# yanyan-li/PlanarSLAM

Measured on AMD Instinct MI355X. Metric: RGB-D frames/sec (extract+match+pose-opt) @640x480; 1->8-GPU batch scaling, higher is better.
Workload: dtype u8/f64

## Files before the change

### include/planar_abi.h

```cpp
#ifndef PLANAR_ABI_H
#define PLANAR_ABI_H

#include <stdint.h>

#ifdef __cplusplus
extern "C" {
#endif

#define PLANAR_OK 0
#define PLANAR_EINVAL (-1)
#define PLANAR_ENOMEM (-2)
#define PLANAR_EDEVICE (-3)
#define PLANAR_ECAPACITY (-4)
#define PLANAR_ESTATE (-5)

typedef struct planar_ctx planar_ctx;

typedef struct planar_keypoint {
    float x, y;
    float size;
    float angle;
    float response;
    int32_t octave;
    int32_t class_id;
// ... 193 lines not shown
    float level_sigma2[PLANAR_MAX_LEVELS];
} planar_tri_camera;

typedef struct planar_tri_keyframes {
    int32_t count, stride;
    const int32_t* n;
    const planar_keypoint* keys_un;
    const float* u_right;
    const uint8_t* desc;
    const int32_t* node;
    const uint8_t* occupied;
    const float* Tcw;
    const planar_keypoint* keys;
    const float* depth;
    const float* cos_stereo;
    const float* Twc;
    const float* mb;
    const float* mbf;
} planar_tri_keyframes;

int planar_search_for_triangulation(planar_ctx* ctx, const planar_tri_camera* cam, const planar_tri_keyframes* kf1, const planar_tri_keyframes* kf2,
                                    int only_stereo, int check_orientation, int32_t* match12, int32_t* nmatches);
int planar_search_for_triangulation_dev(planar_ctx* ctx, const planar_tri_camera* cam, const planar_tri_keyframes* d_kf1,
                                        const planar_tri_keyframes* d_kf2, int only_stereo, int check_orientation, int32_t* d_match12,
                                        int32_t* d_nmatches);

int planar_create_new_map_points(planar_ctx* ctx, const planar_tri_camera* cam, const planar_tri_keyframes* cur, const planar_tri_keyframes* neigh,
                                 const int32_t* n_neigh, int max_neigh, int32_t* n_new, int32_t* new_neigh, int32_t* new_idx1, int32_t* new_idx2,
                                 float* new_x3d);
int planar_create_new_map_points_dev(planar_ctx* ctx, const planar_tri_camera* cam, const planar_tri_keyframes* d_cur,
                                     const planar_tri_keyframes* d_neigh, const int32_t* d_n_neigh, int max_neigh, int32_t* d_n_new,
                                     int32_t* d_new_neigh, int32_t* d_new_idx1, int32_t* d_new_idx2, float* d_new_x3d);

#define PLANAR_MAX_KEYFRAME_LINES 256

struct planar_keyline;
typedef struct planar_tri_line_keyframes {
    int32_t count, stride;
    const int32_t* n;
    const struct planar_keyline* keylines;
    const uint8_t* ldesc;
    const uint8_t* occupied;
    const float* depth_line;
    const double* lines3d;
    const float* Tcw;
    const float* Twc;
    const float* mb;
} planar_tri_line_keyframes;

int planar_lsd_search_for_triangulation(planar_ctx* ctx, const planar_tri_line_keyframes* kf1, const planar_tri_line_keyframes* kf2, int32_t* match12,
                                        int32_t* nmatches, double* nn_mad, double* nn12_mad);
int planar_lsd_search_for_triangulation_dev(planar_ctx* ctx, const planar_tri_line_keyframes* d_kf1, const planar_tri_line_keyframes* d_kf2,
                                            int32_t* d_match12, int32_t* d_nmatches, double* d_nn_mad, double* d_nn12_mad);
int planar_lsd_search_by_descriptor_kf(planar_ctx* ctx, const planar_tri_line_keyframes* kf1, const planar_tri_line_keyframes* kf2, int32_t* match12,
                                       int32_t* nmatches);
int planar_lsd_search_by_descriptor_kf_dev(planar_ctx* ctx, const planar_tri_line_keyframes* d_kf1, const planar_tri_line_keyframes* d_kf2,
                                           int32_t* d_match12, int32_t* d_nmatches);

int planar_create_new_map_lines(planar_ctx* ctx, const planar_tri_camera* cam, const planar_tri_line_keyframes* cur, const planar_tri_line_keyframes* neigh,
                                const int32_t* n_neigh, int max_neigh, int32_t* n_new, int32_t* new_neigh, int32_t* new_idx1, int32_t* new_idx2,
                                double* new_line);
int planar_create_new_map_lines_dev(planar_ctx* ctx, const planar_tri_camera* cam, const planar_tri_line_keyframes* d_cur,
                                    const planar_tri_line_keyframes* d_neigh, const int32_t* d_n_neigh, int max_neigh, int32_t* d_n_new,
                                    int32_t* d_new_neigh, int32_t* d_new_idx1, int32_t* d_new_idx2, double* d_new_line);

int planar_update_average_dir(planar_ctx* ctx, int G, const int32_t* n, int stride, const double* xw6, const uint8_t* valid, const float* ref_Tcw,
                              const int32_t* ref_octave, const int32_t* obs_off, const float* obs_ow, const float* scale_factors, int n_levels,
                              double* normal, float* min_dist, float* max_dist);
int planar_update_average_dir_dev(planar_ctx* ctx, int G, const int32_t* d_n, int stride, const double* d_xw6, const uint8_t* d_valid,
                                  const float* d_ref_Tcw, const int32_t* d_ref_octave, const int32_t* d_obs_off, const float* d_obs_ow,
                                  const float* scale_factors, int n_levels, double* d_normal, float* d_min_dist, float* d_max_dist);

int planar_is_in_frustum_points(planar_ctx* ctx, const planar_frame_view* frame, float log_scale_factor, int n_levels, const int32_t* n, int stride,
                                const uint8_t* valid, const float* xw, const float* normal, const float* min_dist, const float* max_dist,
                                float viewing_cos_limit, uint8_t* in_view, float* proj_x, float* proj_y, float* proj_xr, int32_t* level,
                                float* view_cos);
int planar_is_in_frustum_points_dev(planar_ctx* ctx, const planar_frame_view* d_frame, float log_scale_factor, int n_levels, const int32_t* d_n,
                                    int stride, const uint8_t* d_valid, const float* d_xw, const float* d_normal, const float* d_min_dist,
                                    const float* d_max_dist, float viewing_cos_limit, uint8_t* d_in_view, float* d_proj_x, float* d_proj_y,
                                    float* d_proj_xr, int32_t* d_level, float* d_view_cos);
int planar_is_in_frustum_lines(planar_ctx* ctx, const planar_frame_view* frame, float log_scale_factor, const int32_t* n, int stride,
                               const uint8_t* valid, const double* xw6, const double* normal, const float* min_dist, const float* max_dist,
                               float viewing_cos_limit, uint8_t* in_view, float* proj, int32_t* level, float* view_cos);
int planar_is_in_frustum_lines_dev(planar_ctx* ctx, const planar_frame_view* d_frame, float log_scale_factor, const int32_t* d_n, int stride,
                                   const uint8_t* d_valid, const double* d_xw6, const double* d_normal, const float* d_min_dist,
                                   const float* d_max_dist, float viewing_cos_limit, uint8_t* d_in_view, float* d_proj, int32_t* d_level,
                                   float* d_view_cos);

int planar_fuse_search(planar_ctx* ctx, const planar_frame_view* kf, const float* inv_level_sigma2, float log_scale_factor, int n_levels,
                       const int32_t* n, int stride, int points_shared, const uint8_t* usable, const float* xw, const float* normal,
                       const float* min_dist, const float* max_dist, const uint8_t* desc, float th, int32_t* fuse_idx, int32_t* fuse_dist,
                       int32_t* n_fused);
int planar_fuse_search_dev(planar_ctx* ctx, const planar_frame_view* d_kf, const float* inv_level_sigma2 , float log_scale_factor, int n_levels,
                           const int32_t* d_n, int stride, int points_shared, const uint8_t* d_usable, const float* d_xw, const float* d_normal,
                           const float* d_min_dist, const float* d_max_dist, const uint8_t* d_desc, float th, int32_t* d_fuse_idx,
                           int32_t* d_fuse_dist, int32_t* d_n_fused);

typedef struct planar_keyline {
    float angle;
    int32_t class_id, octave;
    float pt_x, pt_y, response, size;
    float start_x, start_y, end_x, end_y;
    float s_oct_x, s_oct_y, e_oct_x, e_oct_y;
    float line_length;
    int32_t num_pixels;
} planar_keyline;

int planar_lsd_search_by_projection(planar_ctx* ctx, int B, const int32_t* n_lines, int line_stride, const planar_keyline* keylines,
                                    const uint8_t* ldesc, const uint8_t* blocked, const int32_t* n_ml, int ml_stride,
                                    const uint8_t* ml_in_view, const float* ml_proj, const int32_t* ml_level, const float* ml_view_cos,
                                    const uint8_t* ml_desc, const uint8_t* ml_observed, const float* scale_factors, int n_levels, float th,
                                    float nn_ratio, int32_t* match, int32_t* nmatches);
int planar_lsd_search_by_projection_dev(planar_ctx* ctx, int B, const int32_t* d_n_lines, int line_stride, const planar_keyline* d_keylines,
                                        const uint8_t* d_ldesc, const uint8_t* d_blocked, const int32_t* d_n_ml, int ml_stride,
                                        const uint8_t* d_ml_in_view, const float* d_ml_proj, const int32_t* d_ml_level,
                                        const float* d_ml_view_cos, const uint8_t* d_ml_desc, const uint8_t* d_ml_observed,
                                        const float* scale_factors , int n_levels, float th, float nn_ratio, int32_t* d_match,
                                        int32_t* d_nmatches);

int planar_lsd_fuse_search(planar_ctx* ctx, const planar_frame_view* kf, float log_scale_factor, int n_levels, const int32_t* n_lines, int line_stride,
                           const planar_keyline* keylines, const uint8_t* ldesc, const int32_t* n_ml, int ml_stride, int lines_shared,
                           const uint8_t* usable, const double* xw6, const double* normal, const float* min_dist, const float* max_dist,
                           const uint8_t* ml_desc, float th, int32_t* fuse_idx, int32_t* fuse_dist, int32_t* n_fused);
int planar_lsd_fuse_search_dev(planar_ctx* ctx, const planar_frame_view* d_kf, float log_scale_factor, int n_levels, const int32_t* d_n_lines, int line_stride,
                               const planar_keyline* d_keylines, const uint8_t* d_ldesc, const int32_t* d_n_ml, int ml_stride, int lines_shared,
                               const uint8_t* d_usable, const double* d_xw6, const double* d_normal, const float* d_min_dist, const float* d_max_dist,
                               const uint8_t* d_ml_desc, float th, int32_t* d_fuse_idx, int32_t* d_fuse_dist, int32_t* d_n_fused);

int planar_plane_search_by_coefficients(planar_ctx* ctx, int B, const int32_t* n_planes, int pl_stride, const float* pl_coef,
                                        const float* Tcw, int map_shared, const int32_t* n_mp, int mp_stride, const uint8_t* mp_valid,
                                        const float* mp_coef, const int32_t* mp_npts, int pts_stride, const float* mp_pts,
                                        const float* th, int32_t* match, int32_t* ver, int32_t* par, int32_t* nmatches);
int planar_plane_search_by_coefficients_dev(planar_ctx* ctx, int B, const int32_t* d_n_planes, int pl_stride, const float* d_pl_coef,
                                            const float* d_Tcw, int map_shared, const int32_t* d_n_mp, int mp_stride,
                                            const uint8_t* d_mp_valid, const float* d_mp_coef, const int32_t* d_mp_npts, int pts_stride,
                                            const float* d_mp_pts, const float* th , int32_t* d_match, int32_t* d_ver,
                                            int32_t* d_par, int32_t* d_nmatches);

typedef struct planar_lsd planar_lsd;
int planar_lsd_create(planar_ctx* ctx, int width, int height, int max_batch, planar_lsd** out);
void planar_lsd_destroy(planar_lsd* lsd);
int planar_lsd_max_segments(void);
int planar_lsd_scaled_size(planar_lsd* lsd, int* w, int* h);
int planar_lsd_set_tie_order(planar_lsd* lsd, int tie_order);
int planar_lsd_set_top_only(planar_lsd* lsd, int enable);
int planar_lsd_extract(planar_lsd* lsd, const uint8_t* gray, int B, int pitch, int64_t frame_stride, int max_lines, planar_keyline* keylines,
                       uint8_t* ldesc, double* line_eq, int32_t* n_lines);
int planar_lsd_extract_dev(planar_lsd* lsd, const uint8_t* d_gray, int B, int pitch, int64_t frame_stride, int max_lines,
                           planar_keyline* d_keylines, uint8_t* d_ldesc, double* d_line_eq, int32_t* d_n_lines);
int planar_lsd_preprocess_dev(planar_lsd* lsd, const uint8_t* d_gray, int B, int pitch, int64_t frame_stride);
int planar_lsd_detect_dev(planar_lsd* lsd, int B, int max_lines, planar_keyline* d_keylines, uint8_t* d_ldesc, double* d_line_eq, int32_t* d_n_lines);
int planar_lsd_check(planar_lsd* lsd, int B);
int planar_lsd_read_stage(planar_lsd* lsd, int frame, int stage, void* out, int64_t out_bytes);
int planar_lsd_set_profiling(planar_lsd* lsd, int enable);
int planar_lsd_get_profile(planar_lsd* lsd, double* total_ms, int64_t* calls);
#ifdef PLANAR_TEST_HOOKS
int planar_debug_std_sort_desc(planar_ctx* ctx, float* keys, int32_t* perm, int n);
#endif

typedef struct planar_peac planar_peac;
int planar_peac_create(planar_ctx* ctx, int width, int height, int max_batch, planar_peac** out);
void planar_peac_destroy(planar_peac* peac);
int planar_peac_max_planes(void);
int planar_peac_segment(planar_peac* peac, const uint16_t* depth, int B, int pitch_px, int64_t frame_stride_px, float fx, float fy,
                        float cx, float cy, float depth_factor, int32_t* labels, double* planes, int32_t* n_planes);
int planar_peac_segment_dev(planar_peac* peac, const uint16_t* d_depth, int B, int pitch_px, int64_t frame_stride_px, float fx, float fy,
                            float cx, float cy, float depth_factor, int32_t* d_labels, double* d_planes, int32_t* d_n_planes);
int planar_peac_debug_layout(planar_peac* peac, int64_t* out );
int planar_peac_debug_read(planar_peac* peac, int frame, int64_t offset, int64_t bytes, void* out);
int planar_peac_check(planar_peac* peac, int B);
int planar_peac_set_variant(planar_peac* peac, int clustering, int wide_below);
int planar_peac_set_profiling(planar_peac* peac, int enable);
int planar_peac_get_profile(planar_peac* peac, double* total_ms, int64_t* calls);
int planar_peac_read_timing(planar_peac* peac, int B, int64_t* out);

typedef struct planar_comm planar_comm;
typedef struct planar_comm_id { char internal[128]; } planar_comm_id;
int planar_comm_unique_id(planar_comm_id* out);
int planar_comm_create(planar_ctx* ctx, const planar_comm_id* id, int nranks, int rank, planar_comm** out);
typedef int (*planar_allreduce_fn)(void* user, double* buf, size_t n, int op);
int planar_comm_create_hosted(planar_ctx* ctx, planar_allreduce_fn allreduce, void* user, int nranks, int rank, planar_comm** out);
void planar_comm_destroy(planar_comm* comm);

#define PLANAR_BA_MONO 0
#define PLANAR_BA_STEREO 1
#define PLANAR_BA_LINE 2
#define PLANAR_BA_PLANE 3
#define PLANAR_BA_VERTICAL 4
#define PLANAR_BA_PARALLEL 5

typedef struct planar_ba_problem {
    int32_t n_kf;
    const float* kf_Tcw;
    const uint8_t* kf_fixed;
    int32_t n_lm;
    const uint8_t* lm_type;
    const double* lm_init;
    int32_t n_edges;
    const int32_t* e_kf;
    const int32_t* e_lm;
    const uint8_t* e_type;
    const double* e_meas;
    const float* e_inv_sigma2;
} planar_ba_problem;

typedef struct planar_ba_result {
    float* kf_Tcw;
    double* lm;
    uint8_t* e_outlier;
    int32_t lm_iterations;
    int32_t stopped;
} planar_ba_result;

int planar_local_ba(planar_ctx* ctx, const planar_ba_problem* problem, const planar_pose_params* params, int its1, int its2,
                    planar_ba_result* result, const volatile unsigned char* stop_flag, planar_comm* comm);

typedef struct planar_vocab planar_vocab;
int planar_vocab_create(planar_ctx* ctx, int k, int L, int n_nodes, const int32_t* parent, const uint8_t* is_leaf, const uint8_t* desc ,
                        const double* weight, planar_vocab** out);
void planar_vocab_destroy(planar_vocab* voc);
int planar_vocab_words(const planar_vocab* voc);
int planar_bow_transform(planar_vocab* voc, const uint8_t* desc, const int32_t* n, int B, int stride, int levelsup, int32_t* word, double* weight,
                         int32_t* node, int32_t* bow_word, double* bow_value, int32_t* bow_n);
int planar_bow_transform_dev(planar_vocab* voc, const uint8_t* d_desc, const int32_t* d_n, int B, int stride, int levelsup, int32_t* d_word,
                             double* d_weight, int32_t* d_node, int32_t* d_bow_word, double* d_bow_value, int32_t* d_bow_n);

#define PLANAR_KFDB_MAX_WORDS 4096
#define PLANAR_KFDB_MAX_KEYFRAMES 1024
typedef struct planar_kf_database {
    int32_t kf_stride, word_stride;
    const int32_t* n_kf;
    const uint8_t* present;
    const int32_t* add_seq;
    const int32_t* bow_n;
    const int32_t* bow_word;
    const double*  bow_value;
    const int32_t* covis;
} planar_kf_database;
int planar_kfdb_detect(planar_ctx* ctx, int mode, const planar_kf_database* db, int B, const int32_t* q_db, const int32_t* q_bow_n, const int32_t* q_bow_word,
                       const double* q_bow_value, int q_word_stride, const uint8_t* excluded, const float* min_score, float* score, int32_t* common_words,
                       int32_t* n_cand, int32_t* cand, int32_t* n_scored);
int planar_kfdb_detect_dev(planar_ctx* ctx, int mode, const planar_kf_database* db, int B, const int32_t* d_q_db, const int32_t* d_q_bow_n,
                           const int32_t* d_q_bow_word, const double* d_q_bow_value, int q_word_stride, const uint8_t* d_excluded, const float* d_min_score,
                           float* d_score, int32_t* d_common_words, int32_t* d_n_cand, int32_t* d_cand, int32_t* d_n_scored);
int planar_bow_score(planar_ctx* ctx, int P, const int32_t* a_bow_n, const int32_t* a_bow_word, const double* a_bow_value, int a_stride, const int32_t* b_bow_n,
                     const int32_t* b_bow_word, const double* b_bow_value, int b_stride, double* out);
int planar_bow_score_dev(planar_ctx* ctx, int P, const int32_t* d_a_bow_n, const int32_t* d_a_bow_word, const double* d_a_bow_value, int a_stride,
                         const int32_t* d_b_bow_n, const int32_t* d_b_bow_word, const double* d_b_bow_value, int b_stride, double* d_out);

int planar_is_line_good(planar_ctx* ctx, int B, const planar_keyline* keylines, const int32_t* n_lines, int ln_stride, const uint16_t* depth, int width,
                        int height, int pitch_px, int64_t frame_stride_px, float depth_factor, float fx, float fy, float cx, float cy, const uint32_t* seeds,
                        float* depth_line, double* lines3d, uint8_t* good, double* direction, int32_t* n_inliers, double* packed_dirs, int32_t* n_good);
int planar_is_line_good_dev(planar_ctx* ctx, int B, const planar_keyline* d_keylines, const int32_t* d_n_lines, int ln_stride, const uint16_t* d_depth,
                            int width, int height, int pitch_px, int64_t frame_stride_px, float depth_factor, float fx, float fy, float cx, float cy,
                            const uint32_t* d_seeds, float* d_depth_line, double* d_lines3d, uint8_t* d_good, double* d_direction, int32_t* d_n_inliers,
                            double* d_packed_dirs, int32_t* d_n_good);

typedef struct planar_normals planar_normals;
int planar_normals_create(planar_ctx* ctx, int width, int height, int max_batch, planar_normals** out);
void planar_normals_destroy(planar_normals* nrm);
int planar_normals_count(const planar_normals* nrm);
int planar_normals_grid(const planar_normals* nrm, int* grid_w, int* grid_h, int* out_w, int* out_h);
int planar_normals_compute(planar_normals* nrm, const uint16_t* depth, int B, int pitch_px, int64_t frame_stride_px, float fx, float fy, float cx,
                           float cy, float depth_factor, float* normals , float* points );
int planar_normals_compute_dev(planar_normals* nrm, const uint16_t* d_depth, int B, int pitch_px, int64_t frame_stride_px, float fx, float fy,
                               float cx, float cy, float depth_factor, float* d_normals, float* d_points, int out_stride);

int planar_track_manhattan_frame(planar_ctx* ctx, int B, const float* R_last, const float* normals, const int32_t* n_normals, int sn_stride,
                                 const double* line_dirs, const int32_t* n_lines, int ln_stride, float* R_out, uint8_t* member, int32_t* info,
                                 float* density);
int planar_track_manhattan_frame_dev(planar_ctx* ctx, int B, const float* d_R_last, const float* d_normals, const int32_t* d_n_normals, int sn_stride,
                                     const double* d_line_dirs, const int32_t* d_n_lines, int ln_stride, float* d_R_out, uint8_t* d_member,
                                     int32_t* d_info, float* d_density);

typedef struct planar_plane_clouds planar_plane_clouds;
int planar_plane_clouds_create(planar_ctx* ctx, int width, int height, int max_batch, int max_points , planar_plane_clouds** out);
void planar_plane_clouds_destroy(planar_plane_clouds* pc);
int planar_plane_clouds_stride(const planar_plane_clouds* pc, int* pl_stride, int* max_points);
int planar_plane_clouds_set_plane_window(planar_plane_clouds* pc, int first, int count);
int planar_plane_clouds_set_profiling(planar_plane_clouds* pc, int enable);
int planar_plane_clouds_get_profile(planar_plane_clouds* pc, double* total_ms, int64_t* calls);
int planar_plane_clouds_sort_stats(planar_plane_clouds* pc, int B, int64_t* out);
int planar_plane_clouds_set_timing(planar_plane_clouds* pc, int enable);
int planar_plane_clouds_read_timing(planar_plane_clouds* pc, int B, int64_t* out);
int planar_plane_clouds_compute(planar_plane_clouds* pc, const uint16_t* depth, int B, int pitch_px, int64_t frame_stride_px, float fx, float fy, float cx,
                                float cy, float depth_factor, const int32_t* labels, const double* planes, const int32_t* n_planes, double dist_th, float leaf,
                                int32_t* n_out, float* coef, int32_t* src, int32_t* pt_off, float* points, int32_t* state, int32_t* nvox, int32_t* info);
int planar_plane_clouds_compute_dev(planar_plane_clouds* pc, const uint16_t* d_depth, int B, int pitch_px, int64_t frame_stride_px, float fx, float fy,
                                    float cx, float cy, float depth_factor, const int32_t* d_labels, const double* d_planes, const int32_t* d_n_planes,
                                    double dist_th, float leaf, int32_t* d_n_out, float* d_coef, int32_t* d_src, int32_t* d_pt_off, float* d_points,
                                    int32_t* d_status, int32_t* d_state, int32_t* d_nvox, int32_t* d_info);
int planar_plane_clouds_last_status(planar_plane_clouds* pc, int B, int32_t* out);
int planar_plane_refit(planar_plane_clouds* pc, int n_clouds, const float* points, const int32_t* pt_off, double dist_th, float* planes, int32_t* state,
                       int32_t* info);
int planar_flag_matched_plane_points(planar_ctx* ctx, int B, const float* Tcw, const float* coef, const uint8_t* matched, const int32_t* n_planes, int pl_stride,
                                     const float* xw, int n_points, int points_shared, uint8_t* flags, int32_t* n_matches);
int planar_flag_matched_plane_points_dev(planar_ctx* ctx, int B, const float* d_Tcw, const float* d_coef, const uint8_t* d_matched, const int32_t* d_n_planes,
                                         int pl_stride, const float* d_xw, int n_points, int points_shared, uint8_t* d_flags, int32_t* d_n_matches);
int planar_merge_plane_points(planar_plane_clouds* pc, const double* Twc, const float* frame_points, int n_frame, const float* map_points, int n_map, float leaf,
                              float* out_points, int out_cap, int32_t* n_out);

int planar_stereo_from_rgbd(planar_ctx* ctx, int B, const planar_keypoint* keys, const planar_keypoint* keys_un, const int32_t* n, int stride,
                            const uint16_t* depth, int pitch_px, int64_t frame_stride_px, float depth_factor, float fx, float fy, float cx, float cy,
                            float bf, const float* Tcw, float* u_right, float* depth_out, float* xw, uint8_t* valid);
int planar_stereo_from_rgbd_dev(planar_ctx* ctx, int B, const planar_keypoint* d_keys, const planar_keypoint* d_keys_un, const int32_t* d_n, int stride,
                                const uint16_t* d_depth, int pitch_px, int64_t frame_stride_px, float depth_factor, float fx, float fy, float cx,
// ... 56 lines not shown
```

### planarslam_amd/_lib.py

```python
from __future__ import annotations

import ctypes as C
import os

import numpy as np

_HERE = os.path.dirname(os.path.abspath(__file__))
LIB_PATH = os.path.join(_HERE, "libplanar_hip.so")
if os.environ.get("PLANAR_HIP_LIB"):
    _ov = os.path.abspath(os.environ["PLANAR_HIP_LIB"])
    if os.path.dirname(_ov) != _HERE:
        raise ImportError(f"PLANAR_HIP_LIB={_ov}: a developer override must be a library inside {_HERE}")
    import warnings
    warnings.warn(f"planarslam_amd: loading the developer build {_ov} instead of libplanar_hip.so (PLANAR_HIP_LIB)")
    LIB_PATH = _ov

KP_DTYPE = np.dtype([("x", "<f4"), ("y", "<f4"), ("size", "<f4"), ("angle", "<f4"), ("response", "<f4"),
                     ("octave", "<i4"), ("class_id", "<i4")])


class PlanarError(RuntimeError):
    def __init__(self, code: int, msg: str):
        super().__init__(f"libplanar_hip error {code}: {msg}")
        self.code = code
# ... 26 lines not shown
KEYLINE_DTYPE = np.dtype([("angle", "<f4"), ("class_id", "<i4"), ("octave", "<i4"), ("pt_x", "<f4"), ("pt_y", "<f4"), ("response", "<f4"),
                          ("size", "<f4"), ("start_x", "<f4"), ("start_y", "<f4"), ("end_x", "<f4"), ("end_y", "<f4"), ("s_oct_x", "<f4"),
                          ("s_oct_y", "<f4"), ("e_oct_x", "<f4"), ("e_oct_y", "<f4"), ("line_length", "<f4"), ("num_pixels", "<i4")])
MAX_LEVELS = 16


class FrameView(C.Structure):
    _fields_ = [("B", C.c_int32), ("stride", C.c_int32), ("n", C.c_void_p), ("keys_un", C.c_void_p), ("u_right", C.c_void_p),
                ("desc", C.c_void_p), ("blocked", C.c_void_p), ("Tcw", C.c_void_p), ("min_x", C.c_float), ("max_x", C.c_float),
                ("min_y", C.c_float), ("max_y", C.c_float), ("grid_w_inv", C.c_float), ("grid_h_inv", C.c_float), ("fx", C.c_float),
                ("fy", C.c_float), ("cx", C.c_float), ("cy", C.c_float), ("bf", C.c_float), ("b", C.c_float),
                ("scale_factors", C.c_float * MAX_LEVELS)]


class LastFrameView(C.Structure):
    _fields_ = [("stride", C.c_int32)] + [(n, C.c_void_p) for n in ("n", "Tcw", "usable", "xw", "octave", "angle", "mp_desc", "mp_observed")]


class MapProbes(C.Structure):
    _fields_ = [("stride", C.c_int32)] + [(n, C.c_void_p) for n in ("n", "in_view", "proj_x", "proj_y", "proj_xr", "level", "view_cos", "desc",
                                                                   "observed")]


class KeyframeProbes(C.Structure):
    _fields_ = [("stride", C.c_int32)] + [(n, C.c_void_p) for n in ("n", "usable", "found", "xw", "min_dist", "max_dist", "angle", "desc")]


class TriCamera(C.Structure):
    _fields_ = [("fx", C.c_float), ("fy", C.c_float), ("cx", C.c_float), ("cy", C.c_float), ("invfx", C.c_float), ("invfy", C.c_float),
                ("scale_factor", C.c_float), ("n_levels", C.c_int32), ("scale_factors", C.c_float * MAX_LEVELS), ("level_sigma2", C.c_float * MAX_LEVELS)]


class TriLineKeyframes(C.Structure):
    _fields_ = [("count", C.c_int32), ("stride", C.c_int32)] + [(n, C.c_void_p) for n in ("n", "keylines", "ldesc", "occupied", "depth_line", "lines3d", "Tcw", "Twc", "mb")]


class TriKeyframes(C.Structure):
    _fields_ = [("count", C.c_int32), ("stride", C.c_int32)] + [(n, C.c_void_p) for n in ("n", "keys_un", "u_right", "desc", "node", "occupied", "Tcw", "keys",
                                                                                       "depth", "cos_stereo", "Twc", "mb", "mbf")]


class TrackMatches(C.Structure):
    _fields_ = [("B", C.c_int32), ("stride", C.c_int32), ("mp_stride", C.c_int32), ("n_levels", C.c_int32), ("n", C.c_void_p), ("keys_un", C.c_void_p),
                ("u_right", C.c_void_p), ("pt_match", C.c_void_p), ("mp_xw", C.c_void_p), ("mp_valid", C.c_void_p), ("inv_level_sigma2", C.c_float * MAX_LEVELS),
                ("ln_stride", C.c_int32), ("ml_stride", C.c_int32), ("n_lines", C.c_void_p), ("line_eq", C.c_void_p), ("ln_match", C.c_void_p), ("ml_xw6", C.c_void_p),
                ("pl_stride", C.c_int32), ("mpl_stride", C.c_int32), ("mpl_shared", C.c_int32), ("n_planes", C.c_void_p), ("pl_coef", C.c_void_p),
                ("pl_match", C.c_void_p), ("mpl_coef", C.c_void_p), ("Tcw", C.c_void_p)]


class KfDatabase(C.Structure):
    _fields_ = [("kf_stride", C.c_int32), ("word_stride", C.c_int32)] + [(n, C.c_void_p) for n in ("n_kf", "present", "add_seq", "bow_n", "bow_word", "bow_value", "covis")]


KFDB_MAX_WORDS = 4096
KFDB_MAX_KEYFRAMES = 1024


class BAResult(C.Structure):
    _fields_ = [("kf_Tcw", C.c_void_p), ("lm", C.c_void_p), ("e_outlier", C.c_void_p), ("lm_iterations", C.c_int32), ("stopped", C.c_int32)]


_SIGS = {
    "planar_last_error": (C.c_char_p, []),
    "planar_abi_version": (C.c_int, []),
    "planar_ctx_create": (C.c_int, [C.POINTER(C.c_void_p), C.c_int]),
    "planar_ctx_destroy": (None, [C.c_void_p]),
    "planar_ctx_set_stream": (C.c_int, [C.c_void_p, C.c_void_p]),
    "planar_ctx_get_stream": (C.c_void_p, [C.c_void_p]),
    "planar_cu_stream_create": (C.c_int, [C.c_int, C.c_void_p, C.c_int, C.POINTER(C.c_void_p)]),
    "planar_cu_stream_destroy": (None, [C.c_void_p]),
    "planar_ctx_set_seq_stream": (C.c_int, [C.c_void_p, C.c_void_p]),
    "planar_ctx_sync": (C.c_int, [C.c_void_p]),
    "planar_orb_create": (C.c_int, [C.c_void_p, C.POINTER(OrbParams), C.c_int, C.c_int, C.c_int, C.POINTER(C.c_void_p)]),
    "planar_orb_destroy": (None, [C.c_void_p]),
    "planar_orb_check": (C.c_int, [C.c_void_p]),
    "planar_peac_set_profiling": (C.c_int, [C.c_void_p, C.c_int]),
    "planar_peac_get_profile": (C.c_int, [C.c_void_p, C.c_void_p, C.POINTER(C.c_int64)]),
    "planar_orb_max_keypoints": (C.c_int, [C.c_void_p]),
    "planar_orb_get_scale_factors": (C.c_int, [C.c_void_p, C.c_void_p, C.c_void_p, C.c_void_p, C.c_void_p]),
    "planar_orb_level_size": (C.c_int, [C.c_void_p, C.c_int, C.POINTER(C.c_int), C.POINTER(C.c_int)]),
    "planar_orb_features_per_level": (C.c_int, [C.c_void_p, C.c_void_p]),
    "planar_orb_extract": (C.c_int, [C.c_void_p, C.c_void_p, C.c_int, C.c_int, C.c_int64, C.c_void_p, C.c_void_p, C.c_void_p]),
    "planar_orb_extract_dev": (C.c_int, [C.c_void_p, C.c_void_p, C.c_int, C.c_int, C.c_int64, C.c_void_p, C.c_void_p, C.c_void_p]),
    "planar_orb_read_level": (C.c_int, [C.c_void_p, C.c_int, C.c_int, C.c_void_p]),
    "planar_orb_read_blurred": (C.c_int, [C.c_void_p, C.c_int, C.c_int, C.c_void_p]),
    "planar_orb_read_candidates": (C.c_int, [C.c_void_p, C.c_int, C.c_int, C.c_void_p, C.c_int]),
    "planar_orb_set_profiling": (C.c_int, [C.c_void_p, C.c_int]),
    "planar_orb_profile_num_launches": (C.c_int, [C.c_void_p]),
    "planar_orb_profile_launch_name": (C.c_char_p, [C.c_void_p, C.c_int]),
    "planar_orb_get_profile": (C.c_int, [C.c_void_p, C.c_void_p, C.POINTER(C.c_int64)]),
    "planar_hamming_knn": (C.c_int, [C.c_void_p, C.c_void_p, C.c_void_p, C.c_int, C.c_void_p, C.c_void_p, C.c_int, C.c_int, C.c_int, C.c_void_p, C.c_void_p]),
    "planar_hamming_knn_dev": (C.c_int, [C.c_void_p, C.c_void_p, C.c_void_p, C.c_int, C.c_void_p, C.c_void_p, C.c_int, C.c_int, C.c_int, C.c_void_p, C.c_void_p]),
    "planar_match_orb_points": (C.c_int, [C.c_void_p, C.c_void_p, C.c_void_p, C.c_int, C.c_void_p, C.c_void_p, C.c_int, C.c_void_p, C.c_void_p, C.c_int, C.c_void_p, C.c_void_p]),
    "planar_match_orb_points_dev": (C.c_int, [C.c_void_p, C.c_void_p, C.c_void_p, C.c_int, C.c_void_p, C.c_void_p, C.c_int, C.c_void_p, C.c_void_p, C.c_int, C.c_void_p, C.c_void_p]),
    "planar_lsd_search_by_descriptor": (C.c_int, [C.c_void_p, C.c_void_p, C.c_void_p, C.c_int, C.c_void_p, C.c_void_p, C.c_int, C.c_void_p, C.c_int, C.c_void_p, C.c_void_p]),
    "planar_lsd_search_by_descriptor_dev": (C.c_int, [C.c_void_p, C.c_void_p, C.c_void_p, C.c_int, C.c_void_p, C.c_void_p, C.c_int, C.c_void_p, C.c_int, C.c_void_p, C.c_void_p]),
    "planar_search_by_projection_frame": (C.c_int, [C.c_void_p, C.POINTER(FrameView), C.POINTER(LastFrameView), C.c_float, C.c_int, C.c_int, C.c_void_p, C.c_void_p]),
    "planar_search_by_projection_frame_dev": (C.c_int, [C.c_void_p, C.POINTER(FrameView), C.POINTER(LastFrameView), C.c_float, C.c_int, C.c_int, C.c_void_p, C.c_void_p]),
    "planar_search_by_projection_map": (C.c_int, [C.c_void_p, C.POINTER(FrameView), C.POINTER(MapProbes), C.c_float, C.c_float, C.c_void_p, C.c_void_p]),
    "planar_search_by_projection_map_dev": (C.c_int, [C.c_void_p, C.POINTER(FrameView), C.POINTER(MapProbes), C.c_float, C.c_float, C.c_void_p, C.c_void_p]),
    "planar_search_by_projection_keyframe": (C.c_int, [C.c_void_p, C.POINTER(FrameView), C.POINTER(KeyframeProbes), C.c_float, C.c_int, C.c_float, C.c_int, C.c_int, C.c_void_p, C.c_void_p]),
    "planar_search_by_projection_keyframe_dev": (C.c_int, [C.c_void_p, C.POINTER(FrameView), C.POINTER(KeyframeProbes), C.c_float, C.c_int, C.c_float, C.c_int, C.c_int, C.c_void_p, C.c_void_p]),
    "planar_fuse_search": (C.c_int, [C.c_void_p, C.POINTER(FrameView), C.c_void_p, C.c_float, C.c_int, C.c_void_p, C.c_int, C.c_int] + [C.c_void_p] * 6 + [C.c_float] + [C.c_void_p] * 3),
    "planar_fuse_search_dev": (C.c_int, [C.c_void_p, C.POINTER(FrameView), C.c_void_p, C.c_float, C.c_int, C.c_void_p, C.c_int, C.c_int] + [C.c_void_p] * 6 + [C.c_float] + [C.c_void_p] * 3),
    "planar_lsd_fuse_search": (C.c_int, [C.c_void_p, C.POINTER(FrameView), C.c_float, C.c_int, C.c_void_p, C.c_int, C.c_void_p, C.c_void_p, C.c_void_p, C.c_int, C.c_int] + [C.c_void_p] * 6 + [C.c_float] + [C.c_void_p] * 3),
    "planar_lsd_fuse_search_dev": (C.c_int, [C.c_void_p, C.POINTER(FrameView), C.c_float, C.c_int, C.c_void_p, C.c_int, C.c_void_p, C.c_void_p, C.c_void_p, C.c_int, C.c_int] + [C.c_void_p] * 6 + [C.c_float] + [C.c_void_p] * 3),
    "planar_is_in_frustum_points": (C.c_int, [C.c_void_p, C.POINTER(FrameView), C.c_float, C.c_int, C.c_void_p, C.c_int] + [C.c_void_p] * 5 + [C.c_float] + [C.c_void_p] * 6),
    "planar_is_in_frustum_points_dev": (C.c_int, [C.c_void_p, C.POINTER(FrameView), C.c_float, C.c_int, C.c_void_p, C.c_int] + [C.c_void_p] * 5 + [C.c_float] + [C.c_void_p] * 6),
    "planar_is_in_frustum_lines": (C.c_int, [C.c_void_p, C.POINTER(FrameView), C.c_float, C.c_void_p, C.c_int] + [C.c_void_p] * 5 + [C.c_float] + [C.c_void_p] * 4),
    "planar_is_in_frustum_lines_dev": (C.c_int, [C.c_void_p, C.POINTER(FrameView), C.c_float, C.c_void_p, C.c_int] + [C.c_void_p] * 5 + [C.c_float] + [C.c_void_p] * 4),
    "planar_search_for_triangulation": (C.c_int, [C.c_void_p, C.POINTER(TriCamera), C.POINTER(TriKeyframes), C.POINTER(TriKeyframes), C.c_int, C.c_int, C.c_void_p, C.c_void_p]),
    "planar_search_for_triangulation_dev": (C.c_int, [C.c_void_p, C.POINTER(TriCamera), C.POINTER(TriKeyframes), C.POINTER(TriKeyframes), C.c_int, C.c_int, C.c_void_p, C.c_void_p]),
    "planar_create_new_map_points": (C.c_int, [C.c_void_p, C.POINTER(TriCamera), C.POINTER(TriKeyframes), C.POINTER(TriKeyframes), C.c_void_p, C.c_int] + [C.c_void_p] * 5),
    "planar_create_new_map_points_dev": (C.c_int, [C.c_void_p, C.POINTER(TriCamera), C.POINTER(TriKeyframes), C.POINTER(TriKeyframes), C.c_void_p, C.c_int] + [C.c_void_p] * 5),
    "planar_lsd_search_for_triangulation": (C.c_int, [C.c_void_p, C.POINTER(TriLineKeyframes), C.POINTER(TriLineKeyframes)] + [C.c_void_p] * 4),
    "planar_lsd_search_for_triangulation_dev": (C.c_int, [C.c_void_p, C.POINTER(TriLineKeyframes), C.POINTER(TriLineKeyframes)] + [C.c_void_p] * 4),
    "planar_lsd_search_by_descriptor_kf": (C.c_int, [C.c_void_p, C.POINTER(TriLineKeyframes), C.POINTER(TriLineKeyframes)] + [C.c_void_p] * 2),
    "planar_lsd_search_by_descriptor_kf_dev": (C.c_int, [C.c_void_p, C.POINTER(TriLineKeyframes), C.POINTER(TriLineKeyframes)] + [C.c_void_p] * 2),
    "planar_create_new_map_lines": (C.c_int, [C.c_void_p, C.POINTER(TriCamera), C.POINTER(TriLineKeyframes), C.POINTER(TriLineKeyframes), C.c_void_p, C.c_int] + [C.c_void_p] * 5),
    "planar_create_new_map_lines_dev": (C.c_int, [C.c_void_p, C.POINTER(TriCamera), C.POINTER(TriLineKeyframes), C.POINTER(TriLineKeyframes), C.c_void_p, C.c_int] + [C.c_void_p] * 5),
    "planar_update_average_dir": (C.c_int, [C.c_void_p, C.c_int, C.c_void_p, C.c_int] + [C.c_void_p] * 7 + [C.c_int] + [C.c_void_p] * 3),
    "planar_update_average_dir_dev": (C.c_int, [C.c_void_p, C.c_int, C.c_void_p, C.c_int] + [C.c_void_p] * 7 + [C.c_int] + [C.c_void_p] * 3),
    "planar_search_by_bow": (C.c_int, [C.c_void_p, C.c_int] + [C.c_void_p, C.c_int, C.c_void_p, C.c_void_p, C.c_void_p, C.c_void_p] +
                             [C.c_void_p, C.c_int, C.c_void_p, C.c_void_p, C.c_void_p] + [C.c_float, C.c_int, C.c_void_p, C.c_void_p]),
    "planar_search_by_bow_dev": (C.c_int, [C.c_void_p, C.c_int] + [C.c_void_p, C.c_int, C.c_void_p, C.c_void_p, C.c_void_p, C.c_void_p] +
                                 [C.c_void_p, C.c_int, C.c_void_p, C.c_void_p, C.c_void_p] + [C.c_float, C.c_int, C.c_void_p, C.c_void_p]),
    "planar_lsd_search_by_projection": (C.c_int, [C.c_void_p, C.c_int, C.c_void_p, C.c_int, C.c_void_p, C.c_void_p, C.c_void_p, C.c_void_p, C.c_int] +
                                        [C.c_void_p] * 6 + [C.c_void_p, C.c_int, C.c_float, C.c_float, C.c_void_p, C.c_void_p]),
    "planar_lsd_search_by_projection_dev": (C.c_int, [C.c_void_p, C.c_int, C.c_void_p, C.c_int, C.c_void_p, C.c_void_p, C.c_void_p, C.c_void_p, C.c_int] +
                                            [C.c_void_p] * 6 + [C.c_void_p, C.c_int, C.c_float, C.c_float, C.c_void_p, C.c_void_p]),
    "planar_plane_search_by_coefficients": (C.c_int, [C.c_void_p, C.c_int, C.c_void_p, C.c_int, C.c_void_p, C.c_void_p, C.c_int, C.c_void_p, C.c_int,
                                                      C.c_void_p, C.c_void_p, C.c_void_p, C.c_int, C.c_void_p, C.c_void_p] + [C.c_void_p] * 4),
    "planar_plane_search_by_coefficients_dev": (C.c_int, [C.c_void_p, C.c_int, C.c_void_p, C.c_int, C.c_void_p, C.c_void_p, C.c_int, C.c_void_p, C.c_int,
                                                          C.c_void_p, C.c_void_p, C.c_void_p, C.c_int, C.c_void_p, C.c_void_p] + [C.c_void_p] * 4),
    "planar_lsd_create": (C.c_int, [C.c_void_p, C.c_int, C.c_int, C.c_int, C.POINTER(C.c_void_p)]),
    "planar_lsd_destroy": (None, [C.c_void_p]),
    "planar_lsd_max_segments": (C.c_int, []),
    "planar_lsd_set_tie_order": (C.c_int, [C.c_void_p, C.c_int]),
    "planar_lsd_set_top_only": (C.c_int, [C.c_void_p, C.c_int]),
    "planar_undistort_keypoints": (C.c_int, [C.c_void_p, C.c_int, C.c_void_p, C.c_void_p, C.c_int] + [C.c_float] * 4 + [C.c_void_p, C.c_void_p]),
    "planar_undistort_keypoints_dev": (C.c_int, [C.c_void_p, C.c_int, C.c_void_p, C.c_void_p, C.c_int] + [C.c_float] * 4 + [C.c_void_p, C.c_void_p]),
    "planar_plane_clouds_sort_stats": (C.c_int, [C.c_void_p, C.c_int, C.c_void_p]),
    "planar_plane_clouds_set_profiling": (C.c_int, [C.c_void_p, C.c_int]),
    "planar_plane_clouds_get_profile": (C.c_int, [C.c_void_p, C.c_void_p, C.c_void_p]),
    "planar_lsd_set_profiling": (C.c_int, [C.c_void_p, C.c_int]),
    "planar_lsd_get_profile": (C.c_int, [C.c_void_p, C.c_void_p, C.c_void_p]),
    "planar_lsd_scaled_size": (C.c_int, [C.c_void_p, C.POINTER(C.c_int), C.POINTER(C.c_int)]),
    "planar_lsd_extract": (C.c_int, [C.c_void_p, C.c_void_p, C.c_int, C.c_int, C.c_int64, C.c_int, C.c_void_p, C.c_void_p, C.c_void_p, C.c_void_p]),
    "planar_lsd_extract_dev": (C.c_int, [C.c_void_p, C.c_void_p, C.c_int, C.c_int, C.c_int64, C.c_int, C.c_void_p, C.c_void_p, C.c_void_p, C.c_void_p]),
    "planar_lsd_preprocess_dev": (C.c_int, [C.c_void_p, C.c_void_p, C.c_int, C.c_int, C.c_int64]),
    "planar_lsd_detect_dev": (C.c_int, [C.c_void_p, C.c_int, C.c_int, C.c_void_p, C.c_void_p, C.c_void_p, C.c_void_p]),
    "planar_lsd_check": (C.c_int, [C.c_void_p, C.c_int]),
    "planar_lsd_read_stage": (C.c_int, [C.c_void_p, C.c_int, C.c_int, C.c_void_p, C.c_int64]),
    "planar_debug_std_sort_desc": (C.c_int, [C.c_void_p, C.c_void_p, C.c_void_p, C.c_int]),
    "planar_peac_create": (C.c_int, [C.c_void_p, C.c_int, C.c_int, C.c_int, C.POINTER(C.c_void_p)]),
    "planar_peac_destroy": (None, [C.c_void_p]),
    "planar_peac_max_planes": (C.c_int, []),
    "planar_peac_segment": (C.c_int, [C.c_void_p, C.c_void_p, C.c_int, C.c_int, C.c_int64, C.c_float, C.c_float, C.c_float, C.c_float, C.c_float, C.c_void_p, C.c_void_p, C.c_void_p]),
    "planar_peac_segment_dev": (C.c_int, [C.c_void_p, C.c_void_p, C.c_int, C.c_int, C.c_int64, C.c_float, C.c_float, C.c_float, C.c_float, C.c_float, C.c_void_p, C.c_void_p, C.c_void_p]),
    "planar_peac_check": (C.c_int, [C.c_void_p, C.c_int]),
    "planar_peac_set_variant": (C.c_int, [C.c_void_p, C.c_int, C.c_int]),
    "planar_track_manhattan_frame": (C.c_int, [C.c_void_p, C.c_int, C.c_void_p, C.c_void_p, C.c_void_p, C.c_int, C.c_void_p, C.c_void_p, C.c_int, C.c_void_p, C.c_void_p, C.c_void_p, C.c_void_p]),
    "planar_track_manhattan_frame_dev": (C.c_int, [C.c_void_p, C.c_int, C.c_void_p, C.c_void_p, C.c_void_p, C.c_int, C.c_void_p, C.c_void_p, C.c_int, C.c_void_p, C.c_void_p, C.c_void_p, C.c_void_p]),
    "planar_peac_read_timing": (C.c_int, [C.c_void_p, C.c_int, C.c_void_p]),
    "planar_reset_matches_dev": (C.c_int, [C.c_void_p, C.c_void_p, C.c_int64]),
    "planar_blocked_mask_dev": (C.c_int, [C.c_void_p, C.c_void_p, C.c_int64, C.c_void_p]),
    "planar_merge_matches_dev": (C.c_int, [C.c_void_p, C.c_void_p, C.c_void_p, C.c_int, C.c_int64, C.c_void_p]),
    "planar_manhattan_pose_dev": (C.c_int, [C.c_void_p, C.c_int, C.c_void_p, C.c_void_p, C.c_void_p, C.c_void_p]),
    "planar_keypoint_fields_dev": (C.c_int, [C.c_void_p, C.c_void_p, C.c_int64, C.c_void_p, C.c_void_p]),
    "planar_add_scalar_i32_dev": (C.c_int, [C.c_void_p, C.c_void_p, C.c_int64, C.c_int, C.c_void_p]),
    "planar_copy_rows_dev": (C.c_int, [C.c_void_p, C.c_void_p, C.c_int64, C.c_void_p, C.c_int64, C.c_int64, C.c_int64]),
    "planar_peac_debug_layout": (C.c_int, [C.c_void_p, C.c_void_p]),
    "planar_peac_debug_read": (C.c_int, [C.c_void_p, C.c_int, C.c_int64, C.c_int64, C.c_void_p]),
    "planar_comm_unique_id": (C.c_int, [C.c_void_p]),
    "planar_comm_create": (C.c_int, [C.c_void_p, C.c_void_p, C.c_int, C.c_int, C.POINTER(C.c_void_p)]),
    "planar_vocab_create": (C.c_int, [C.c_void_p, C.c_int, C.c_int, C.c_int, C.c_void_p, C.c_void_p, C.c_void_p, C.c_void_p, C.POINTER(C.c_void_p)]),
    "planar_vocab_destroy": (None, [C.c_void_p]),
    "planar_vocab_words": (C.c_int, [C.c_void_p]),
    "planar_bow_transform": (C.c_int, [C.c_void_p, C.c_void_p, C.c_void_p, C.c_int, C.c_int, C.c_int] + [C.c_void_p] * 6),
    "planar_bow_transform_dev": (C.c_int, [C.c_void_p, C.c_void_p, C.c_void_p, C.c_int, C.c_int, C.c_int] + [C.c_void_p] * 6),
    "planar_kfdb_detect": (C.c_int, [C.c_void_p, C.c_int, C.POINTER(KfDatabase), C.c_int] + [C.c_void_p] * 4 + [C.c_int] + [C.c_void_p] * 7),
    "planar_kfdb_detect_dev": (C.c_int, [C.c_void_p, C.c_int, C.POINTER(KfDatabase), C.c_int] + [C.c_void_p] * 4 + [C.c_int] + [C.c_void_p] * 7),
    "planar_bow_score": (C.c_int, [C.c_void_p, C.c_int] + [C.c_void_p] * 3 + [C.c_int] + [C.c_void_p] * 3 + [C.c_int, C.c_void_p]),
    "planar_bow_score_dev": (C.c_int, [C.c_void_p, C.c_int] + [C.c_void_p] * 3 + [C.c_int] + [C.c_void_p] * 3 + [C.c_int, C.c_void_p]),
    "planar_is_line_good": (C.c_int, [C.c_void_p, C.c_int, C.c_void_p, C.c_void_p, C.c_int, C.c_void_p, C.c_int, C.c_int, C.c_int, C.c_int64, C.c_float, C.c_float, C.c_float, C.c_float, C.c_float] + [C.c_void_p] * 8),
    "planar_is_line_good_dev": (C.c_int, [C.c_void_p, C.c_int, C.c_void_p, C.c_void_p, C.c_int, C.c_void_p, C.c_int, C.c_int, C.c_int, C.c_int64, C.c_float, C.c_float, C.c_float, C.c_float, C.c_float] + [C.c_void_p] * 8),
    "planar_normals_create": (C.c_int, [C.c_void_p, C.c_int, C.c_int, C.c_int, C.POINTER(C.c_void_p)]),
    "planar_normals_destroy": (None, [C.c_void_p]),
    "planar_normals_count": (C.c_int, [C.c_void_p]),
    "planar_normals_grid": (C.c_int, [C.c_void_p, C.POINTER(C.c_int), C.POINTER(C.c_int), C.POINTER(C.c_int), C.POINTER(C.c_int)]),
    "planar_normals_compute": (C.c_int, [C.c_void_p, C.c_void_p, C.c_int, C.c_int, C.c_int64, C.c_float, C.c_float, C.c_float, C.c_float, C.c_float, C.c_void_p, C.c_void_p]),
    "planar_normals_compute_dev": (C.c_int, [C.c_void_p, C.c_void_p, C.c_int, C.c_int, C.c_int64, C.c_float, C.c_float, C.c_float, C.c_float, C.c_float, C.c_void_p,
                                            C.c_void_p, C.c_int]),
    "planar_plane_clouds_create": (C.c_int, [C.c_void_p, C.c_int, C.c_int, C.c_int, C.c_int, C.POINTER(C.c_void_p)]),
    "planar_plane_clouds_destroy": (None, [C.c_void_p]),
    "planar_plane_clouds_set_timing": (C.c_int, [C.c_void_p, C.c_int]),
    "planar_plane_clouds_read_timing": (C.c_int, [C.c_void_p, C.c_int, C.c_void_p]),
    "planar_plane_clouds_stride": (C.c_int, [C.c_void_p, C.POINTER(C.c_int), C.POINTER(C.c_int)]),
    "planar_plane_clouds_set_plane_window": (C.c_int, [C.c_void_p, C.c_int, C.c_int]),
    "planar_plane_clouds_compute": (C.c_int, [C.c_void_p, C.c_void_p, C.c_int, C.c_int, C.c_int64, C.c_float, C.c_float, C.c_float, C.c_float, C.c_float, C.c_void_p, C.c_void_p,
                                             C.c_void_p, C.c_double, C.c_float] + [C.c_void_p] * 8),
    "planar_plane_clouds_compute_dev": (C.c_int, [C.c_void_p, C.c_void_p, C.c_int, C.c_int, C.c_int64, C.c_float, C.c_float, C.c_float, C.c_float, C.c_float, C.c_void_p,
                                                 C.c_void_p, C.c_void_p, C.c_double, C.c_float] + [C.c_void_p] * 9),
    "planar_plane_clouds_last_status": (C.c_int, [C.c_void_p, C.c_int, C.c_void_p]),
    "planar_plane_refit": (C.c_int, [C.c_void_p, C.c_int, C.c_void_p, C.c_void_p, C.c_double, C.c_void_p, C.c_void_p, C.c_void_p]),
    "planar_flag_matched_plane_points": (C.c_int, [C.c_void_p, C.c_int, C.c_void_p, C.c_void_p, C.c_void_p, C.c_void_p, C.c_int, C.c_void_p, C.c_int, C.c_int, C.c_void_p, C.c_void_p]),
    "planar_flag_matched_plane_points_dev": (C.c_int, [C.c_void_p, C.c_int, C.c_void_p, C.c_void_p, C.c_void_p, C.c_void_p, C.c_int, C.c_void_p, C.c_int, C.c_int, C.c_void_p,
                                                      C.c_void_p]),
    "planar_merge_plane_points": (C.c_int, [C.c_void_p, C.c_void_p, C.c_void_p, C.c_int, C.c_void_p, C.c_int, C.c_float, C.c_void_p, C.c_int, C.c_void_p]),
    "planar_distinctive_descriptors": (C.c_int, [C.c_void_p, C.c_int, C.c_void_p, C.c_void_p, C.c_void_p, C.c_void_p]),
    "planar_distinctive_descriptors_dev": (C.c_int, [C.c_void_p, C.c_int, C.c_void_p, C.c_void_p, C.c_int, C.c_void_p, C.c_void_p]),
    "planar_update_normal_and_depth": (C.c_int, [C.c_void_p, C.c_int, C.c_void_p, C.c_int] + [C.c_void_p] * 7 + [C.c_int] + [C.c_void_p] * 3),
    "planar_update_normal_and_depth_dev": (C.c_int, [C.c_void_p, C.c_int, C.c_void_p, C.c_int] + [C.c_void_p] * 7 + [C.c_int] + [C.c_void_p] * 3),
    "planar_comm_create_hosted": (C.c_int, [C.c_void_p, C.c_void_p, C.c_void_p, C.c_int, C.c_int, C.POINTER(C.c_void_p)]),
    "planar_comm_destroy": (None, [C.c_void_p]),
    "planar_local_ba": (C.c_int, [C.c_void_p, C.POINTER(BAProblem), C.POINTER(PoseParams), C.c_int, C.c_int, C.POINTER(BAResult), C.c_void_p, C.c_void_p]),
    "planar_stereo_from_rgbd": (C.c_int, [C.c_void_p, C.c_int, C.c_void_p, C.c_void_p, C.c_void_p, C.c_int, C.c_void_p, C.c_int, C.c_int64] + [C.c_float] * 6 + [C.c_void_p] * 5),
    "planar_stereo_from_rgbd_dev": (C.c_int, [C.c_void_p, C.c_int, C.c_void_p, C.c_void_p, C.c_void_p, C.c_int, C.c_void_p, C.c_int, C.c_int64] + [C.c_float] * 6 + [C.c_void_p] * 5),
    "planar_pose_assemble": (C.c_int, [C.c_void_p, C.POINTER(TrackMatches), C.POINTER(PoseBatch)]),
    "planar_pose_assemble_dev": (C.c_int, [C.c_void_p, C.POINTER(TrackMatches), C.POINTER(PoseBatch)]),
    "planar_discard_outliers": (C.c_int, [C.c_void_p, C.c_int, C.c_void_p, C.c_int, C.c_int, C.c_void_p, C.c_void_p, C.c_void_p]),
    "planar_discard_outliers_dev": (C.c_int, [C.c_void_p, C.c_int, C.c_void_p, C.c_int, C.c_int, C.c_void_p, C.c_void_p, C.c_void_p]),
    "planar_pose_opt": (C.c_int, [C.c_void_p, C.POINTER(PoseBatch), C.POINTER(PoseParams), C.c_int, C.c_int, C.c_int]),
    "planar_pose_opt_dev": (C.c_int, [C.c_void_p, C.POINTER(PoseBatch), C.POINTER(PoseParams), C.c_int, C.c_int, C.c_int]),
}

TEST_HOOKS = ("planar_debug_std_sort_desc",)
_LIB = None


def exported_symbols():
    return sorted(n for n in _SIGS if n not in TEST_HOOKS)


def lib():
    global _LIB
    if _LIB is None:
        if not os.path.exists(LIB_PATH):
            raise OSError(f"{LIB_PATH} not built: run `python -c 'import __graft_entry__ as g; g.build()'` "
                          "(hipcc --offload-arch=gfx950); there is no CPU fallback")
        L = C.CDLL(LIB_PATH)
        for name, (res, args) in _SIGS.items():
            if name in TEST_HOOKS and not hasattr(L, name):
                continue
            f = getattr(L, name)
            f.restype = res
            f.argtypes = args
        _LIB = L
    return _LIB


def check(rc: int):
    if rc < 0:
        raise PlanarError(rc, lib().planar_last_error().decode(errors="replace"))
    return rc


def cu_stream_create(device: int, n_cus: int, first: int = 0, total: int = 256) -> int:
    import numpy as np
    words = np.zeros((total + 31) // 32, np.uint32)
    for i in range(first, min(first + n_cus, total)):
        words[i >> 5] |= np.uint32(1 << (i & 31))
    out = C.c_void_p()
    check(lib().planar_cu_stream_create(device, words.ctypes.data, len(words), C.byref(out)))
    return out.value


class Context:

    def __init__(self, device: int = 0, stream: int | None = None):
        self.L = lib()
        h = C.c_void_p()
        check(self.L.planar_ctx_create(C.byref(h), device))
        self.h = h
        self.device = device
        if stream is not None:
            self.set_stream(stream)

    def set_stream(self, hip_stream: int | None):
        check(self.L.planar_ctx_set_stream(self.h, C.c_void_p(hip_stream) if hip_stream else None))

    def set_seq_stream(self, hip_stream: int | None):
        check(self.L.planar_ctx_set_seq_stream(self.h, C.c_void_p(hip_stream) if hip_stream else None))

    def sync(self):
        check(self.L.planar_ctx_sync(self.h))

    def close(self):
        if getattr(self, "h", None):
            self.L.planar_ctx_destroy(self.h)
            self.h = None

    def __del__(self):
        try:
            self.close()
        except Exception:
            pass
```

### planarslam_amd/csrc/common.h

```cpp
#pragma once
#include <hip/hip_runtime.h>

#include <cstdarg>
#include <cstdint>
#include <cstdio>
#include <cstring>
#include <vector>

#include "../../include/planar_abi.h"

namespace planar {

void set_error(const char* fmt, ...);

#define PLANAR_HIP_CHECK(expr)                                                                        \
    do {                                                                                              \
        hipError_t _e = (expr);                                                                       \
        if (_e != hipSuccess) {                                                                       \
            ::planar::set_error("%s failed: %s (%s:%d)", #expr, hipGetErrorString(_e), __FILE__, __LINE__); \
            return (_e == hipErrorOutOfMemory) ? PLANAR_ENOMEM : PLANAR_EDEVICE;                      \
        }                                                                                             \
    } while (0)

#define PLANAR_REQUIRE(cond, code, msg)                  \
    do {                                                 \
        if (!(cond)) {                                   \
            ::planar::set_error("%s: %s", __func__, msg); \
            return (code);                               \
        }                                                \
    } while (0)

template <typename T>
static inline T align_up(T v, T a) { return (v + a - 1) / a * a; }

struct DevBuf {
    void* p = nullptr;
    size_t bytes = 0;
    int alloc(size_t n) {
        release();
        if (n == 0) n = 16;
        hipError_t e = hipMalloc(&p, n);
        if (e != hipSuccess) { p = nullptr; set_error("hipMalloc(%zu) failed: %s", n, hipGetErrorString(e)); return PLANAR_ENOMEM; }
        bytes = n;
        return PLANAR_OK;
    }
    void release() { if (p) { (void)hipFree(p); p = nullptr; bytes = 0; } }
    ~DevBuf() { release(); }
    template <typename T> T* as() const { return (T*)p; }
};

struct Stager {
    struct Item { const void* h_in; void* h_out; size_t bytes; size_t off; void* field; };
    template <typename T> struct Dev {
        const Stager* s = nullptr; size_t off = 0;
        operator T*() const { return s ? (T*)(s->buf.as<uint8_t>() + off) : nullptr; }
    };
    std::vector<Item> items;
    size_t total = 0;
    DevBuf buf;
    template <typename T> Dev<const T> in(const T* h, size_t count) { return h ? add<const T>(h, nullptr, count) : Dev<const T>{}; }
    template <typename T> Dev<T> out(T* h, size_t count) { return h ? add<T>(nullptr, h, count) : Dev<T>{}; }
    template <typename T> Dev<T> inout(T* h, size_t count) { return h ? add<T>(h, h, count) : Dev<T>{}; }
    template <typename T> Dev<T> temp(size_t count) { return add<T>(nullptr, nullptr, count); }
    template <typename T> void in_field(const T*& field, size_t count) { if (field) add<const T>(field, nullptr, count, &field); }
    template <typename T> void out_field(const T*& field, size_t count) { add<T>(nullptr, const_cast<T*>(field), count, &field); }
    template <typename T> Dev<T> add(const void* hin, void* hout, size_t count, void* field = nullptr) {
        const size_t bytes = count * sizeof(T);
        items.push_back({hin, hout, bytes, total, field});
        total += align_up(bytes ? bytes : (size_t)1, (size_t)256);
        return {this, items.back().off};
    }
    int upload(hipStream_t st) {
        int rc = buf.alloc(total);
        if (rc) return rc;
        for (const Item& it : items) {
            void* const d = buf.as<uint8_t>() + it.off;
            if (it.field) memcpy(it.field, &d, sizeof d);
        }
        for (const Item& it : items)
            if (it.h_in && it.bytes) {
                hipError_t e = hipMemcpyAsync(buf.as<uint8_t>() + it.off, it.h_in, it.bytes, hipMemcpyHostToDevice, st);
                if (e != hipSuccess) { set_error("staging upload failed: %s", hipGetErrorString(e)); return PLANAR_EDEVICE; }
            }
        return PLANAR_OK;
    }
    template <typename T> hipError_t zero_from(const Dev<T>& first, hipStream_t st) { return hipMemsetAsync((T*)first, 0, total - first.off, st); }
    template <typename F> int run(hipStream_t st, F&& launch) {
        int rc = upload(st);
        if (!rc) rc = launch();
        return rc ? rc : download(st);
    }
    int download(hipStream_t st) {
        for (const Item& it : items)
            if (it.h_out && it.bytes) {
                hipError_t e = hipMemcpyAsync(it.h_out, buf.as<uint8_t>() + it.off, it.bytes, hipMemcpyDeviceToHost, st);
                if (e != hipSuccess) { set_error("staging download failed: %s", hipGetErrorString(e)); return PLANAR_EDEVICE; }
            }
        hipError_t e = hipStreamSynchronize(st);
        if (e != hipSuccess) { set_error("stream sync failed: %s", hipGetErrorString(e)); return PLANAR_EDEVICE; }
        return PLANAR_OK;
    }
};

struct LaunchProfile {
    const int slots;
    bool on = false;
    bool open = false;
    std::vector<hipEvent_t> ev;
    std::vector<int> marked;
    size_t used = 0;
    explicit LaunchProfile(int nslots) : slots(nslots) {}
    LaunchProfile(const LaunchProfile&) = delete;
    ~LaunchProfile() { for (hipEvent_t e : ev) (void)hipEventDestroy(e); }
    void reset() { used = 0; open = false; }
    int begin() {
        open = false;
        if (!on) return PLANAR_OK;
        if (used == marked.size()) {
            for (int i = 0; i <= slots; i++) {
                hipEvent_t e;
                const hipError_t err = hipEventCreate(&e);
                if (err != hipSuccess) {
                    for (; i > 0; i--) { (void)hipEventDestroy(ev.back()); ev.pop_back(); }
                    set_error("hipEventCreate failed: %s", hipGetErrorString(err));
                    return err == hipErrorOutOfMemory ? PLANAR_ENOMEM : PLANAR_EDEVICE;
                }
                ev.push_back(e);
            }
            marked.push_back(0);
        }
        marked[used++] = 0;
        open = true;
        return PLANAR_OK;
    }
    void mark(hipStream_t st) {
        if (!open) return;
        int& k = marked[used - 1];
        (void)hipEventRecord(ev[(used - 1) * (slots + 1) + k], st);
        open = ++k <= slots;
    }
    int sum(double* total_ms, int64_t* calls) {
        for (int i = 0; i < slots; i++) total_ms[i] = 0;
        int64_t counted = 0;
        for (size_t c = 0; c < used; c++) {
            if (marked[c] != slots + 1) continue;
            for (int i = 0; i < slots; i++) {
                float ms = 0;
                PLANAR_HIP_CHECK(hipEventElapsedTime(&ms, ev[c * (slots + 1) + i], ev[c * (slots + 1) + i + 1]));
                total_ms[i] += ms;
            }
            counted++;
        }
        *calls = counted;
        reset();
        return PLANAR_OK;
    }
};

#ifdef __HIPCC__
__device__ __forceinline__ void xcd_frame_block(int per_frame, int B, int& frame, int& blk) {
    const int n = (int)blockIdx.x, group = 8 * per_frame, full = (B >> 3) * group;
    if (n < full) { const int g = n / group, r = n - g * group; frame = g * 8 + (r & 7); blk = r >> 3; }
    else { const int r = n - full; frame = (B & ~7) + r / per_frame; blk = r - (r / per_frame) * per_frame; }
}
#endif

}

struct planar_ctx {
    int device = 0;
    hipStream_t own_stream = nullptr;
    hipStream_t stream = nullptr;
    planar::DevBuf scratch;
    hipStream_t seq_stream = nullptr;
    hipEvent_t seq_fork = nullptr, seq_join = nullptr;
    hipStream_t seq_begin() {
        if (!seq_stream) return stream;
        hipError_t e = hipEventRecord(seq_fork, stream);
        if (e == hipSuccess) e = hipStreamWaitEvent(seq_stream, seq_fork, 0);
        if (e == hipSuccess) return seq_stream;
        planar::set_error("planar_ctx: the fork to the side stream failed (%s): launching on the context's stream", hipGetErrorString(e));
        return stream;
    }
    int seq_end(hipStream_t sq) {
        if (!seq_stream || sq != seq_stream) return PLANAR_OK;
        PLANAR_HIP_CHECK(hipEventRecord(seq_join, sq));
        PLANAR_HIP_CHECK(hipStreamWaitEvent(stream, seq_join, 0));
        return PLANAR_OK;
    }
    int ensure_scratch(size_t bytes) {
        if (scratch.bytes >= bytes) return PLANAR_OK;
        if (scratch.p) (void)hipStreamSynchronize(stream);
        return scratch.alloc(bytes);
    }
    void* host_scratch = nullptr;
    size_t host_scratch_bytes = 0;
    int ensure_host_scratch(size_t bytes) {
        if (host_scratch_bytes >= bytes) return PLANAR_OK;
        if (host_scratch) { (void)hipStreamSynchronize(stream); (void)hipHostFree(host_scratch); host_scratch = nullptr; host_scratch_bytes = 0; }
        const size_t want = planar::align_up(bytes + bytes / 4, (size_t)4096);
        hipError_t e = hipHostMalloc(&host_scratch, want, hipHostMallocDefault);
        if (e != hipSuccess) { (void)hipGetLastError(); host_scratch = nullptr; planar::set_error("hipHostMalloc(%zu) failed: %s", want, hipGetErrorString(e)); return PLANAR_EDEVICE; }
        host_scratch_bytes = want;
        return PLANAR_OK;
    }
};
```

### planarslam_amd/csrc/lsd.hip

```cpp
#include "common.h"
#include "ref_arith.h"
#include "wave_ops.h"
#include "lsd_nfa.h"
#include "isort.h"

namespace planar {
namespace lsd {

constexpr double LSD_PI = 3.14159265358979323846;
constexpr double M_3_2_PI = 3 * LSD_PI / 2, M_2__PI = 2 * LSD_PI;
constexpr float NOTDEF_F = -1024.0f;
constexpr double DEG_TO_RADS = LSD_PI / 180;
constexpr double RELATIVE_ERROR_FACTOR = 100.0;
constexpr int N_BINS = 1024;
constexpr int MAX_SEGS = 2048;
constexpr int MAX_RECTS = 4096;
constexpr int RING = 512;
constexpr int USED_LDS_BITS = 32768;

struct Plan {
    int W, H, w, h;
    int taps7[7], taps5[5];
    double rho, prec, p, log_nt, density_th, log_eps;
    int min_reg_size;
    size_t off_blur7, off_blur5, off_dx, off_dy, off_ang, off_g2, off_pix, off_seed, off_ord, off_ordr, off_gused, off_tmp, off_reg, off_valid, off_sortr, off_sortb, off_heapj, off_segs, off_kl, off_rects, off_res, off_est, frame_bytes;
    const double* lgamma_tab;
    double p_log[12], p1_log[12], p_log10[12];
    double gaussCoefL[21], gaussCoefG[63];
};

struct Misc { uint32_t g2max; int n_ord; int n_seg; int n_kl; int status; int n_regions; int n_grown_px; int n_rect; long long t[8]; int sort_counts[2]; int heap_n; int sort_kv; int sort_prefix; int n_refine; float imp_T; int imp_done; int imp_redo; int imp_full; };

__device__ __forceinline__ float fast_atan2_deg(float y, float x) {
    const float scale = (float)(180 / 3.1415926535897932384626433832795);
    const float p1 = 0.9997878412794807f * scale, p3 = -0.3258083974640975f * scale;
    const float p5 = 0.1555786518463281f * scale, p7 = -0.04432655554792128f * scale;
    const float ax = fabsf(x), ay = fabsf(y);
    const bool flat = ax >= ay;
    const float c = (flat ? ay : ax) / ((flat ? ax : ay) + 2.220446049250313e-16f);
    const float c2 = c * c;
    const float t = (((p7 * c2 + p5) * c2 + p3) * c2 + p1) * c;
    float a = flat ? t : 90.f - t;
    if (x < 0) a = 180.f - a;
    if (y < 0) a = 360.f - a;
    return a;
}

__device__ __forceinline__ int reflect101(int p, int n) {
    if (n == 1) return 0;
    while (p < 0 || p >= n) p = p < 0 ? -p : 2 * n - 2 - p;
    return p;
}

template <int KS>
__global__ __launch_bounds__(256) void lsd_gauss(const uint8_t* __restrict__ src, int pitch, int64_t src_stride, int W, int H,
                                                 const int* __restrict__ taps_g, uint8_t* __restrict__ ws, size_t frame_bytes, size_t off_dst, int B) {
    constexpr int R = KS / 2, TW = 64, TH = 16;
    __shared__ uint8_t s_in[TH + 2 * R][TW + 2 * R];
    __shared__ uint16_t s_h[TH + 2 * R][TW];
    int taps[KS];
    for (int i = 0; i < KS; i++) taps[i] = taps_g[i];
    const int tiles_x = (W + TW - 1) / TW, tiles_y = (H + TH - 1) / TH, tid = threadIdx.x;
    int b, tile;
    xcd_frame_block(tiles_x * tiles_y, B, b, tile);
    const int x0 = (tile % tiles_x) * TW, y0 = (tile / tiles_x) * TH;
    const uint8_t* S = src + (int64_t)b * src_stride;
    for (int i = tid; i < (TH + 2 * R) * (TW + 2 * R); i += 256) {
        const int r = i / (TW + 2 * R), c = i % (TW + 2 * R);
        s_in[r][c] = S[(int64_t)reflect101(y0 + r - R, H) * pitch + reflect101(x0 + c - R, W)];
    }
    __syncthreads();
    for (int i = tid; i < (TH + 2 * R) * TW; i += 256) {
        const int r = i / TW, c = i % TW;
        uint32_t s = 0;
        for (int k = 0; k < KS; k++) s += (uint32_t)taps[k] * s_in[r][c + k];
        s_h[r][c] = (uint16_t)min(s, 65535u);
    }
    __syncthreads();
    uint8_t* D = ws + (size_t)b * frame_bytes + off_dst;
    for (int i = tid; i < TH * TW; i += 256) {
        const int r = i / TW, c = i % TW;
        const int x = x0 + c, y = y0 + r;
        if (x >= W || y >= H) continue;
        uint32_t s = 0;
        for (int k = 0; k < KS; k++) s += (uint32_t)taps[k] * s_h[r + k][c];
        D[(size_t)y * W + x] = (uint8_t)min((s + 32768u) >> 16, 255u);
    }
}

__global__ __launch_bounds__(256) void lsd_gauss75(const uint8_t* __restrict__ src, int pitch, int64_t src_stride, int W, int H, const int* __restrict__ taps_g,
                                                   uint8_t* __restrict__ ws, size_t frame_bytes, size_t off7, size_t off5, int B) {
    constexpr int TW = 64, TH = 16, R = 3, NR = TH + 2 * R, NWD = TW / 4 + 2;
    __shared__ uint32_t s_in[NR][NWD + 1];
    __shared__ __attribute__((aligned(8))) uint16_t s_h7[NR][TW + 4], s_h5[NR][TW + 4];
    int t7[7], t5[5];
    for (int i = 0; i < 7; i++) t7[i] = taps_g[i];
    for (int i = 0; i < 5; i++) t5[i] = taps_g[8 + i];
    const int tiles_x = (W + TW - 1) / TW, tiles_y = (H + TH - 1) / TH, tid = threadIdx.x;
    int b, tile;
    xcd_frame_block(tiles_x * tiles_y, B, b, tile);
    const int x0 = (tile % tiles_x) * TW, y0 = (tile / tiles_x) * TH;
    const uint8_t* S = src + (int64_t)b * src_stride;
    for (int i = tid; i < NR * NWD; i += 256) {
        const int r = i / NWD, wq = i - r * NWD;
        const uint8_t* row = S + (int64_t)reflect101(y0 + r - R, H) * pitch;
        const int xb = x0 - 4 + 4 * wq;
        uint32_t v;
        if (xb >= 0 && xb + 3 < W) v = *(const uint32_t*)(row + xb);
        else v = (uint32_t)row[reflect101(xb, W)] | ((uint32_t)row[reflect101(xb + 1, W)] << 8) | ((uint32_t)row[reflect101(xb + 2, W)] << 16) | ((uint32_t)row[reflect101(xb + 3, W)] << 24);
        s_in[r][wq] = v;
    }
    __syncthreads();
    for (int i = tid; i < NR * (TW / 4); i += 256) {
        const int r = i / (TW / 4), q = i - r * (TW / 4);
        const uint32_t w0 = s_in[r][q], w1 = s_in[r][q + 1], w2 = s_in[r][q + 2];
        uint32_t px[12];
#pragma unroll
        for (int k = 0; k < 4; k++) { px[k] = (w0 >> (8 * k)) & 0xffu; px[4 + k] = (w1 >> (8 * k)) & 0xffu; px[8 + k] = (w2 >> (8 * k)) & 0xffu; }
        uint32_t h7[4], h5[4];
#pragma unroll
        for (int o = 0; o < 4; o++) {
            uint32_t a = 0, c = 0;
#pragma unroll
            for (int k = 0; k < 7; k++) a += (uint32_t)t7[k] * px[o + 1 + k];
#pragma unroll
            for (int k = 0; k < 5; k++) c += (uint32_t)t5[k] * px[o + 2 + k];
            h7[o] = min(a, 65535u); h5[o] = min(c, 65535u);
        }
        *(uint2*)&s_h7[r][4 * q] = make_uint2(h7[0] | (h7[1] << 16), h7[2] | (h7[3] << 16));
        *(uint2*)&s_h5[r][4 * q] = make_uint2(h5[0] | (h5[1] << 16), h5[2] | (h5[3] << 16));
    }
    __syncthreads();
    {
        const int r = tid >> 4, q = tid & 15;
        const int x = x0 + 4 * q, y = y0 + r;
        if (x < W && y < H) {
            uint32_t a[4] = {0, 0, 0, 0}, c[4] = {0, 0, 0, 0};
#pragma unroll
            for (int k = 0; k < 7; k++) {
                const uint2 v = *(const uint2*)&s_h7[r + k][4 * q];
                a[0] += (uint32_t)t7[k] * (v.x & 0xffffu); a[1] += (uint32_t)t7[k] * (v.x >> 16); a[2] += (uint32_t)t7[k] * (v.y & 0xffffu); a[3] += (uint32_t)t7[k] * (v.y >> 16);
            }
#pragma unroll
            for (int k = 0; k < 5; k++) {
                const uint2 v = *(const uint2*)&s_h5[r + 1 + k][4 * q];
                c[0] += (uint32_t)t5[k] * (v.x & 0xffffu); c[1] += (uint32_t)t5[k] * (v.x >> 16); c[2] += (uint32_t)t5[k] * (v.y & 0xffffu); c[3] += (uint32_t)t5[k] * (v.y >> 16);
            }
            uint32_t o7 = 0, o5 = 0;
#pragma unroll
            for (int o = 0; o < 4; o++) { o7 |= min((a[o] + 32768u) >> 16, 255u) << (8 * o); o5 |= min((c[o] + 32768u) >> 16, 255u) << (8 * o); }
            uint8_t* F = ws + (size_t)b * frame_bytes;
            *(uint32_t*)(F + off7 + (size_t)y * W + x) = o7;
            *(uint32_t*)(F + off5 + (size_t)y * W + x) = o5;
        }
    }
}

struct Coef { int ofs, c0, c1; };

__device__ __forceinline__ int scaled_px(const uint8_t* __restrict__ B7, int W, const Coef& cx, const Coef& cy) {
    const uint8_t* r0 = B7 + (size_t)cy.ofs * W + cx.ofs;
    const uint8_t* r1 = r0 + W;
    const uint32_t h0 = min((uint32_t)cx.c0 * r0[0] + (uint32_t)cx.c1 * r0[1], 65535u);
    const uint32_t h1 = min((uint32_t)cx.c0 * r1[0] + (uint32_t)cx.c1 * r1[1], 65535u);
    const uint32_t v = h0 * (uint32_t)cy.c0 + h1 * (uint32_t)cy.c1;
    return (int)min((v + 32768u) >> 16, 255u);
}

__device__ __forceinline__ float2 seed_cos_sin(float deg) {
    const double a = (double)deg * DEG_TO_RADS;
    return make_float2((float)cos(a), (float)sin(a));
}

__global__ __launch_bounds__(256) void lsd_grad(const Plan* __restrict__ plan, const Coef* __restrict__ cxs, const Coef* __restrict__ cys,
                                                uint8_t* __restrict__ ws, Misc* __restrict__ miscs) {
    __shared__ uint8_t s_px[5][68];
    const Plan& P = *plan;
    const int b = blockIdx.z;
    const int x0 = blockIdx.x * 64, y0 = blockIdx.y * 4;
    uint8_t* F = ws + (size_t)b * P.frame_bytes;
    const uint8_t* B7 = F + P.off_blur7;
    for (int i = threadIdx.x; i < 5 * 65; i += 256) {
        const int r = i / 65, c = i - r * 65;
        const int xs = min(x0 + c, P.w - 1), ys = min(y0 + r, P.h - 1);
        s_px[r][c] = (uint8_t)scaled_px(B7, P.W, cxs[xs], cys[ys]);
    }
    __syncthreads();
    const int lx = threadIdx.x & 63, ly = threadIdx.x >> 6;
    const int x = x0 + lx, y = y0 + ly;
    if (x >= P.w || y >= P.h) return;
    float* ang = (float*)(F + P.off_ang);
    uint32_t* g2a = (uint32_t*)(F + P.off_g2);
    float4* pix4 = (float4*)(F + P.off_pix);
    Misc* misc = miscs + b;
    const size_t o = (size_t)y * P.w + x;
    if (x >= P.w - 1 || y >= P.h - 1) { ang[o] = NOTDEF_F; g2a[o] = 0; pix4[o] = make_float4(NOTDEF_F, 0.f, 0.f, 0.f); return; }
    const int s00 = s_px[ly][lx], s10 = s_px[ly][lx + 1], s01 = s_px[ly + 1][lx], s11 = s_px[ly + 1][lx + 1];
    const int DA = s11 - s00, BC = s10 - s01;
    const int gx = DA + BC, gy = DA - BC;
    const int g2 = gx * gx + gy * gy;
    const double norm = sqrt(g2 / 4.0);
    g2a[o] = (uint32_t)g2;
    if (norm <= P.rho) { ang[o] = NOTDEF_F; pix4[o] = make_float4(NOTDEF_F, 0.f, 0.f, 0.f); }
    else {
        const float deg = fast_atan2_deg((float)gx, (float)(-gy));
        ang[o] = deg;
        const double a = (double)deg * DEG_TO_RADS;
        const float af = (float)a;
        pix4[o] = make_float4(deg, (float)cos((double)af), (float)sin((double)af), 0.f);
        atomicMax(&misc->g2max, (uint32_t)g2);
    }
}

__device__ __forceinline__ void wave_sync();
__device__ __forceinline__ void lds_sync();
#ifndef PLANAR_WIDE_T
#define PLANAR_WIDE_T 1024
#endif
constexpr int SORT_T = PLANAR_WIDE_T, SORT_LT = 256, SORT_E = 23, SORT_SHIFT = 20, SORT_R = 64;
constexpr int SORT_HJOBS = 1024, SORT_HCAP = 8192, SORT_HY = 2;
using SortLds = isort::LdsLayout<SORT_LT, SORT_E>;
using SortGl = isort::GlobalLayout<SORT_T>;

__global__ __launch_bounds__(SORT_T) void lsd_sort_global(const Plan* __restrict__ plan, uint8_t* __restrict__ ws, Misc* __restrict__ miscs, int rows_cap, int rows_long) {
    extern __shared__ __align__(16) uint8_t sort_lds[];
    __shared__ isort::Range s_init;
    const Plan& P = *plan;
    const int b = blockIdx.x, tid = threadIdx.x, lane = tid & 63;
    uint8_t* F = ws + (size_t)b * P.frame_bytes;
    const uint32_t* g2a = (const uint32_t*)(F + P.off_g2);
    uint32_t* arr = (uint32_t*)(F + P.off_tmp);
    unsigned long long* vb = (unsigned long long*)(F + P.off_valid);
    Misc* misc = miscs + b;
    const int w1 = P.w - 1, h1 = P.h - 1, n = w1 * h1, npix = P.w * P.h;
    const double max_grad = misc->g2max ? sqrt(misc->g2max / 4.0) : -1.0;
    const double bin_coef = (max_grad > 0) ? double(N_BINS - 1) / max_grad : 0;
    const long long ts0 = __builtin_readcyclecounter();
    __shared__ unsigned int s_kv, s_prefix;
    if (tid == 0) { s_kv = 0u; s_prefix = 0u; }
    __syncthreads();
    uint32_t kv = 0;
    for (int p0 = tid - lane; p0 < npix; p0 += SORT_T) {
        const int pix = p0 + lane, y = pix / P.w, x = pix - y * P.w;
        const bool in = pix < npix && x < w1 && y < h1;
        bool valid = false;
        if (in) {
            const double norm = sqrt(g2a[pix] / 4.0);
            const int bin = int(norm * bin_coef);
            arr[pix - y] = ((uint32_t)(N_BINS - 1 - bin) << SORT_SHIFT) | (uint32_t)pix;
            valid = !(norm <= P.rho);
            if (valid) kv = max(kv, (uint32_t)(N_BINS - 1 - bin));
        }
        const unsigned long long m = __ballot(valid);
        if (lane == 0) vb[p0 >> 6] = m;
    }
    kv = (uint32_t)planar::wave_max_f64((double)kv);
    if (lane == 0) atomicMax(&s_kv, kv);
    __syncthreads();
    kv = s_kv;
    int cnt = 0;
    for (int p0 = tid - lane; p0 < npix; p0 += SORT_T) {
        const int pix = p0 + lane, y = pix / P.w, x = pix - y * P.w;
        if (pix < npix && x < w1 && y < h1) cnt += ((arr[pix - y] >> SORT_SHIFT) <= kv) ? 1 : 0;
    }
    cnt = planar::wave_sum_i32(cnt);
    if (lane == 0) atomicAdd(&s_prefix, (unsigned int)cnt);
    if (tid == 0) s_init = isort::Range{0, n, isort::depth_limit(n)};
    __threadfence_block();
    __syncthreads();
    if (tid == 0) { misc->sort_kv = (int)kv; misc->sort_prefix = (int)s_prefix; }
    const isort::HeapSink HS{(isort::HeapJob*)(F + P.off_heapj), &misc->heap_n, SORT_HJOBS};
    isort::global_tier<SORT_SHIFT, SORT_T>(arr, &s_init, 1, SortLds::N, 64, (isort::Range*)(F + P.off_sortr), (isort::Block*)(F + P.off_sortb), isort::G_FMAX,
                                           misc->sort_counts, sort_lds, rows_cap, HS, &misc->status, kv,
                                           rows_long, (uint32_t*)(F + P.off_ord), n / 2 + 1);
    if (tid == 0) misc->t[5] = __builtin_readcyclecounter() - ts0;
}

__global__ __launch_bounds__(SORT_LT, 4) void lsd_sort_lds(const Plan* __restrict__ plan, uint8_t* __restrict__ ws, Misc* __restrict__ miscs) {
    extern __shared__ __align__(16) uint8_t sort_lds[];
    const Plan& P = *plan;
    const int b = blockIdx.x;
    uint8_t* F = ws + (size_t)b * P.frame_bytes;
    Misc* misc = miscs + b;
    const isort::Range* ranges = (const isort::Range*)(F + P.off_sortr);
    const isort::Block* blocks = (const isort::Block*)(F + P.off_sortb);
    const int nb = misc->sort_counts[1];
    const isort::HeapSink HS{(isort::HeapJob*)(F + P.off_heapj), &misc->heap_n, SORT_HJOBS};
    const long long ts0 = __builtin_readcyclecounter();
    for (int k = blockIdx.y; k < nb; k += gridDim.y) {
        const isort::Block K = blocks[k];
        isort::lds_tier<SORT_SHIFT, SORT_LT, SORT_E>((uint32_t*)(F + P.off_tmp), ranges + K.r0, K.nr, K.f, K.l, sort_lds, HS, &misc->status, (uint32_t)misc->sort_kv);
    }
    if (threadIdx.x == 0 && blockIdx.y == 0) misc->t[6] = __builtin_readcyclecounter() - ts0;
}

__global__ __launch_bounds__(64) void lsd_sort_heap(const Plan* __restrict__ plan, uint8_t* __restrict__ ws, Misc* __restrict__ miscs) {
    extern __shared__ __align__(16) uint8_t sort_lds[];
    const Plan& P = *plan;
    uint8_t* F = ws + (size_t)blockIdx.x * P.frame_bytes;
    const int nj = min(miscs[blockIdx.x].heap_n, SORT_HJOBS);
    if (nj) isort::heap_jobs<SORT_SHIFT>((uint32_t*)(F + P.off_tmp), (const isort::HeapJob*)(F + P.off_heapj), nj, blockIdx.y, gridDim.y, (uint32_t*)sort_lds, SORT_HCAP, 0, 1 << 30);
}

__global__ __launch_bounds__(SORT_T) void lsd_sort_compact(const Plan* __restrict__ plan, uint8_t* __restrict__ ws, Misc* __restrict__ miscs) {
    __shared__ int s_cnt[SORT_T / 64];
    const Plan& P = *plan;
    const int b = blockIdx.x, tid = threadIdx.x, lane = tid & 63, wave = tid >> 6;
    uint8_t* F = ws + (size_t)b * P.frame_bytes;
    const uint32_t* arr = (const uint32_t*)(F + P.off_tmp);
    const unsigned long long* vb = (const unsigned long long*)(F + P.off_valid);
    uint32_t* ord = (uint32_t*)(F + P.off_ord);
    uint32_t* ordr = (uint32_t*)(F + P.off_ordr);
    float* pixw = (float*)(F + P.off_pix);
    Misc* misc = miscs + b;
    const int n = min((P.w - 1) * (P.h - 1), misc->sort_prefix);
    const long long ts0 = __builtin_readcyclecounter();
    constexpr int NW = SORT_T / 64, U = 4;
    const int seg = ((n + NW - 1) / NW + 63) & ~63, w0 = min(n, wave * seg), w1 = min(n, w0 + seg);
    auto is_valid = [&](uint32_t e, bool in) { const uint32_t pix = e & 0xfffffu; return in && ((vb[pix >> 6] >> (pix & 63u)) & 1ull); };
    int cnt = 0;
    for (int i0 = w0; i0 < w1; i0 += 64 * U) {
        uint32_t e[U];
#pragma unroll
        for (int u = 0; u < U; u++) e[u] = arr[min(i0 + 64 * u + lane, w1 - 1)];
#pragma unroll
        for (int u = 0; u < U; u++) cnt += __popcll(__ballot(is_valid(e[u], i0 + 64 * u + lane < w1)));
    }
    if (lane == 0) s_cnt[wave] = cnt;
    __syncthreads();
    int pos = 0, total = 0;
    for (int q = 0; q < NW; q++) { if (q < wave) pos += s_cnt[q]; total += s_cnt[q]; }
    for (int i0 = w0; i0 < w1; i0 += 64 * U) {
        uint32_t e[U];
#pragma unroll
        for (int u = 0; u < U; u++) e[u] = arr[min(i0 + 64 * u + lane, w1 - 1)];
#pragma unroll
        for (int u = 0; u < U; u++) {
            const bool v = is_valid(e[u], i0 + 64 * u + lane < w1);
            const unsigned long long m = __ballot(v);
            if (v) {
                const uint32_t pix = e[u] & 0xfffffu, slot = (uint32_t)(pos + __popcll(m & ((1ull << lane) - 1ull)));
                ord[slot] = pix; ordr[slot] = slot;
                pixw[(size_t)pix * 4 + 3] = __uint_as_float(slot);
            }
            pos += __popcll(m);
        }
    }
    if (tid == 0) { misc->n_ord = total; misc->t[7] = __builtin_readcyclecounter() - ts0; }
}

constexpr int SORT_NT = 256, SORT_NW = SORT_NT / 64;
__global__ __launch_bounds__(SORT_NT) void lsd_sort_raster(const Plan* __restrict__ plan, uint8_t* __restrict__ ws, Misc* __restrict__ miscs) {
    __shared__ int wsum[SORT_NW];
    __shared__ int cnt[32 * SORT_NW];
    const Plan& P = *plan;
    const int b = blockIdx.x, tid = threadIdx.x, lane = tid & 63, wave = tid >> 6;
    uint8_t* F = ws + (size_t)b * P.frame_bytes;
    const float* ang = (const float*)(F + P.off_ang);
    const uint32_t* g2a = (const uint32_t*)(F + P.off_g2);
    uint32_t* arr = (uint32_t*)(F + P.off_tmp);
    uint32_t* ord = (uint32_t*)(F + P.off_ord);
    uint32_t* ordr = (uint32_t*)(F + P.off_ordr);
// ... 917 lines not shown
            __threadfence_block();
            __syncthreads();
            if (partial) {
                bool tie = false;
                for (int i = lane; i < min(n - 1, max_lines); i += 64) tie = tie || key[i] == key[i + 1];
                if ((__ballot(tie) != 0ull || phase == 3) && lane == 0) misc->imp_redo = 1;
            }
        }
        for (int i = lane; i < nk; i += 64) {
            const planar_keyline kl = make_keyline(segs[idx[i]], P.W, P.H, n > max_lines ? i : idx[i]);
            K[i] = kl; Kws[i] = kl;
            const double sp0 = kl.start_x, sp1 = kl.start_y, ep0 = kl.end_x, ep1 = kl.end_y;
            const double l0 = sp1 * 1.0 - 1.0 * ep1, l1 = 1.0 * ep0 - sp0 * 1.0, l2 = sp0 * ep1 - sp1 * ep0;
            const double nrm = sqrt(l0 * l0 + l1 * l1 + l2 * l2);
            double* E = out_eq + ((size_t)b * max_lines + i) * 3;
            E[0] = l0 / nrm; E[1] = l1 / nrm; E[2] = l2 / nrm;
        }
    };
    if (n <= LDS_SORT) body(key_l, idx_l);
    else body((float*)(F + P.off_tmp), (int*)(F + P.off_tmp) + MAX_SEGS);
    if (lane == 0) { n_out[b] = misc->status ? 0 : nk; misc->n_kl = nk; }
}

constexpr int NUM_OF_BANDS = 9, WIDTH_OF_BAND = 7, LSP_H = 63;
__constant__ int LBD_COMB[32][2] = {{0, 1}, {0, 2}, {0, 3}, {0, 4}, {0, 5}, {0, 6}, {1, 2}, {1, 3}, {1, 4}, {1, 5}, {1, 6}, {2, 3}, {2, 4}, {2, 5}, {2, 6}, {2, 7},
                                    {2, 8}, {3, 4}, {3, 5}, {3, 6}, {3, 7}, {3, 8}, {4, 5}, {4, 6}, {4, 7}, {4, 8}, {5, 6}, {5, 7}, {5, 8}, {6, 7}, {6, 8}, {7, 8}};

__global__ __launch_bounds__(64) void lbd_describe(const Plan* __restrict__ plan, uint8_t* __restrict__ ws, const Misc* __restrict__ miscs, int max_lines,
                                                   uint8_t* __restrict__ out_desc, int B) {
    __shared__ float row[LSP_H][8];
    __shared__ float des[NUM_OF_BANDS * 8];
    const Plan& P = *plan;
    int b, li;
    xcd_frame_block(max_lines, B, b, li);
    const int lane = threadIdx.x;
    uint8_t* F = ws + (size_t)b * P.frame_bytes;
    const Misc* misc = miscs + b;
    if (li >= misc->n_kl) return;
    const planar_keyline L = ((const planar_keyline*)(F + P.off_kl))[li];
    const uint8_t* S5 = F + P.off_blur5;
    const short realWidth = (short)P.W, imageWidth = (short)(P.W - 1), imageHeight = (short)(P.H - 1);
    const short lengthOfLSP = (short)L.num_pixels;
    const short halfWidth = (lengthOfLSP - 1) / 2, halfHeight = (LSP_H - 1) / 2;
    const float lineMiddlePointX = (float)(0.5 * (L.s_oct_x + L.e_oct_x));
    const float lineMiddlePointY = (float)(0.5 * (L.s_oct_y + L.e_oct_y));
    float dL[2], dO[2];
    dL[0] = (float)cos((double)L.angle); dL[1] = (float)sin((double)L.angle);
    dO[0] = -dL[1]; dO[1] = dL[0];
    if (lane < LSP_H) {
        float sCorX0 = -dL[0] * halfWidth + dL[1] * halfHeight + lineMiddlePointX;
        float sCorY0 = -dL[1] * halfWidth - dL[0] * halfHeight + lineMiddlePointY;
        for (int h = 0; h < lane; h++) { sCorX0 -= dL[1]; sCorY0 += dL[0]; }
        float sCorX = sCorX0, sCorY = sCorY0;
        float pgdLRowSum = 0, ngdLRowSum = 0, pgdORowSum = 0, ngdORowSum = 0;
        for (short wID = 0; wID < lengthOfLSP; wID++) {
            short tempCor = (short)roundf(sCorX);
            const short xCor = (tempCor < 0) ? 0 : (tempCor > imageWidth) ? imageWidth : tempCor;
            tempCor = (short)roundf(sCorY);
            const short yCor = (tempCor < 0) ? 0 : (tempCor > imageHeight) ? imageHeight : tempCor;
            const uint8_t* r0 = S5 + (size_t)reflect101(yCor - 1, P.H) * realWidth;
            const uint8_t* r1 = S5 + (size_t)yCor * realWidth;
            const uint8_t* r2 = S5 + (size_t)reflect101(yCor + 1, P.H) * realWidth;
            const int xm = reflect101(xCor - 1, P.W), xp = reflect101(xCor + 1, P.W);
            const int a0 = r0[xm], a1 = r0[xCor], a2 = r0[xp], b0 = r1[xm], b2 = r1[xp], c0 = r2[xm], c1 = r2[xCor], c2 = r2[xp];
            const short dx = (short)((a2 - a0) + 2 * (b2 - b0) + (c2 - c0)), dy = (short)((c0 - a0) + 2 * (c1 - a1) + (c2 - a2));
            const float gDL = dx * dL[0] + dy * dL[1];
            const float gDO = dx * dO[0] + dy * dO[1];
            if (gDL > 0) pgdLRowSum += gDL; else ngdLRowSum -= gDL;
            if (gDO > 0) pgdORowSum += gDO; else ngdORowSum -= gDO;
            sCorX += dL[0];
            sCorY += dL[1];
        }
        const float coef = (float)P.gaussCoefG[lane];
        pgdLRowSum = coef * pgdLRowSum; ngdLRowSum = coef * ngdLRowSum;
        pgdORowSum = coef * pgdORowSum; ngdORowSum = coef * ngdORowSum;
        row[lane][0] = pgdLRowSum; row[lane][1] = ngdLRowSum; row[lane][2] = pgdLRowSum * pgdLRowSum; row[lane][3] = ngdLRowSum * ngdLRowSum;
        row[lane][4] = pgdORowSum; row[lane][5] = ngdORowSum; row[lane][6] = pgdORowSum * pgdORowSum; row[lane][7] = ngdORowSum * ngdORowSum;
    }
    __syncthreads();
    if (lane < NUM_OF_BANDS) {
        float sum[8] = {0, 0, 0, 0, 0, 0, 0, 0};
        const int h0 = max(0, (lane - 1) * WIDTH_OF_BAND), h1 = min(LSP_H, (lane + 2) * WIDTH_OF_BAND);
        for (int hID = h0; hID < h1; hID++) {
            const int own = hID / WIDTH_OF_BAND;
            float c;
            if (own == lane) c = (float)P.gaussCoefL[hID % WIDTH_OF_BAND + WIDTH_OF_BAND];
            else if (own == lane + 1) c = (float)P.gaussCoefL[hID % WIDTH_OF_BAND + 2 * WIDTH_OF_BAND];
            else c = (float)P.gaussCoefL[hID % WIDTH_OF_BAND];
            sum[0] += c * row[hID][0]; sum[1] += c * row[hID][1]; sum[2] += c * c * row[hID][2]; sum[3] += c * c * row[hID][3];
            sum[4] += c * row[hID][4]; sum[5] += c * row[hID][5]; sum[6] += c * c * row[hID][6]; sum[7] += c * c * row[hID][7];
        }
        const float invN2 = (float)(1.0 / (WIDTH_OF_BAND * 2.0)), invN3 = (float)(1.0 / (WIDTH_OF_BAND * 3.0));
        const float invN = (lane == 0 || lane == NUM_OF_BANDS - 1) ? invN2 : invN3;
        float* d = des + lane * 8;
        float temp = sum[0] * invN;
        d[0] = temp; d[4] = sqrtf(sum[2] * invN - temp * temp);
        temp = sum[1] * invN;
        d[1] = temp; d[5] = sqrtf(sum[3] * invN - temp * temp);
        temp = sum[4] * invN;
        d[2] = temp; d[6] = sqrtf(sum[6] * invN - temp * temp);
        temp = sum[5] * invN;
        d[3] = temp; d[7] = sqrtf(sum[7] * invN - temp * temp);
    }
    __syncthreads();
    if (lane == 0) {
        float tempM = 0, tempS = 0;
        for (int i = 0; i < NUM_OF_BANDS; i++) {
            const float* d = des + 8 * i;
            tempM += d[0] * d[0]; tempM += d[1] * d[1]; tempM += d[2] * d[2]; tempM += d[3] * d[3];
            tempS += d[4] * d[4]; tempS += d[5] * d[5]; tempS += d[6] * d[6]; tempS += d[7] * d[7];
        }
        tempM = 1 / sqrtf(tempM);
        tempS = 1 / sqrtf(tempS);
        for (int i = 0; i < NUM_OF_BANDS; i++) {
            float* d = des + 8 * i;
            d[0] *= tempM; d[1] *= tempM; d[2] *= tempM; d[3] *= tempM;
            d[4] *= tempS; d[5] *= tempS; d[6] *= tempS; d[7] *= tempS;
        }
        for (int i = 0; i < NUM_OF_BANDS * 8; i++) if ((double)des[i] > 0.4) des[i] = (float)0.4;
        float temp = 0;
        for (int i = 0; i < NUM_OF_BANDS * 8; i++) temp += des[i] * des[i];
        temp = 1 / sqrtf(temp);
        for (int i = 0; i < NUM_OF_BANDS * 8; i++) des[i] = des[i] * temp;
    }
    __syncthreads();
    if (lane < 32) {
        const float *f1 = &des[8 * LBD_COMB[lane][0]], *f2 = &des[8 * LBD_COMB[lane][1]];
        uint8_t result = 0;
        for (int i = 0; i < 8; i++) if (f1[i] > f2[i]) result += (uint8_t)(128 >> i);
        out_desc[((size_t)b * max_lines + li) * 32 + lane] = result;
    }
}

#ifdef PLANAR_TEST_HOOKS
__global__ __launch_bounds__(64) void debug_sort_kernel(float* key, int* idx, int n) {
    if (threadIdx.x == 0) { SortBuf s{key, idx}; std_sort_desc(s, n); }
}
#endif

}
}

using namespace planar;

struct planar_lsd {
    planar_ctx* ctx = nullptr;
    int W = 0, H = 0, max_batch = 0;
    lsd::Plan plan{};
    int detect_smem = 0;
    DevBuf d_plan, d_cx, d_cy, d_taps, d_ws, d_misc, d_lgamma;
    DevBuf d_in, d_kl, d_desc, d_eq, d_n;
    int stage_lines = 0;
    int pre_B = 0;
    int tie_order = 0;
    int top_only = 0;
    int sort_smem_g = 0, sort_smem_l = 0, sort_rows = 0, sort_rows_long = 0;
    LaunchProfile prof{4};
};

static void host_taps_q8(int ksize, double sigma, int* taps) {
    const double scale2X = -0.5 / (sigma * sigma);
    std::vector<double> v(ksize);
    double sum = 0;
    for (int i = 0; i < ksize; i++) { const double x = i - (ksize - 1) * 0.5; v[i] = std::exp(scale2X * x * x); sum += v[i]; }
    sum = 1. / sum;
    for (int i = 0; i < ksize; i++) taps[i] = (int)std::nearbyint(v[i] * sum * 256.0);
}
static bool host_exact_coefs(double inv_scale, int srcsize, int dstsize, std::vector<lsd::Coef>& out) {
    const double scale = 1.0 / inv_scale;
    out.assign(dstsize, lsd::Coef{0, 0, 0});
    if (srcsize < 2) return false;
    for (int val = 0; val < dstsize; val++) {
        const double fval = scale * ((double)val + 0.5) - 0.5;
        const int ival = (int)std::floor(fval);
        if (ival < 0) out[val] = lsd::Coef{0, 256, 0};
        else if (ival >= srcsize - 1) out[val] = lsd::Coef{srcsize - 2, 0, 256};
        else {
            out[val].ofs = ival;
            out[val].c1 = (int)std::nearbyint((fval - (double)ival) * 256.0);
            out[val].c0 = 256 - out[val].c1;
        }
    }
    return true;
}

extern "C" {

int planar_lsd_max_segments(void) { return lsd::MAX_SEGS; }

int planar_lsd_create(planar_ctx* ctx, int width, int height, int max_batch, planar_lsd** out) {
    PLANAR_REQUIRE(ctx && out, PLANAR_EINVAL, "null argument");
    *out = nullptr;
    PLANAR_REQUIRE(width >= 32 && height >= 32 && width <= 4096 && height <= 1280, PLANAR_EINVAL, "image size out of range (32..4096 x 32..1280)");
    PLANAR_REQUIRE(max_batch >= 1, PLANAR_EINVAL, "max_batch must be >= 1");
    PLANAR_HIP_CHECK(hipSetDevice(ctx->device));
    planar_lsd* o = new (std::nothrow) planar_lsd();
    PLANAR_REQUIRE(o != nullptr, PLANAR_ENOMEM, "host allocation failed");
    o->ctx = ctx; o->W = width; o->H = height; o->max_batch = max_batch;
    lsd::Plan& P = o->plan;
    const double SCALE = 0.8, SIGMA_SCALE = 0.6, QUANT = 2.0, ANG_TH = 22.5;
    P.W = width; P.H = height;
    P.w = (int)std::nearbyint(width * SCALE); P.h = (int)std::nearbyint(height * SCALE);
    P.prec = lsd::LSD_PI * ANG_TH / 180; P.p = ANG_TH / 180; P.rho = QUANT / std::sin(P.prec);
    P.density_th = 0.7; P.log_eps = 0;
    const double sigma = SIGMA_SCALE / SCALE;
    const unsigned hk = (unsigned)(std::ceil(sigma * std::sqrt(2 * 3.0 * std::log(10.0))));
    if (1 + 2 * (int)hk != 7) { delete o; set_error("planar_lsd_create: unexpected LSD Gaussian size"); return PLANAR_EINVAL; }
    host_taps_q8(7, sigma, P.taps7);
    host_taps_q8(5, 1.0, P.taps5);
    P.log_nt = 5 * (std::log10(double(P.w)) + std::log10(double(P.h))) / 2 + std::log10(11.0);
    P.min_reg_size = (int)(size_t)(-P.log_nt / std::log10(P.p));
    {
        double u = (7 * 3 - 1) / 2, sg = (7 * 2 + 1) / 2, inv = -1 / (2 * sg * sg);
        for (int i = 0; i < 21; i++) { const double dis = i - u; P.gaussCoefL[i] = std::exp(dis * dis * inv); }
        u = (9 * 7 - 1) / 2; sg = (9 * 7) / 2; inv = -1 / (2 * sg * sg);
        for (int i = 0; i < 63; i++) { const double dis = i - u; P.gaussCoefG[i] = std::exp(dis * dis * inv); }
    }
    std::vector<lsd::Coef> cx, cy;
    if (!host_exact_coefs(SCALE, width, P.w, cx) || !host_exact_coefs(SCALE, height, P.h, cy)) {
        delete o; set_error("planar_lsd_create: image too small to resample"); return PLANAR_EINVAL;
    }
    size_t off = 0;
    auto carve = [&](size_t bytes) { size_t o2 = off; off = align_up(off + bytes, (size_t)256); return o2; };
    const size_t NPf = (size_t)width * height, NPs = (size_t)P.w * P.h;
    P.off_blur7 = carve(NPf); P.off_blur5 = carve(NPf); P.off_dx = 0; P.off_dy = 0;
    
    P.off_ang = carve(NPs * 4); P.off_g2 = carve(NPs * 4); P.off_pix = carve(NPs * 16); P.off_seed = 0;
     P.off_ordr = carve(NPs * 4); P.off_gused = carve((NPs + 31) / 32 * 4 + 256); P.off_ord = carve(NPs * 4); P.off_tmp = carve(NPs * 4); P.off_reg = carve(NPs * 4 + 64);
    P.off_valid = carve((NPs + 63) / 64 * 8 + 8); P.off_sortr = carve((size_t)isort::G_FMAX * sizeof(isort::Range)); P.off_sortb = carve((size_t)isort::G_FMAX * sizeof(isort::Block)); P.off_heapj = carve((size_t)lsd::SORT_HJOBS * sizeof(isort::HeapJob));
    P.off_segs = carve((size_t)lsd::MAX_SEGS * sizeof(lsd::Seg)); P.off_kl = carve((size_t)lsd::MAX_SEGS * sizeof(planar_keyline));
    P.off_rects = carve((size_t)lsd::MAX_RECTS * sizeof(lsd::Rect)); P.off_res = carve((size_t)lsd::MAX_RECTS * sizeof(lsd::Seg)); P.off_est = carve((size_t)lsd::MAX_RECTS * 4);
    P.frame_bytes = off;
    o->detect_smem = 64 * 3 * 8 + lsd::USED_LDS_BITS / 8 + lsd::RING * 4 + 16;
    if (o->detect_smem > 150 * 1024 || NPs > (1u << 20)) { delete o; set_error("planar_lsd_create: image too large for the LDS-resident used map"); return PLANAR_EINVAL; }
    std::vector<double> lgam(NPs + 3, 0.0);
    for (size_t i = 1; i < lgam.size(); i++) {
        const double x = (double)i;
        if (x > 15.0) lgam[i] = 0.918938533204673 + (x - 0.5) * std::log(x) - x + 0.5 * x * std::log(x * std::sinh(1 / x) + 1 / (810.0 * std::pow(x, 6.0)));
        else {
            static const double q[7] = {75122.6331530, 80916.6278952, 36308.2951477, 8687.24529705, 1168.92649479, 83.8676043424, 2.50662827511};
            double a = (x + 0.5) * std::log(x + 5.5) - (x + 5.5), bsum = 0;
            for (int n = 0; n < 7; ++n) { a -= std::log(x + double(n)); bsum += q[n] * std::pow(x, double(n)); }
            lgam[i] = a + std::log(bsum);
        }
    }
    { double pp = P.p; for (int j = 0; j < 12; j++) { P.p_log[j] = std::log(pp); P.p1_log[j] = std::log(1.0 - pp); P.p_log10[j] = std::log10(pp); pp /= 2; } }
    int rc = o->d_lgamma.alloc(lgam.size() * 8);
    if (rc) { delete o; return rc; }
    P.lgamma_tab = o->d_lgamma.as<double>();
    if (hipMemcpy(o->d_lgamma.p, lgam.data(), lgam.size() * 8, hipMemcpyHostToDevice) != hipSuccess) { delete o; set_error("planar_lsd_create: table upload failed"); return PLANAR_EDEVICE; }
    rc = o->d_plan.alloc(sizeof(lsd::Plan));
    if (!rc) rc = o->d_cx.alloc(cx.size() * sizeof(lsd::Coef));
    if (!rc) rc = o->d_cy.alloc(cy.size() * sizeof(lsd::Coef));
    if (!rc) rc = o->d_taps.alloc(16 * 4);
    if (!rc) rc = o->d_ws.alloc(P.frame_bytes * (size_t)max_batch);
    if (!rc) rc = o->d_misc.alloc(sizeof(lsd::Misc) * (size_t)max_batch);
    if (rc) { delete o; return rc; }
    int taps[16] = {0};
    for (int i = 0; i < 7; i++) taps[i] = P.taps7[i];
    for (int i = 0; i < 5; i++) taps[8 + i] = P.taps5[i];
    hipError_t e = hipMemcpy(o->d_plan.p, &P, sizeof(P), hipMemcpyHostToDevice);
    if (e == hipSuccess) e = hipMemcpy(o->d_cx.p, cx.data(), cx.size() * sizeof(lsd::Coef), hipMemcpyHostToDevice);
    if (e == hipSuccess) e = hipMemcpy(o->d_cy.p, cy.data(), cy.size() * sizeof(lsd::Coef), hipMemcpyHostToDevice);
    if (e == hipSuccess) e = hipMemcpy(o->d_taps.p, taps, sizeof(taps), hipMemcpyHostToDevice);
    if (!lsd::SortGl::plan((P.w - 1) * (P.h - 1), o->sort_rows, o->sort_rows_long)) { delete o; set_error("planar_lsd_create: image too large for the sort's LDS-resident rank prefixes (about 1.1 M working pixels)"); return PLANAR_EINVAL; }
    o->sort_smem_g = lsd::SortGl::bytes(o->sort_rows);
    o->sort_smem_l = lsd::SortLds::bytes;
    if (e == hipSuccess) e = hipFuncSetAttribute((const void*)lsd::lsd_detect, hipFuncAttributeMaxDynamicSharedMemorySize, o->detect_smem);
    if (e == hipSuccess) e = hipFuncSetAttribute((const void*)lsd::lsd_sort_global, hipFuncAttributeMaxDynamicSharedMemorySize, o->sort_smem_g);
    if (e == hipSuccess) e = hipFuncSetAttribute((const void*)lsd::lsd_sort_lds, hipFuncAttributeMaxDynamicSharedMemorySize, o->sort_smem_l);
    if (e != hipSuccess) { delete o; set_error("planar_lsd_create: %s", hipGetErrorString(e)); return PLANAR_EDEVICE; }
    *out = o;
    return PLANAR_OK;
}

void planar_lsd_destroy(planar_lsd* o) { delete o; }

int planar_lsd_preprocess_dev(planar_lsd* o, const uint8_t* d_gray, int B, int pitch, int64_t frame_stride) {
    PLANAR_REQUIRE(o && d_gray, PLANAR_EINVAL, "null argument");
    PLANAR_REQUIRE(B >= 1 && B <= o->max_batch, PLANAR_EINVAL, "B out of range");
    PLANAR_REQUIRE(B <= 65535, PLANAR_EINVAL, "at most 65535 frames per call (the frame index is a grid's y / z coordinate in several launches)");
    PLANAR_REQUIRE(pitch >= o->W, PLANAR_EINVAL, "bad pitch");
    hipStream_t st = o->ctx->stream;
    const lsd::Plan& P = o->plan;
    const lsd::Plan* dP = o->d_plan.as<lsd::Plan>();
    uint8_t* ws = o->d_ws.as<uint8_t>();
    lsd::Misc* dm = o->d_misc.as<lsd::Misc>();
    PLANAR_HIP_CHECK(hipMemsetAsync(dm, 0, sizeof(lsd::Misc) * (size_t)B, st));
    const int rc = o->prof.begin();
    if (rc) return rc;
    o->prof.mark(st);
    const dim3 gfull((unsigned)(((P.W + 63) / 64) * ((P.H + 15) / 16) * B));
    if ((P.W & 3) == 0 && (pitch & 3) == 0 && (frame_stride & 3) == 0 && ((uintptr_t)d_gray & 3) == 0 && (P.off_blur7 & 3) == 0 && (P.off_blur5 & 3) == 0 && (P.frame_bytes & 3) == 0)
        hipLaunchKernelGGL(lsd::lsd_gauss75, gfull, dim3(256), 0, st, d_gray, pitch, frame_stride, P.W, P.H, o->d_taps.as<int>(), ws, P.frame_bytes, P.off_blur7, P.off_blur5, B);
    else {
        hipLaunchKernelGGL(lsd::lsd_gauss<7>, gfull, dim3(256), 0, st, d_gray, pitch, frame_stride, P.W, P.H, o->d_taps.as<int>(), ws, P.frame_bytes, P.off_blur7, B);
        hipLaunchKernelGGL(lsd::lsd_gauss<5>, gfull, dim3(256), 0, st, d_gray, pitch, frame_stride, P.W, P.H, o->d_taps.as<int>() + 8, ws, P.frame_bytes, P.off_blur5, B);
    }
    hipLaunchKernelGGL(lsd::lsd_grad, dim3((P.w + 63) / 64, (P.h + 3) / 4, B), dim3(256), 0, st, dP, o->d_cx.as<lsd::Coef>(), o->d_cy.as<lsd::Coef>(), ws, dm);
    o->prof.mark(st);
    if (o->tie_order != 0) hipLaunchKernelGGL(lsd::lsd_sort_raster, dim3(B), dim3(lsd::SORT_NT), 0, st, dP, ws, dm);
    else {
        hipLaunchKernelGGL(lsd::lsd_sort_global, dim3(B), dim3(lsd::SORT_T), o->sort_smem_g, st, dP, ws, dm, o->sort_rows, o->sort_rows_long);
        hipLaunchKernelGGL(lsd::lsd_sort_lds, dim3(B, lsd::SORT_R), dim3(lsd::SORT_LT), o->sort_smem_l, st, dP, ws, dm);
        hipLaunchKernelGGL(lsd::lsd_sort_heap, dim3(B, lsd::SORT_HY), dim3(64), lsd::SORT_HCAP * 4, st, dP, ws, dm);
        hipLaunchKernelGGL(lsd::lsd_sort_compact, dim3(B), dim3(lsd::SORT_T), 0, st, dP, ws, dm);
    }
    o->prof.mark(st);
    PLANAR_HIP_CHECK(hipGetLastError());
    o->pre_B = B;
    return PLANAR_OK;
}

int planar_lsd_detect_dev(planar_lsd* o, int B, int max_lines, planar_keyline* d_keylines, uint8_t* d_ldesc, double* d_line_eq, int32_t* d_n_lines) {
    PLANAR_REQUIRE(o && d_keylines && d_ldesc && d_line_eq && d_n_lines, PLANAR_EINVAL, "null argument");
    PLANAR_REQUIRE(B >= 1 && B == o->pre_B, PLANAR_ESTATE, "planar_lsd_preprocess_dev must have been enqueued for the same B");
    PLANAR_REQUIRE(max_lines >= 1 && max_lines <= lsd::MAX_SEGS, PLANAR_EINVAL, "bad max_lines");
    hipStream_t st = o->ctx->stream;
    const lsd::Plan* dP = o->d_plan.as<lsd::Plan>();
    uint8_t* ws = o->d_ws.as<uint8_t>();
    lsd::Misc* dm = o->d_misc.as<lsd::Misc>();
    const hipStream_t sq = o->ctx->seq_begin();
    hipLaunchKernelGGL(lsd::lsd_detect, dim3(B), dim3(64), o->detect_smem, sq, dP, ws, dm);
    const int rc = o->ctx->seq_end(sq);
    if (rc) return rc;
    o->prof.mark(st);
    if (!o->top_only) {
        hipLaunchKernelGGL(lsd::lsd_improve, dim3(128, B), dim3(64), 0, st, dP, ws, dm, -1);
        hipLaunchKernelGGL(lsd::lsd_accept, dim3(B), dim3(64), 0, st, dP, ws, dm, 0);
        hipLaunchKernelGGL(lsd::lsd_keylines, dim3(B), dim3(64), 0, st, dP, ws, dm, max_lines, d_keylines, d_line_eq, d_n_lines, -1);
    } else {
        hipLaunchKernelGGL(lsd::lsd_improve_plan, dim3(B), dim3(256), 0, st, dP, ws, dm);
        hipLaunchKernelGGL(lsd::lsd_improve, dim3(32, B), dim3(64), 0, st, dP, ws, dm, 0);
        hipLaunchKernelGGL(lsd::lsd_improve_check, dim3(B), dim3(64), 0, st, dP, ws, dm, max_lines);
        hipLaunchKernelGGL(lsd::lsd_improve, dim3(128, B), dim3(64), 0, st, dP, ws, dm, 1);
        hipLaunchKernelGGL(lsd::lsd_accept, dim3(B), dim3(64), 0, st, dP, ws, dm, 0);
        hipLaunchKernelGGL(lsd::lsd_keylines, dim3(B), dim3(64), 0, st, dP, ws, dm, max_lines, d_keylines, d_line_eq, d_n_lines, o->top_only == 2 ? 3 : 0);
        hipLaunchKernelGGL(lsd::lsd_improve, dim3(128, B), dim3(64), 0, st, dP, ws, dm, 2);
        hipLaunchKernelGGL(lsd::lsd_accept, dim3(B), dim3(64), 0, st, dP, ws, dm, 1);
        hipLaunchKernelGGL(lsd::lsd_keylines, dim3(B), dim3(64), 0, st, dP, ws, dm, max_lines, d_keylines, d_line_eq, d_n_lines, 1);
    }
    hipLaunchKernelGGL(lsd::lbd_describe, dim3(max_lines * B), dim3(64), 0, st, dP, ws, dm, max_lines, d_ldesc, B);
    o->prof.mark(st);
    PLANAR_HIP_CHECK(hipGetLastError());
    return PLANAR_OK;
}

int planar_lsd_set_profiling(planar_lsd* o, int enable) {
    PLANAR_REQUIRE(o != nullptr, PLANAR_EINVAL, "lsd is null");
    PLANAR_HIP_CHECK(hipStreamSynchronize(o->ctx->stream));
    o->prof.on = enable != 0;
    o->prof.reset();
    return PLANAR_OK;
}
int planar_lsd_get_profile(planar_lsd* o, double* total_ms , int64_t* calls) {
    PLANAR_REQUIRE(o && total_ms && calls, PLANAR_EINVAL, "null argument");
    PLANAR_HIP_CHECK(hipStreamSynchronize(o->ctx->stream));
    return o->prof.sum(total_ms, calls);
}

int planar_lsd_extract_dev(planar_lsd* o, const uint8_t* d_gray, int B, int pitch, int64_t frame_stride, int max_lines, planar_keyline* d_keylines,
                           uint8_t* d_ldesc, double* d_line_eq, int32_t* d_n_lines) {
    PLANAR_REQUIRE(o && d_gray && d_keylines && d_ldesc && d_line_eq && d_n_lines, PLANAR_EINVAL, "null argument");
    int rc = planar_lsd_preprocess_dev(o, d_gray, B, pitch, frame_stride);
    if (rc) return rc;
    return planar_lsd_detect_dev(o, B, max_lines, d_keylines, d_ldesc, d_line_eq, d_n_lines);
}

int planar_lsd_extract(planar_lsd* o, const uint8_t* gray, int B, int pitch, int64_t frame_stride, int max_lines, planar_keyline* keylines,
                       uint8_t* ldesc, double* line_eq, int32_t* n_lines) {
    PLANAR_REQUIRE(o && gray && keylines && ldesc && line_eq && n_lines, PLANAR_EINVAL, "null argument");
    PLANAR_REQUIRE(B >= 1 && B <= o->max_batch, PLANAR_EINVAL, "B out of range");
    PLANAR_REQUIRE(pitch >= o->W && frame_stride >= (int64_t)pitch * o->H, PLANAR_EINVAL, "bad pitch / frame stride");
    PLANAR_REQUIRE(max_lines >= 1 && max_lines <= lsd::MAX_SEGS, PLANAR_EINVAL, "bad max_lines");
    PLANAR_HIP_CHECK(hipSetDevice(o->ctx->device));
    hipStream_t st = o->ctx->stream;
    const size_t in_bytes = (size_t)frame_stride * B, nl = (size_t)o->max_batch * max_lines;
    if (o->d_in.bytes < in_bytes) { int rc = o->d_in.alloc(in_bytes); if (rc) return rc; }
    if (o->stage_lines < max_lines) {
        int rc = o->d_kl.alloc(nl * sizeof(planar_keyline));
        if (!rc) rc = o->d_desc.alloc(nl * 32);
        if (!rc) rc = o->d_eq.alloc(nl * 24);
        if (!rc) rc = o->d_n.alloc((size_t)o->max_batch * 4);
        if (rc) return rc;
        o->stage_lines = max_lines;
    }
    PLANAR_HIP_CHECK(hipMemcpyAsync(o->d_in.p, gray, in_bytes, hipMemcpyHostToDevice, st));
    int rc = planar_lsd_extract_dev(o, o->d_in.as<uint8_t>(), B, pitch, frame_stride, max_lines, o->d_kl.as<planar_keyline>(), o->d_desc.as<uint8_t>(),
                                    o->d_eq.as<double>(), o->d_n.as<int32_t>());
    if (rc) return rc;
    const size_t n = (size_t)B * max_lines;
    PLANAR_HIP_CHECK(hipMemcpyAsync(keylines, o->d_kl.p, n * sizeof(planar_keyline), hipMemcpyDeviceToHost, st));
    PLANAR_HIP_CHECK(hipMemcpyAsync(ldesc, o->d_desc.p, n * 32, hipMemcpyDeviceToHost, st));
    PLANAR_HIP_CHECK(hipMemcpyAsync(line_eq, o->d_eq.p, n * 24, hipMemcpyDeviceToHost, st));
    PLANAR_HIP_CHECK(hipMemcpyAsync(n_lines, o->d_n.p, (size_t)B * 4, hipMemcpyDeviceToHost, st));
    PLANAR_HIP_CHECK(hipStreamSynchronize(st));
    return planar_lsd_check(o, B);
}

int planar_lsd_check(planar_lsd* o, int B) {
    PLANAR_REQUIRE(o && B >= 1 && B <= o->max_batch, PLANAR_EINVAL, "bad argument");
    PLANAR_HIP_CHECK(hipSetDevice(o->ctx->device));
    PLANAR_HIP_CHECK(hipStreamSynchronize(o->ctx->stream));
    std::vector<lsd::Misc> m(B);
    PLANAR_HIP_CHECK(hipMemcpy(m.data(), o->d_misc.p, (size_t)B * sizeof(lsd::Misc), hipMemcpyDeviceToHost));
    for (int b = 0; b < B; b++)
        if (m[b].status != 0) {
            set_error("planar_lsd: frame %d (zero lines delivered): %s (code %d)", b, m[b].status == 1 ? "more regions / segments than the workspace holds"
                      : "the std::sort order of the gradient pixels is not reproducible (introsort depth limit / sort workspace)", m[b].status);
            return PLANAR_ECAPACITY;
        }
    return PLANAR_OK;
}

int planar_lsd_read_stage(planar_lsd* o, int frame, int stage, void* out, int64_t out_bytes) {
    PLANAR_REQUIRE(o && out, PLANAR_EINVAL, "null argument");
    PLANAR_REQUIRE(frame >= 0 && frame < o->max_batch, PLANAR_EINVAL, "frame out of range");
    PLANAR_HIP_CHECK(hipSetDevice(o->ctx->device));
    PLANAR_HIP_CHECK(hipStreamSynchronize(o->ctx->stream));
    const lsd::Plan& P = o->plan;
    const uint8_t* F = o->d_ws.as<uint8_t>() + (size_t)frame * P.frame_bytes;
    lsd::Misc m;
    PLANAR_HIP_CHECK(hipMemcpy(&m, o->d_misc.as<lsd::Misc>() + frame, sizeof(m), hipMemcpyDeviceToHost));
    const size_t NPs = (size_t)P.w * P.h;
    size_t bytes = 0, off = 0;
    int ret = 0;
    switch (stage) {
        case 0: bytes = NPs * 4; off = P.off_ang; break;
        case 1: bytes = NPs * 4; off = P.off_g2; break;
        case 2: bytes = (size_t)m.n_ord * 4; off = P.off_ord; ret = m.n_ord; break;
        case 3: bytes = (size_t)std::min(m.n_seg, lsd::MAX_SEGS) * sizeof(lsd::Seg); off = P.off_segs; ret = m.n_seg; break;
        case 4: { PLANAR_REQUIRE(out_bytes >= 4, PLANAR_EINVAL, "buffer too small"); *(int32_t*)out = m.n_regions; return PLANAR_OK; }
        case 5: {
            PLANAR_REQUIRE(out_bytes >= 56, PLANAR_EINVAL, "buffer too small");
            long long* o64 = (long long*)out;
            for (int i = 0; i < 5; i++) o64[i] = m.t[i];
            o64[5] = m.n_ord; o64[6] = m.n_grown_px;
            if (out_bytes >= 80) { o64[7] = m.t[5]; o64[8] = m.t[6]; o64[9] = m.t[7]; }
            return PLANAR_OK;
        }
        case 6: {
            PLANAR_REQUIRE(out_bytes >= 32, PLANAR_EINVAL, "buffer too small");
            long long* o64 = (long long*)out;
            o64[0] = m.imp_done; o64[1] = m.imp_redo; o64[2] = m.imp_full; o64[3] = m.n_rect;
            return PLANAR_OK;
        }
        case 7: {
            PLANAR_REQUIRE(out_bytes >= 8, PLANAR_EINVAL, "buffer too small");
            ((int32_t*)out)[0] = m.n_refine & 0xffff; ((int32_t*)out)[1] = m.n_refine >> 16;
            return PLANAR_OK;
        }
        default: set_error("planar_lsd_read_stage: unknown stage"); return PLANAR_EINVAL;
    }
    PLANAR_REQUIRE((int64_t)bytes <= out_bytes, PLANAR_EINVAL, "buffer too small");
    if (bytes) PLANAR_HIP_CHECK(hipMemcpy(out, F + off, bytes, hipMemcpyDeviceToHost));
    return ret;
}

int planar_lsd_set_top_only(planar_lsd* o, int enable) {
    PLANAR_REQUIRE(o != nullptr, PLANAR_EINVAL, "null argument");
    o->top_only = enable == 2 ? 2 : (enable != 0);
    return PLANAR_OK;
}
int planar_lsd_set_tie_order(planar_lsd* o, int tie_order) {
    PLANAR_REQUIRE(o && (tie_order == 0 || tie_order == 1), PLANAR_EINVAL, "tie_order must be 0 (libstdc++ std::sort order) or 1 (raster order)");
    o->tie_order = tie_order;
    return PLANAR_OK;
}

int planar_lsd_scaled_size(planar_lsd* o, int* w, int* h) {
    PLANAR_REQUIRE(o && w && h, PLANAR_EINVAL, "null argument");
    *w = o->plan.w; *h = o->plan.h;
    return PLANAR_OK;
}

#ifdef PLANAR_TEST_HOOKS
int planar_debug_std_sort_desc(planar_ctx* ctx, float* keys, int32_t* perm, int n) {
    PLANAR_REQUIRE(ctx && keys && perm && n >= 0 && n <= (1 << 20), PLANAR_EINVAL, "bad argument");
    PLANAR_HIP_CHECK(hipSetDevice(ctx->device));
    std::vector<int32_t> idx(n);
    for (int i = 0; i < n; i++) idx[i] = i;
    DevBuf dk, di;
    int rc = dk.alloc((size_t)n * 4);
    if (!rc) rc = di.alloc((size_t)n * 4);
    if (rc) return rc;
    PLANAR_HIP_CHECK(hipMemcpyAsync(dk.p, keys, (size_t)n * 4, hipMemcpyHostToDevice, ctx->stream));
    PLANAR_HIP_CHECK(hipMemcpyAsync(di.p, idx.data(), (size_t)n * 4, hipMemcpyHostToDevice, ctx->stream));
    hipLaunchKernelGGL(lsd::debug_sort_kernel, dim3(1), dim3(64), 0, ctx->stream, dk.as<float>(), di.as<int>(), n);
    PLANAR_HIP_CHECK(hipGetLastError());
    PLANAR_HIP_CHECK(hipMemcpyAsync(keys, dk.p, (size_t)n * 4, hipMemcpyDeviceToHost, ctx->stream));
    PLANAR_HIP_CHECK(hipMemcpyAsync(perm, di.p, (size_t)n * 4, hipMemcpyDeviceToHost, ctx->stream));
    PLANAR_HIP_CHECK(hipStreamSynchronize(ctx->stream));
    return PLANAR_OK;
}
#endif

}
```

### planarslam_amd/csrc/orb.hip

```cpp
#include <algorithm>
#include <cmath>

#include "common.h"

namespace planar {
namespace orb {

constexpr int PATCH_SIZE = 31;
constexpr int HALF_PATCH = 15;
constexpr int EDGE_THRESHOLD = 19;
constexpr int MAX_LEVELS = 16;
constexpr int CELL_W = 30;
constexpr int RADIX_BITS = 4;

struct LevelDev {
    int w, h, pitch;
    int64_t off;
    int minBX, minBY, maxBX, maxBY;
    int nCols, nRows, wCell, hCell;
    int cell_begin, ncells;
    int cand_off, cand_cap;
    int nfeat;
    int depth;
    int nIni;
    float hX;
    int code_bits;
    int kept_off, kept_cap;
    float scale;
    float patch;
    int rs_off;
};

struct CellDev {
    short level;
    short x0, y0;
    short ww, wh;
    int slot_off, slot_cap;
};

struct PlanDev {
    int nlevels, ini_th, min_th;
    int ncells_total;
    int64_t pyr_stride;
    int cand_stride;
    int kept_stride;
    int kp_cap;
    int umax[HALF_PATCH + 1];
    LevelDev lv[MAX_LEVELS];
};

__constant__ signed char c_pattern[1024] = {
#include "brief_pattern.inc"
};

__global__ __launch_bounds__(256) void orb_resize(const PlanDev* __restrict__ plan, const short4* __restrict__ tabs,
                                                  uint8_t* __restrict__ pyr, int level) {
    const LevelDev& L = plan->lv[level];
    const LevelDev& S = plan->lv[level - 1];
    const int qw = L.pitch >> 2;
    const int q = blockIdx.x * blockDim.x + threadIdx.x;
    if (q >= qw * L.h) return;
    const int dy = q / qw, dx0 = (q - dy * qw) << 2;
    uint8_t* frame = pyr + (int64_t)blockIdx.y * plan->pyr_stride;
    const uint8_t* src = frame + S.off;
    const short4* tx = tabs + L.rs_off;
    const short4 ty = tx[L.pitch + dy];
    const uint8_t* r0 = src + (int64_t)ty.x * S.pitch;
    const uint8_t* r1 = src + (int64_t)ty.y * S.pitch;
    uint32_t packed = 0;
#pragma unroll
    for (int i = 0; i < 4; i++) {
        const int dx = dx0 + i;
        uint32_t v = 0;
        if (dx < L.w) {
            const short4 t = tx[dx];
            const int h0 = r0[t.x] * t.z + r0[t.y] * t.w;
            const int h1 = r1[t.x] * t.z + r1[t.y] * t.w;
            v = (uint32_t)(((((int)ty.z * (h0 >> 4)) >> 16) + (((int)ty.w * (h1 >> 4)) >> 16) + 2) >> 2) & 0xffu;
        }
        packed |= v << (8 * i);
    }
    *(uint32_t*)(frame + L.off + (int64_t)dy * L.pitch + dx0) = packed;
}

__global__ __launch_bounds__(256) void orb_copy_level0(const PlanDev* __restrict__ plan, const uint8_t* __restrict__ gray,
                                                       int pitch, int64_t frame_stride, uint8_t* __restrict__ pyr) {
    const LevelDev& L = plan->lv[0];
    const int qw = L.pitch >> 2;
    const int q = blockIdx.x * blockDim.x + threadIdx.x;
    if (q >= qw * L.h) return;
    const int y = q / qw, x0 = (q - y * qw) << 2;
    const uint8_t* s = gray + (int64_t)blockIdx.y * frame_stride + (int64_t)y * pitch;
    uint32_t packed = 0;
#pragma unroll
    for (int i = 0; i < 4; i++)
        if (x0 + i < L.w) packed |= (uint32_t)s[x0 + i] << (8 * i);
    *(uint32_t*)(pyr + (int64_t)blockIdx.y * plan->pyr_stride + L.off + (int64_t)y * L.pitch + x0) = packed;
}

__device__ __forceinline__ bool has9(uint32_t m16) {
    uint32_t m = m16 | (m16 << 16);
    uint32_t a = m & (m >> 1);
    a &= a >> 2;
    a &= a >> 4;
    a &= m >> 8;
    return (a & 0xffffu) != 0;
}

__device__ __forceinline__ bool fast_quick(const uint8_t* c, int stride, int min_th) {
    const int v = c[0];
    const int a0 = v - c[3 * stride], a8 = v - c[-3 * stride], a4 = v - c[3], a12 = v - c[-3];
    const bool dark = (a0 > min_th || a8 > min_th) && (a4 > min_th || a12 > min_th);
    const bool bright = (a0 < -min_th || a8 < -min_th) && (a4 < -min_th || a12 < -min_th);
    return dark || bright;
}
__device__ __forceinline__ void fast_ring(const uint8_t* c, int stride, int d[16]) {
    const int v = c[0];
    d[0] = v - c[3 * stride];       d[1] = v - c[3 * stride + 1];   d[2] = v - c[2 * stride + 2];   d[3] = v - c[stride + 3];
    d[4] = v - c[3];                d[5] = v - c[-stride + 3];      d[6] = v - c[-2 * stride + 2];  d[7] = v - c[-3 * stride + 1];
    d[8] = v - c[-3 * stride];      d[9] = v - c[-3 * stride - 1];  d[10] = v - c[-2 * stride - 2]; d[11] = v - c[-stride - 3];
    d[12] = v - c[-3];              d[13] = v - c[stride - 3];      d[14] = v - c[2 * stride - 2];  d[15] = v - c[3 * stride - 1];
}
__device__ __forceinline__ bool fast_is_corner(const uint8_t* c, int stride, int min_th) {
    int d[16];
    fast_ring(c, stride, d);
    uint32_t dark = 0, bright = 0;
#pragma unroll
    for (int k = 0; k < 16; k++) {
        dark |= (uint32_t)(d[k] > min_th) << k;
        bright |= (uint32_t)(d[k] < -min_th) << k;
    }
    return has9(dark) || has9(bright);
}
__device__ __forceinline__ int fast_corner_score(const uint8_t* c, int stride) {
    int d[16];
    fast_ring(c, stride, d);
    int lo2[16], hi2[16], lo4[16], hi4[16];
#pragma unroll
    for (int k = 0; k < 16; k++) { lo2[k] = min(d[k], d[(k + 1) & 15]); hi2[k] = max(d[k], d[(k + 1) & 15]); }
#pragma unroll
    for (int k = 0; k < 16; k++) { lo4[k] = min(lo2[k], lo2[(k + 2) & 15]); hi4[k] = max(hi2[k], hi2[(k + 2) & 15]); }
    int best_dark = -256, best_bright = -256;
#pragma unroll
    for (int k = 0; k < 16; k++) {
        const int lo9 = min(min(lo4[k], lo4[(k + 4) & 15]), d[(k + 8) & 15]);
        const int hi9 = max(max(hi4[k], hi4[(k + 4) & 15]), d[(k + 8) & 15]);
        best_dark = max(best_dark, lo9);
        best_bright = max(best_bright, -hi9);
    }
    return max(best_dark, best_bright) - 1;
}

__global__ __launch_bounds__(256) void orb_fast_cells(const PlanDev* __restrict__ plan, const CellDev* __restrict__ cells,
                                                      const uint8_t* __restrict__ pyr, uint32_t* __restrict__ cand,
                                                      int* __restrict__ cell_count, int* __restrict__ dropped, int B) {
    extern __shared__ __attribute__((aligned(16))) uint8_t smem[];
    __shared__ int s_any_ini, s_cnt;
    int frame, cell;
    xcd_frame_block(plan->ncells_total, B, frame, cell);
    const CellDev C = cells[cell];
    const LevelDev& L = plan->lv[C.level];
    const int tid = threadIdx.x, lane = tid & 63, wave = tid >> 6;
    const int ww = C.ww, wh = C.wh;
    int* out_count = cell_count + (int64_t)frame * plan->ncells_total + cell;
    if (ww <= 0 || wh <= 0) { if (tid == 0) *out_count = 0; return; }
    const int tw = ww + 6, th = wh + 6;
    const int gx0 = C.x0 - 3, mis = gx0 & 3, nd = (mis + tw + 3) >> 2;
    const int tstride = nd * 4;
    const int sw = ww + 2, sh = wh + 2;
    uint8_t* tile = smem;
    uint8_t* score = smem + ((tstride * th + 15) & ~15);
    const uint8_t* img = pyr + (int64_t)frame * plan->pyr_stride + L.off;
    {
        const int q = tid & 15;
        if (q < nd)
            for (int y = tid >> 4; y < th; y += 16)
                *(uint32_t*)(tile + y * tstride + 4 * q) = *(const uint32_t*)(img + (int64_t)(C.y0 - 3 + y) * L.pitch + (gx0 - mis) + 4 * q);
    }
    for (int i = tid; i < sw * sh; i += 256) score[i] = 0;
    if (tid == 0) { s_any_ini = 0; s_cnt = 0; }
    __syncthreads();
    const int min_th = plan->min_th, ini_th = plan->ini_th;
    const int npx = ww * wh;
    const float inv_ww = 1.0f / (float)ww;
    auto row_of = [&](int p_) { return (int)(((float)p_ + 0.5f) * inv_ww); };
    unsigned short* list = (unsigned short*)(score + ((sw * sh + 15) & ~15));
    auto compact = [&](bool keep, int value, int& count) {
        const unsigned long long m = __ballot(keep);
        int base = 0;
        if (lane == 0 && m) base = atomicAdd(&s_cnt, __popcll(m));
        base = __builtin_amdgcn_readfirstlane(base);
        if (keep) list[base + __popcll(m & ((1ull << lane) - 1ull))] = (unsigned short)value;
        (void)count;
    };
    int dummy = 0;
    for (int p0 = 0; p0 < npx; p0 += 256) {
        const int p = p0 + tid;
        bool k1 = false;
        if (p < npx) { const int y = row_of(p), x = p - y * ww; k1 = fast_quick(tile + (y + 3) * tstride + (x + 3 + mis), tstride, min_th); }
        compact(k1, p, dummy);
    }
    __syncthreads();
    const int n1 = s_cnt;
    __syncthreads();
    if (tid == 0) s_cnt = 0;
    __syncthreads();
    for (int i0 = 0; i0 < n1; i0 += 256) {
        const int i = i0 + tid;
        int p = 0;
        bool k2 = false;
        if (i < n1) { p = list[i]; const int y = row_of(p), x = p - y * ww; k2 = fast_is_corner(tile + (y + 3) * tstride + (x + 3 + mis), tstride, min_th); }
        __syncthreads();
        compact(k2, p, dummy);
        __syncthreads();
    }
    const int n2 = s_cnt;
    for (int i = tid; i < n2; i += 256) {
        const int p = list[i];
        const int y = row_of(p), x = p - y * ww;
        score[(y + 1) * sw + (x + 1)] = (uint8_t)fast_corner_score(tile + (y + 3) * tstride + (x + 3 + mis), tstride);
    }
    __syncthreads();
    __shared__ unsigned s_keep[128];
    __shared__ unsigned short s_kpre[128];
    for (int i = tid; i < 128; i += 256) s_keep[i] = 0u;
    __syncthreads();
    int any = 0;
    bool ismax[4] = {false, false, false, false};
    for (int i = tid, k = 0; i < n2; i += 256, k++) {
        const int p = list[i];
        const int y = row_of(p), x = p - y * ww;
        const uint8_t* sc = score + (y + 1) * sw + (x + 1);
        const int s = sc[0];
        const bool mx = s > sc[-1] && s > sc[1] && s > sc[-sw - 1] && s > sc[-sw] && s > sc[-sw + 1] && s > sc[sw - 1] && s > sc[sw] && s > sc[sw + 1];
        if (k < 4) ismax[k] = mx;
        if (mx && s >= ini_th) any = 1;
    }
    if (__any(any) && lane == 0) s_any_ini = 1;
    __syncthreads();
    const int th_cell = s_any_ini ? ini_th : min_th;
    for (int i = tid, k = 0; i < n2; i += 256, k++) {
        const int p = list[i];
        const int y = row_of(p), x = p - y * ww;
        const uint8_t* sc = score + (y + 1) * sw + (x + 1);
        const int s = sc[0];
        const bool mx = k < 4 ? ismax[k] : (s > sc[-1] && s > sc[1] && s > sc[-sw - 1] && s > sc[-sw] && s > sc[-sw + 1] && s > sc[sw - 1] && s > sc[sw] && s > sc[sw + 1]);
        if (mx && s >= th_cell) atomicOr(&s_keep[p >> 5], 1u << (p & 31));
    }
    __syncthreads();
    if (wave == 0) {
// ... 181 lines not shown
    };
    auto push_front = [&](int s) {
        if (lane == 0) { n_prev[s] = -1; n_next[s] = head; if (head >= 0) n_prev[head] = s; }
        if (head < 0) tail = s;
        head = s; count++;
    };
    auto push_back = [&](int s) {
        if (lane == 0) { n_next[s] = -1; n_prev[s] = tail; if (tail >= 0) n_next[tail] = s; }
        if (tail < 0) head = s;
        tail = s; count++;
    };
    auto erase = [&](int s) -> int {
        __threadfence_block();
        const int p = n_prev[s], n = n_next[s];
        if (lane == 0) { if (p >= 0) n_next[p] = n; if (n >= 0) n_prev[n] = p; freel[nfree] = s; }
        if (p < 0) head = n;
        if (n < 0) tail = p;
        nfree++; count--;
        return n;
    };

    {
        const int ini_shift = 2 * L.depth;
        int lo = 0;
        for (int i = 0; i < L.nIni; i++) {
            int a = lo, b = K;
            while (b - a > 0) {
                const int mid = (a + b) >> 1;
                if ((int)(S[mid] >> (32 + ini_shift)) > i) b = mid; else a = mid + 1;
            }
            const int hi = a;
            if (hi > lo) { const int s = alloc_node(lo, hi, 0); __threadfence_block(); push_back(s); }
            lo = hi;
        }
    }
    __threadfence_block();

    int* c_size = e_size0; int* c_seq = e_seq0; int* c_slot = e_slot0; int c_n = 0;
    int* p_size = e_size1; int* p_seq = e_seq1; int* p_slot = e_slot1; int p_n = 0;

    auto split = [&](int s) -> int {
        __threadfence_block();
        const int lo = n_lo[s], hi = n_hi[s], depth = n_depth[s];
        const int shift = 2 * (L.depth - 1 - depth);
        int b1, b2, b3;
        const int n = hi - lo;
        if (n <= 256) {
            int c0 = 0, c1 = 0, c2 = 0;
            for (int i0 = 0; i0 < n; i0 += 64) {
                const int idx = lo + i0 + lane;
                const int dg = idx < hi ? digit_at(S, idx, shift) : 4;
                c0 += __popcll(__ballot(dg == 0)); c1 += __popcll(__ballot(dg == 1)); c2 += __popcll(__ballot(dg == 2));
            }
            b1 = lo + c0; b2 = b1 + c1; b3 = b2 + c2;
        } else {
            b1 = wave_lower_bound(S, lo, hi, shift, 1, lane);
            b2 = wave_lower_bound(S, b1, hi, shift, 2, lane);
            b3 = wave_lower_bound(S, b2, hi, shift, 3, lane);
        }
        const int bl[5] = {lo, b1, b2, b3, hi};
        int nexp = 0;
#pragma unroll
        for (int q = 0; q < 4; q++) {
            const int sz = bl[q + 1] - bl[q];
            if (sz <= 0) continue;
            const int myseq = seq_ctr;
            const int c = alloc_node(bl[q], bl[q + 1], depth + 1);
            __threadfence_block();
            push_front(c);
            if (sz > 1) {
                if (lane == 0) { c_size[c_n] = sz; c_seq[c_n] = myseq; c_slot[c_n] = c; }
                c_n++;
                nexp++;
            }
        }
        __threadfence_block();
        return nexp;
    };

    bool finish = false;
    while (!finish) {
        const int prevSize = count;
        int nToExpand = 0;
        c_n = 0;
        int it = head;
        while (it >= 0) {
            __threadfence_block();
            const int sz = n_hi[it] - n_lo[it];
            if (sz == 1) { it = n_next[it]; continue; }
            nToExpand += split(it);
            it = erase(it);
        }
        if (count >= N || count == prevSize) {
            finish = true;
        } else if (count + nToExpand * 3 > N) {
            while (!finish) {
                const int prevSize2 = count;
                { int* t; t = c_size; c_size = p_size; p_size = t; t = c_seq; c_seq = p_seq; p_seq = t; t = c_slot; c_slot = p_slot; p_slot = t; }
                p_n = c_n; c_n = 0;
                __threadfence_block();
                for (int step = 0; step < p_n; step++) {
                    unsigned long long best = 0;
                    for (int i = lane; i < p_n; i += 64) {
                        const int sz = p_size[i];
                        if (sz > 0) {
                            const unsigned long long v = ((unsigned long long)sz << 40) | ((unsigned long long)p_seq[i] << 16) | (unsigned)i;
                            best = v > best ? v : best;
                        }
                    }
#pragma unroll
                    for (int o = 32; o > 0; o >>= 1) { const unsigned long long t = __shfl_xor(best, o); best = t > best ? t : best; }
                    const int idx = (int)(best & 0xffffu);
                    const int slot = p_slot[idx];
                    if (lane == 0) p_size[idx] = 0;
                    __threadfence_block();
                    split(slot);
                    erase(slot);
                    if (count >= N) break;
                }
                if (count >= N || count == prevSize2) finish = true;
            }
        }
    }

    __threadfence_block();
    int pos = 0;
    const int cw = L.wCell, ch = L.hCell, ncols = L.nCols;
    for (int it = head; it >= 0; it = n_next[it], pos++) {
        const int lo = n_lo[it], hi = n_hi[it];
        unsigned long long best = 0;
        for (int i = lo + lane; i < hi; i += 64) {
            const uint32_t key = (uint32_t)S[i];
            const unsigned x = key & 0xfffu, y = (key >> 12) & 0xfffu, sc = key >> 24;
            const unsigned cell = ((y - 3) / ch) * ncols + (x - 3) / cw;
            const unsigned long long ord = ((unsigned long long)cell << 24) | (y << 12) | x;
            const unsigned long long v = ((unsigned long long)sc << 48) | ((~ord) & 0xffffffffffffull);
            best = v > best ? v : best;
        }
#pragma unroll
        for (int o = 32; o > 0; o >>= 1) { const unsigned long long t = __shfl_xor(best, o); best = t > best ? t : best; }
        if (lane == 0) {
            const unsigned long long ord = (~best) & 0xffffffffffffull;
            out[pos] = (uint32_t)(ord & 0xffffffu) | ((uint32_t)(best >> 48) << 24);
        }
    }
    if (lane == 0) *out_count = pos;
}

struct TileDev { short level, tx, ty, pad; };

__global__ __launch_bounds__(256) void orb_blur(const PlanDev* __restrict__ plan, const TileDev* __restrict__ tiles,
                                                const uint8_t* __restrict__ pyr, uint8_t* __restrict__ blur, int n_tiles, int B) {
    __shared__ uint32_t s_pw[22][19];
    __shared__ __attribute__((aligned(8))) uint16_t s_h[22][68];
    int frame, tile;
    xcd_frame_block(n_tiles, B, frame, tile);
    const TileDev T = tiles[tile];
    const LevelDev& L = plan->lv[T.level];
    const int tid = threadIdx.x;
    const int x0 = T.tx * 64, y0 = T.ty * 16;
    const uint8_t* img = pyr + (int64_t)frame * plan->pyr_stride + L.off;
    for (int i = tid; i < 22 * 18; i += 256) {
        const int r = i / 18, wq = i - r * 18;
        int y = y0 + r - 3;
        y = y < 0 ? -y : y; y = y >= L.h ? 2 * L.h - 2 - y : y; y = max(0, min(y, L.h - 1));
        const uint8_t* row = img + (int64_t)y * L.pitch;
        const int xs = x0 - 4 + 4 * wq;
        uint32_t w;
        if (xs >= 0 && xs + 3 < L.w) w = *(const uint32_t*)(row + xs);
        else {
            w = 0;
#pragma unroll
            for (int k = 0; k < 4; k++) {
                int x = xs + k;
                x = x < 0 ? -x : x; x = x >= L.w ? 2 * L.w - 2 - x : x; x = max(0, min(x, L.w - 1));
                w |= (uint32_t)row[x] << (8 * k);
            }
        }
        s_pw[r][wq] = w;
    }
    __syncthreads();
    for (int i = tid; i < 22 * 16; i += 256) {
        const int r = i >> 4, q = i & 15;
        const uint32_t w0 = s_pw[r][q], w1 = s_pw[r][q + 1], w2 = s_pw[r][q + 2];
        uint32_t b[10];
        b[0] = (w0 >> 8) & 255u; b[1] = (w0 >> 16) & 255u; b[2] = w0 >> 24;
        b[3] = w1 & 255u; b[4] = (w1 >> 8) & 255u; b[5] = (w1 >> 16) & 255u; b[6] = w1 >> 24;
        b[7] = w2 & 255u; b[8] = (w2 >> 8) & 255u; b[9] = (w2 >> 16) & 255u;
        uint32_t o[4];
#pragma unroll
        for (int j = 0; j < 4; j++) {
            const uint32_t v = 18u * (b[j] + b[j + 6]) + 34u * (b[j + 1] + b[j + 5]) + 49u * (b[j + 2] + b[j + 4]) + 55u * b[j + 3];
            o[j] = min(v, 65535u);
        }
        *(uint2*)&s_h[r][4 * q] = make_uint2(o[0] | (o[1] << 16), o[2] | (o[3] << 16));
    }
    __syncthreads();
    {
        const int c4 = (tid & 15) * 4, r = tid >> 4;
        uint32_t acc[4] = {0, 0, 0, 0};
        const uint32_t taps[7] = {18u, 34u, 49u, 55u, 49u, 34u, 18u};
#pragma unroll
        for (int k = 0; k < 7; k++) {
            const uint2 v = *(const uint2*)&s_h[r + k][c4];
            acc[0] += taps[k] * (v.x & 0xffffu); acc[1] += taps[k] * (v.x >> 16);
            acc[2] += taps[k] * (v.y & 0xffffu); acc[3] += taps[k] * (v.y >> 16);
        }
        uint32_t packed = 0;
#pragma unroll
        for (int i = 0; i < 4; i++) packed |= min((acc[i] + 32768u) >> 16, 255u) << (8 * i);
        const int y = y0 + r, x = x0 + c4;
        if (y < L.h && x < L.pitch)
            *(uint32_t*)(blur + (int64_t)frame * plan->pyr_stride + L.off + (int64_t)y * L.pitch + x) = packed;
    }
}

__device__ __forceinline__ float fast_atan2_deg(float y, float x) {
    const float scale = (float)(180 / 3.1415926535897932384626433832795);
    const float p1 = 0.9997878412794807f * scale, p3 = -0.3258083974640975f * scale;
    const float p5 = 0.1555786518463281f * scale, p7 = -0.04432655554792128f * scale;
    const float ax = fabsf(x), ay = fabsf(y);
    float a, c, c2;
    if (ax >= ay) {
        c = __fdiv_rn(ay, __fadd_rn(ax, 2.220446049250313e-16f));
        c2 = __fmul_rn(c, c);
        a = __fmul_rn(__fadd_rn(__fmul_rn(__fadd_rn(__fmul_rn(__fadd_rn(__fmul_rn(p7, c2), p5), c2), p3), c2), p1), c);
    } else {
        c = __fdiv_rn(ax, __fadd_rn(ay, 2.220446049250313e-16f));
        c2 = __fmul_rn(c, c);
        a = __fsub_rn(90.f, __fmul_rn(__fadd_rn(__fmul_rn(__fadd_rn(__fmul_rn(__fadd_rn(__fmul_rn(p7, c2), p5), c2), p3), c2), p1), c));
    }
    if (x < 0) a = __fsub_rn(180.f, a);
    if (y < 0) a = __fsub_rn(360.f, a);
    return a;
}

__global__ __launch_bounds__(256) void orb_describe(const PlanDev* __restrict__ plan, const uint8_t* __restrict__ pyr,
                                                    const uint8_t* __restrict__ blur, const uint32_t* __restrict__ kept,
                                                    const int* __restrict__ kept_count, planar_keypoint* __restrict__ kps,
                                                    uint8_t* __restrict__ desc, int32_t* __restrict__ n_out, int per_frame, int B) {
    int frame, bx;
    xcd_frame_block(per_frame, B, frame, bx);
    const int sub = threadIdx.x & 15;
    const int kpi = bx * 16 + (threadIdx.x >> 4);
    int level = -1, first = 0, total = 0;
    for (int l = 0; l < plan->nlevels; l++) {
        const int c = kept_count[frame * MAX_LEVELS + l];
        if (level < 0 && kpi < total + c) { level = l; first = total; }
        total += c;
    }
    if (bx == 0 && threadIdx.x == 0) n_out[frame] = total;
    if (level < 0) return;
    const LevelDev& L = plan->lv[level];
    const uint32_t key = kept[(int64_t)frame * plan->kept_stride + L.kept_off + (kpi - first)];
    const int x = (int)(key & 0xfffu) + L.minBX, y = (int)((key >> 12) & 0xfffu) + L.minBY;
    const int score = (int)(key >> 24);
    const int64_t lvl_off = (int64_t)frame * plan->pyr_stride + L.off;

    const uint8_t* c = pyr + lvl_off + (int64_t)y * L.pitch + x;
    int m10 = 0, m01 = 0;
    if (sub == 0) {
        for (int u = -HALF_PATCH; u <= HALF_PATCH; ++u) m10 += u * c[u];
    } else {
        const int d = plan->umax[sub];
        int vsum = 0;
        const uint8_t* cp = c + (int64_t)sub * L.pitch;
        const uint8_t* cm = c - (int64_t)sub * L.pitch;
        for (int u = -d; u <= d; ++u) {
            const int vp = cp[u], vm = cm[u];
            vsum += vp - vm;
            m10 += u * (vp + vm);
        }
        m01 = sub * vsum;
    }
#pragma unroll
    for (int o = 8; o > 0; o >>= 1) { m10 += __shfl_xor(m10, o); m01 += __shfl_xor(m01, o); }
    const float angle = fast_atan2_deg((float)m01, (float)m10);

    const float factorPI = (float)(3.1415926535897932384626433832795 / 180.f);
    const float ang = __fmul_rn(angle, factorPI);
    const float a = (float)cos((double)ang), b = (float)sin((double)ang);
    const uint8_t* bc = blur + lvl_off + (int64_t)y * L.pitch + x;
    const int step = L.pitch;
    uint32_t bits = 0;
    const signed char* pat = c_pattern + sub * 64;
#pragma unroll
    for (int i = 0; i < 16; i++) {
        const float x0 = (float)pat[4 * i], y0 = (float)pat[4 * i + 1], x1 = (float)pat[4 * i + 2], y1 = (float)pat[4 * i + 3];
        const int r0 = __float2int_rn(__fadd_rn(__fmul_rn(x0, b), __fmul_rn(y0, a)));
        const int q0 = __float2int_rn(__fsub_rn(__fmul_rn(x0, a), __fmul_rn(y0, b)));
        const int r1 = __float2int_rn(__fadd_rn(__fmul_rn(x1, b), __fmul_rn(y1, a)));
        const int q1 = __float2int_rn(__fsub_rn(__fmul_rn(x1, a), __fmul_rn(y1, b)));
        const int t0 = bc[r0 * step + q0], t1 = bc[r1 * step + q1];
        bits |= (uint32_t)(t0 < t1) << i;
    }
    const int64_t o = (int64_t)frame * plan->kp_cap + kpi;
    *(uint16_t*)(desc + o * 32 + sub * 2) = (uint16_t)bits;
    if (sub == 0) {
        planar_keypoint kp;
        kp.x = __fmul_rn((float)x, L.scale);
        kp.y = __fmul_rn((float)y, L.scale);
        kp.size = L.patch;
        kp.angle = angle;
        kp.response = (float)score;
        kp.octave = level;
        kp.class_id = -1;
        kps[o] = kp;
    }
}

}
}

using namespace planar;
using namespace planar::orb;

struct planar_orb {
    planar_ctx* ctx = nullptr;
    planar_orb_params params{};
    int W = 0, H = 0, max_batch = 0;
    PlanDev plan{};
    std::vector<CellDev> cells;
    std::vector<TileDev> tiles;
    std::vector<float> scale, inv_scale, sigma2, inv_sigma2;
    int fast_smem = 0, node_cap = 0, oct_smem = 0;
    int last_B = 0;
    DevBuf d_plan, d_cells, d_tiles, d_tabs, d_pyr, d_blur, d_cand, d_cell_count, d_sortA, d_sortB, d_level_count,
        d_kept, d_kept_count, d_dropped;
    DevBuf d_in, d_kps, d_desc, d_nout;
    std::vector<const char*> launch_names;
    LaunchProfile prof;
    explicit planar_orb(int nlevels) : prof(nlevels + 5) {}
};

static inline int cv_round_f(float v) { return (int)nearbyintf(v); }
static inline int cv_round_d(double v) { return (int)nearbyint(v); }
static inline short sat_short(float v) { int i = cv_round_f(v); return (short)std::min(32767, std::max(-32768, i)); }

extern "C" {

int planar_orb_create(planar_ctx* ctx, const planar_orb_params* p, int W, int H, int max_batch, planar_orb** out) {
    PLANAR_REQUIRE(ctx && p && out, PLANAR_EINVAL, "null argument");
    *out = nullptr;
    PLANAR_REQUIRE(p->nlevels >= 1 && p->nlevels <= MAX_LEVELS, PLANAR_EINVAL, "nlevels must be in [1,16]");
    PLANAR_REQUIRE(p->nfeatures >= 1 && p->nfeatures <= 60000, PLANAR_EINVAL, "nfeatures out of range");
    PLANAR_REQUIRE(p->scale_factor > 1.0f, PLANAR_EINVAL, "scale_factor must be > 1");
    PLANAR_REQUIRE(p->min_th_fast >= 1 && p->ini_th_fast >= p->min_th_fast && p->ini_th_fast <= 254, PLANAR_EINVAL,
                   "FAST thresholds must satisfy 1 <= min <= ini <= 254");
    PLANAR_REQUIRE(W >= 64 && H >= 64 && W <= 4096 && H <= 4096, PLANAR_EINVAL, "image size must be within [64,4096]");
    PLANAR_REQUIRE(max_batch >= 1, PLANAR_EINVAL, "max_batch must be >= 1");
    PLANAR_HIP_CHECK(hipSetDevice(ctx->device));

    planar_orb* o = new (std::nothrow) planar_orb(p->nlevels);
    PLANAR_REQUIRE(o != nullptr, PLANAR_ENOMEM, "host allocation failed");
    o->ctx = ctx; o->params = *p; o->W = W; o->H = H; o->max_batch = max_batch;
    const int nl = p->nlevels;
    const double scaleFactor = p->scale_factor;
    o->scale.resize(nl); o->sigma2.resize(nl); o->inv_scale.resize(nl); o->inv_sigma2.resize(nl);
    o->scale[0] = 1.0f; o->sigma2[0] = 1.0f;
    for (int i = 1; i < nl; i++) { o->scale[i] = (float)(o->scale[i - 1] * scaleFactor); o->sigma2[i] = o->scale[i] * o->scale[i]; }
    for (int i = 0; i < nl; i++) { o->inv_scale[i] = 1.0f / o->scale[i]; o->inv_sigma2[i] = 1.0f / o->sigma2[i]; }
    std::vector<int> nfeat(nl);
    {
        float factor = (float)(1.0f / scaleFactor);
        float nDesired = p->nfeatures * (1 - factor) / (1 - (float)std::pow((double)factor, (double)nl));
        int sum = 0;
        for (int l = 0; l < nl - 1; l++) { nfeat[l] = cv_round_f(nDesired); sum += nfeat[l]; nDesired *= factor; }
        nfeat[nl - 1] = std::max(p->nfeatures - sum, 0);
    }
    PlanDev& P = o->plan;
    memset(&P, 0, sizeof(P));
    {
        int v, v0, vmax = (int)std::floor(HALF_PATCH * std::sqrt(2.f) / 2 + 1);
        int vmin = (int)std::ceil(HALF_PATCH * std::sqrt(2.f) / 2);
        const double hp2 = HALF_PATCH * HALF_PATCH;
        for (v = 0; v <= vmax; ++v) P.umax[v] = cv_round_d(std::sqrt(hp2 - v * v));
        for (v = HALF_PATCH, v0 = 0; v >= vmin; --v) { while (P.umax[v0] == P.umax[v0 + 1]) ++v0; P.umax[v] = v0; ++v0; }
    }
    P.nlevels = nl; P.ini_th = p->ini_th_fast; P.min_th = p->min_th_fast;

    int64_t pyr_off = 0;
    int cand_off = 0, kept_off = 0, rs_off = 0;
    int max_tile_bytes = 0, max_nfeat = 0;
    std::vector<short4> tabs;
    for (int l = 0; l < nl; l++) {
        LevelDev& L = P.lv[l];
        L.w = cv_round_f((float)W * o->inv_scale[l]);
        L.h = cv_round_f((float)H * o->inv_scale[l]);
        L.minBX = L.minBY = EDGE_THRESHOLD - 3;
        L.maxBX = L.w - EDGE_THRESHOLD + 3; L.maxBY = L.h - EDGE_THRESHOLD + 3;
        const float width = (float)(L.maxBX - L.minBX), height = (float)(L.maxBY - L.minBY);
        L.nCols = (int)(width / CELL_W); L.nRows = (int)(height / CELL_W);
        if (L.nCols < 1 || L.nRows < 1 || L.w < 2 * EDGE_THRESHOLD + 8 || L.h < 2 * EDGE_THRESHOLD + 8) {
            delete o;
            set_error("planar_orb_create: pyramid level %d (%dx%d) is too small for the 30-px FAST cell grid", l, L.w, L.h);
            return PLANAR_EINVAL;
        }
        L.wCell = (int)std::ceil(width / L.nCols); L.hCell = (int)std::ceil(height / L.nRows);
        L.pitch = align_up(L.w, 16);
        L.off = pyr_off;
        pyr_off += align_up((int64_t)L.pitch * L.h, (int64_t)256);
        L.nfeat = nfeat[l];
        max_nfeat = std::max(max_nfeat, nfeat[l]);
        L.scale = o->scale[l];
        L.patch = (float)(int)(PATCH_SIZE * o->scale[l]);
        L.nIni = (int)std::round((float)(L.maxBX - L.minBX) / (L.maxBY - L.minBY));
        if (L.nIni < 1 || L.nIni > 64) {
            delete o;
            set_error("planar_orb_create: level %d aspect ratio gives %d initial octree nodes (supported: 1..64)", l, L.nIni);
            return PLANAR_EINVAL;
        }
        L.hX = (float)(L.maxBX - L.minBX) / L.nIni;
        int ext = std::max(L.maxBX - L.minBX, L.maxBY - L.minBY), D = 1;
        while ((1 << (D - 1)) < ext) D++;
        L.depth = D;
        int ini_bits = 0; while ((1 << ini_bits) < L.nIni) ini_bits++;
        L.code_bits = align_up(2 * D + ini_bits, RADIX_BITS);
        if (L.code_bits > 32) { delete o; set_error("planar_orb_create: path code needs %d bits", L.code_bits); return PLANAR_EINVAL; }
        L.cell_begin = (int)o->cells.size();
        L.cand_off = cand_off;
        for (int i = 0; i < L.nRows; i++) {
            const float iniY = (float)(L.minBY + i * L.hCell);
            float maxY = iniY + L.hCell + 6;
            if (iniY >= L.maxBY - 3) continue;
            if (maxY > L.maxBY) maxY = (float)L.maxBY;
            for (int j = 0; j < L.nCols; j++) {
                const float iniX = (float)(L.minBX + j * L.wCell);
                float maxX = iniX + L.wCell + 6;
                if (iniX >= L.maxBX - 6) continue;
                if (maxX > L.maxBX) maxX = (float)L.maxBX;
                CellDev C;
                C.level = (short)l;
                C.x0 = (short)((int)iniX + 3); C.y0 = (short)((int)iniY + 3);
                C.ww = (short)((int)maxX - 3 - C.x0); C.wh = (short)((int)maxY - 3 - C.y0);
                if (C.ww <= 0 || C.wh <= 0) continue;
                C.slot_off = cand_off;
                C.slot_cap = ((C.ww + 1) / 2) * ((C.wh + 1) / 2);
                cand_off += C.slot_cap;
                o->cells.push_back(C);
                const int tstride = ((((int)C.x0 - 3) & 3) + C.ww + 6 + 3) & ~3;
                if (tstride > 64 || C.ww * C.wh >= 4096) { delete o; set_error("planar_orb_create: FAST cell of %d x %d pixels at level %d is larger than the kernel's tile", (int)C.ww, (int)C.wh, l); return PLANAR_EINVAL; }
                const int bytes = ((tstride * (C.wh + 6) + 15) & ~15) + (((C.ww + 2) * (C.wh + 2) + 15) & ~15) + 2 * C.ww * C.wh;
                max_tile_bytes = std::max(max_tile_bytes, bytes);
            }
        }
        L.ncells = (int)o->cells.size() - L.cell_begin;
        L.cand_cap = cand_off - L.cand_off;
        L.kept_off = kept_off;
        L.kept_cap = std::max(L.nfeat + 4, 4 * L.nIni + 4);
        kept_off += L.kept_cap;
        L.rs_off = rs_off;
        if (l > 0) {
            const LevelDev& S = P.lv[l - 1];
            const double sx_scale = 1. / ((double)L.w / S.w), sy_scale = 1. / ((double)L.h / S.h);
            std::vector<short4> tx(L.pitch), ty(L.h);
            for (int dx = 0; dx < L.pitch; dx++) {
                if (dx >= L.w) { tx[dx] = make_short4(0, 0, 0, 0); continue; }
                float fx = (float)((dx + 0.5) * sx_scale - 0.5);
                int sx = (int)std::floor(fx);
                fx -= sx;
                if (sx < 0) { fx = 0; sx = 0; }
                if (sx >= S.w - 1) { fx = 0; sx = S.w - 1; }
                tx[dx] = make_short4((short)sx, (short)std::min(sx + 1, S.w - 1), sat_short((1.f - fx) * 2048), sat_short(fx * 2048));
            }
            for (int dy = 0; dy < L.h; dy++) {
                float fy = (float)((dy + 0.5) * sy_scale - 0.5);
                int sy = (int)std::floor(fy);
                fy -= sy;
                ty[dy] = make_short4((short)std::min(std::max(sy, 0), S.h - 1), (short)std::min(std::max(sy + 1, 0), S.h - 1),
                                     sat_short((1.f - fy) * 2048), sat_short(fy * 2048));
            }
            tabs.insert(tabs.end(), tx.begin(), tx.end());
            tabs.insert(tabs.end(), ty.begin(), ty.end());
            rs_off += L.pitch + L.h;
        }
        for (int ty_ = 0; ty_ < (L.h + 15) / 16; ty_++)
            for (int tx_ = 0; tx_ < (L.w + 63) / 64; tx_++) o->tiles.push_back(TileDev{(short)l, (short)tx_, (short)ty_, 0});
    }
    P.ncells_total = (int)o->cells.size();
    P.pyr_stride = pyr_off;
    P.cand_stride = cand_off;
    P.kept_stride = kept_off;
    P.kp_cap = kept_off;
    o->fast_smem = max_tile_bytes;
    o->node_cap = std::max(max_nfeat + 8, 4 * 64 + 8);
    o->oct_smem = 13 * o->node_cap * (int)sizeof(int);
    if (o->oct_smem > 160 * 1024 || o->fast_smem > 64 * 1024) {
        delete o; set_error("planar_orb_create: LDS budget exceeded (octree %d B, FAST tile %d B)", o->oct_smem, o->fast_smem);
        return PLANAR_EINVAL;
    }

    int rc = PLANAR_OK;
    const size_t B = (size_t)max_batch;
    if ((rc = o->d_plan.alloc(sizeof(PlanDev))) || (rc = o->d_cells.alloc(o->cells.size() * sizeof(CellDev))) ||
        (rc = o->d_tiles.alloc(o->tiles.size() * sizeof(TileDev))) || (rc = o->d_tabs.alloc(std::max<size_t>(tabs.size(), 1) * sizeof(short4))) ||
        (rc = o->d_pyr.alloc(B * P.pyr_stride)) || (rc = o->d_blur.alloc(B * P.pyr_stride)) ||
        (rc = o->d_cand.alloc(B * P.cand_stride * sizeof(uint32_t))) || (rc = o->d_cell_count.alloc(B * P.ncells_total * sizeof(int))) ||
        (rc = o->d_sortA.alloc(B * P.cand_stride * sizeof(uint64_t))) || (rc = o->d_sortB.alloc(B * P.cand_stride * sizeof(uint64_t))) ||
        (rc = o->d_level_count.alloc(B * MAX_LEVELS * sizeof(int))) || (rc = o->d_kept.alloc(B * P.kept_stride * sizeof(uint32_t))) ||
        (rc = o->d_kept_count.alloc(B * MAX_LEVELS * sizeof(int))) || (rc = o->d_dropped.alloc(64))) {
        delete o;
        return rc;
    }
    hipError_t e = hipMemcpy(o->d_plan.p, &P, sizeof(P), hipMemcpyHostToDevice);
    if (e == hipSuccess) e = hipMemset(o->d_dropped.p, 0, 64);
    if (e == hipSuccess) e = hipMemcpy(o->d_cells.p, o->cells.data(), o->cells.size() * sizeof(CellDev), hipMemcpyHostToDevice);
    if (e == hipSuccess) e = hipMemcpy(o->d_tiles.p, o->tiles.data(), o->tiles.size() * sizeof(TileDev), hipMemcpyHostToDevice);
    if (e == hipSuccess && !tabs.empty()) e = hipMemcpy(o->d_tabs.p, tabs.data(), tabs.size() * sizeof(short4), hipMemcpyHostToDevice);
    if (e == hipSuccess && o->oct_smem > 64 * 1024)
        e = hipFuncSetAttribute((const void*)orb_octree, hipFuncAttributeMaxDynamicSharedMemorySize, o->oct_smem);
    if (e != hipSuccess) { delete o; set_error("planar_orb_create: upload failed: %s", hipGetErrorString(e)); return PLANAR_EDEVICE; }
    o->launch_names.push_back("orb_copy_level0");
    for (int l = 1; l < nl; l++) o->launch_names.push_back("orb_resize");
    for (const char* n : {"orb_fast_cells", "orb_sort", "orb_octree", "orb_blur", "orb_describe"}) o->launch_names.push_back(n);
    *out = o;
    return PLANAR_OK;
}

void planar_orb_destroy(planar_orb* o) { delete o; }

int planar_orb_set_profiling(planar_orb* o, int enable) {
    PLANAR_REQUIRE(o != nullptr, PLANAR_EINVAL, "orb is null");
    PLANAR_HIP_CHECK(hipStreamSynchronize(o->ctx->stream));
    o->prof.on = enable != 0;
    o->prof.reset();
    return PLANAR_OK;
}

int planar_orb_profile_num_launches(const planar_orb* o) { return o ? (int)o->launch_names.size() : PLANAR_EINVAL; }

const char* planar_orb_profile_launch_name(const planar_orb* o, int i) {
    return (o && i >= 0 && i < (int)o->launch_names.size()) ? o->launch_names[i] : nullptr;
}

int planar_orb_get_profile(planar_orb* o, double* total_ms, int64_t* calls) {
    PLANAR_REQUIRE(o && total_ms && calls, PLANAR_EINVAL, "null argument");
    PLANAR_HIP_CHECK(hipStreamSynchronize(o->ctx->stream));
    return o->prof.sum(total_ms, calls);
}

int planar_orb_max_keypoints(const planar_orb* o) { return o ? o->plan.kp_cap : PLANAR_EINVAL; }

int planar_orb_get_scale_factors(const planar_orb* o, float* s, float* is, float* s2, float* is2) {
    PLANAR_REQUIRE(o != nullptr, PLANAR_EINVAL, "orb is null");
    const int n = o->params.nlevels;
    if (s) memcpy(s, o->scale.data(), n * sizeof(float));
    if (is) memcpy(is, o->inv_scale.data(), n * sizeof(float));
    if (s2) memcpy(s2, o->sigma2.data(), n * sizeof(float));
    if (is2) memcpy(is2, o->inv_sigma2.data(), n * sizeof(float));
    return PLANAR_OK;
}

int planar_orb_level_size(const planar_orb* o, int level, int* w, int* h) {
    PLANAR_REQUIRE(o && w && h, PLANAR_EINVAL, "null argument");
    PLANAR_REQUIRE(level >= 0 && level < o->params.nlevels, PLANAR_EINVAL, "level out of range");
    *w = o->plan.lv[level].w; *h = o->plan.lv[level].h;
    return PLANAR_OK;
}

int planar_orb_features_per_level(const planar_orb* o, int32_t* out) {
    PLANAR_REQUIRE(o && out, PLANAR_EINVAL, "null argument");
    for (int l = 0; l < o->params.nlevels; l++) out[l] = o->plan.lv[l].nfeat;
    return PLANAR_OK;
}

int planar_orb_extract_dev(planar_orb* o, const uint8_t* d_gray, int B, int pitch, int64_t frame_stride,
                           planar_keypoint* d_kps, uint8_t* d_desc, int32_t* d_n_out) {
    PLANAR_REQUIRE(o && d_gray && d_kps && d_desc && d_n_out, PLANAR_EINVAL, "null argument");
    PLANAR_REQUIRE(B >= 1 && B <= o->max_batch, PLANAR_EINVAL, "B must be in [1, max_batch]");
    PLANAR_REQUIRE(pitch >= o->W && frame_stride >= (int64_t)pitch * o->H, PLANAR_EINVAL, "pitch/frame_stride too small");
    hipStream_t st = o->ctx->stream;
    const PlanDev& P = o->plan;
    const PlanDev* dp = o->d_plan.as<PlanDev>();
    uint8_t* pyr = o->d_pyr.as<uint8_t>();
    const int rc = o->prof.begin();
    if (rc) return rc;
    auto mark = [&]() { o->prof.mark(st); };
    mark();
    {
        const int n = (P.lv[0].pitch / 4) * P.lv[0].h;
        hipLaunchKernelGGL(orb_copy_level0, dim3((n + 255) / 256, B), dim3(256), 0, st, dp, d_gray, pitch, frame_stride, pyr);
        mark();
    }
    for (int l = 1; l < P.nlevels; l++) {
        const int n = (P.lv[l].pitch / 4) * P.lv[l].h;
        hipLaunchKernelGGL(orb_resize, dim3((n + 255) / 256, B), dim3(256), 0, st, dp, o->d_tabs.as<short4>(), pyr, l);
        mark();
    }
    hipLaunchKernelGGL(orb_fast_cells, dim3(P.ncells_total * B), dim3(256), o->fast_smem, st, dp, o->d_cells.as<CellDev>(), pyr,
                       o->d_cand.as<uint32_t>(), o->d_cell_count.as<int>(), o->d_dropped.as<int>(), B);
    mark();
    hipLaunchKernelGGL(orb_sort, dim3(P.nlevels, B), dim3(256), 0, st, dp, o->d_cells.as<CellDev>(), o->d_cand.as<uint32_t>(),
                       o->d_cell_count.as<int>(), o->d_sortA.as<uint64_t>(), o->d_sortB.as<uint64_t>(), o->d_level_count.as<int>());
    mark();
    hipLaunchKernelGGL(orb_octree, dim3(P.nlevels, B), dim3(64), o->oct_smem, st, dp, o->d_sortA.as<uint64_t>(), o->d_sortB.as<uint64_t>(),
                       o->d_level_count.as<int>(), o->d_kept.as<uint32_t>(), o->d_kept_count.as<int>(), o->node_cap);
    mark();
    hipLaunchKernelGGL(orb_blur, dim3((unsigned)o->tiles.size() * B), dim3(256), 0, st, dp, o->d_tiles.as<TileDev>(), pyr, o->d_blur.as<uint8_t>(), (int)o->tiles.size(), B);
    mark();
    hipLaunchKernelGGL(orb_describe, dim3((P.kp_cap + 15) / 16 * B), dim3(256), 0, st, dp, pyr, o->d_blur.as<uint8_t>(), o->d_kept.as<uint32_t>(),
                       o->d_kept_count.as<int>(), d_kps, d_desc, d_n_out, (P.kp_cap + 15) / 16, B);
    mark();
    PLANAR_HIP_CHECK(hipGetLastError());
    o->last_B = B;
    return PLANAR_OK;
}

int planar_orb_check(planar_orb* o) {
    PLANAR_REQUIRE(o != nullptr, PLANAR_EINVAL, "orb is null");
    int dropped = 0;
    PLANAR_HIP_CHECK(hipMemcpyAsync(&dropped, o->d_dropped.p, 4, hipMemcpyDeviceToHost, o->ctx->stream));
    PLANAR_HIP_CHECK(hipStreamSynchronize(o->ctx->stream));
    if (dropped != 0) {
        (void)hipMemsetAsync(o->d_dropped.p, 0, 4, o->ctx->stream);
        set_error("planar_orb: %d FAST candidates did not fit their cell's slot array", dropped);
        return PLANAR_ECAPACITY;
    }
    return PLANAR_OK;
}

int planar_orb_extract(planar_orb* o, const uint8_t* gray, int B, int pitch, int64_t frame_stride, planar_keypoint* kps,
                       uint8_t* desc, int32_t* n_out) {
    PLANAR_REQUIRE(o && gray && kps && desc && n_out, PLANAR_EINVAL, "null argument");
    PLANAR_REQUIRE(B >= 1 && B <= o->max_batch, PLANAR_EINVAL, "B must be in [1, max_batch]");
    PLANAR_REQUIRE(pitch >= o->W && frame_stride >= (int64_t)pitch * o->H, PLANAR_EINVAL, "pitch/frame_stride too small");
    PLANAR_HIP_CHECK(hipSetDevice(o->ctx->device));
    const size_t in_bytes = (size_t)frame_stride * (B - 1) + (size_t)pitch * o->H;
    const size_t cap = (size_t)o->plan.kp_cap;
    int rc;
    if (o->d_in.bytes < in_bytes && (rc = o->d_in.alloc(in_bytes))) return rc;
    if (o->d_kps.bytes < (size_t)o->max_batch * cap * sizeof(planar_keypoint)) {
        if ((rc = o->d_kps.alloc((size_t)o->max_batch * cap * sizeof(planar_keypoint)))) return rc;
        if ((rc = o->d_desc.alloc((size_t)o->max_batch * cap * 32))) return rc;
        if ((rc = o->d_nout.alloc((size_t)o->max_batch * sizeof(int32_t)))) return rc;
    }
    hipStream_t st = o->ctx->stream;
    PLANAR_HIP_CHECK(hipMemcpyAsync(o->d_in.p, gray, in_bytes, hipMemcpyHostToDevice, st));
    if ((rc = planar_orb_extract_dev(o, o->d_in.as<uint8_t>(), B, pitch, frame_stride, o->d_kps.as<planar_keypoint>(),
                                     o->d_desc.as<uint8_t>(), o->d_nout.as<int32_t>())))
        return rc;
    PLANAR_HIP_CHECK(hipMemcpyAsync(kps, o->d_kps.p, (size_t)B * cap * sizeof(planar_keypoint), hipMemcpyDeviceToHost, st));
    PLANAR_HIP_CHECK(hipMemcpyAsync(desc, o->d_desc.p, (size_t)B * cap * 32, hipMemcpyDeviceToHost, st));
    PLANAR_HIP_CHECK(hipMemcpyAsync(n_out, o->d_nout.p, (size_t)B * sizeof(int32_t), hipMemcpyDeviceToHost, st));
    return planar_orb_check(o);
}

static int read_plane(planar_orb* o, const DevBuf& buf, int frame, int level, uint8_t* out) {
    PLANAR_REQUIRE(o && out, PLANAR_EINVAL, "null argument");
    PLANAR_REQUIRE(frame >= 0 && frame < o->last_B, PLANAR_ESTATE, "frame not part of the last extract call");
    PLANAR_REQUIRE(level >= 0 && level < o->params.nlevels, PLANAR_EINVAL, "level out of range");
    const LevelDev& L = o->plan.lv[level];
    PLANAR_HIP_CHECK(hipStreamSynchronize(o->ctx->stream));
    PLANAR_HIP_CHECK(hipMemcpy2D(out, L.w, buf.as<uint8_t>() + (int64_t)frame * o->plan.pyr_stride + L.off, L.pitch, L.w, L.h,
                                 hipMemcpyDeviceToHost));
    return PLANAR_OK;
}

int planar_orb_read_level(planar_orb* o, int frame, int level, uint8_t* out) { return read_plane(o, o->d_pyr, frame, level, out); }
int planar_orb_read_blurred(planar_orb* o, int frame, int level, uint8_t* out) { return read_plane(o, o->d_blur, frame, level, out); }

int planar_orb_read_candidates(planar_orb* o, int frame, int level, int32_t* out, int cap) {
    PLANAR_REQUIRE(o && out, PLANAR_EINVAL, "null argument");
    PLANAR_REQUIRE(frame >= 0 && frame < o->last_B, PLANAR_ESTATE, "frame not part of the last extract call");
    PLANAR_REQUIRE(level >= 0 && level < o->params.nlevels, PLANAR_EINVAL, "level out of range");
    const LevelDev& L = o->plan.lv[level];
    PLANAR_HIP_CHECK(hipStreamSynchronize(o->ctx->stream));
    std::vector<int> counts(L.ncells);
    std::vector<uint32_t> slots(L.cand_cap);
    PLANAR_HIP_CHECK(hipMemcpy(counts.data(), o->d_cell_count.as<int>() + (int64_t)frame * o->plan.ncells_total + L.cell_begin,
                               L.ncells * sizeof(int), hipMemcpyDeviceToHost));
    PLANAR_HIP_CHECK(hipMemcpy(slots.data(), o->d_cand.as<uint32_t>() + (int64_t)frame * o->plan.cand_stride + L.cand_off,
                               (size_t)L.cand_cap * sizeof(uint32_t), hipMemcpyDeviceToHost));
    int n = 0;
    for (int c = 0; c < L.ncells; c++) {
        const CellDev& C = o->cells[L.cell_begin + c];
        for (int i = 0; i < counts[c]; i++, n++) {
            if (n >= cap) { set_error("planar_orb_read_candidates: capacity %d too small", cap); return PLANAR_ECAPACITY; }
            const uint32_t k = slots[C.slot_off - L.cand_off + i];
            out[3 * n] = (int)(k & 0xfffu); out[3 * n + 1] = (int)((k >> 12) & 0xfffu); out[3 * n + 2] = (int)(k >> 24);
        }
    }
    return n;
}

}
```

### planarslam_amd/lines.py

```python
from __future__ import annotations

import ctypes as C

import numpy as np

from ._lib import KEYLINE_DTYPE, Context, check, lib

SEG_DTYPE = np.dtype([("x1", "<f4"), ("y1", "<f4"), ("x2", "<f4"), ("y2", "<f4"), ("width", "<f8"), ("p", "<f8"), ("nfa", "<f8")])


class LineSegment:
    def __init__(self, width: int = 640, height: int = 480, max_batch: int = 1, ctx: Context | None = None, tie_order: int = 0, top_only: bool = False):
        self.ctx = ctx or Context(0)
        self.W, self.H, self.max_batch = width, height, max_batch
        h = C.c_void_p()
        check(lib().planar_lsd_create(self.ctx.h, width, height, max_batch, C.byref(h)))
        self.h = h
        w_, h_ = C.c_int(), C.c_int()
        check(lib().planar_lsd_scaled_size(self.h, C.byref(w_), C.byref(h_)))
        self.scaled = (w_.value, h_.value)
        check(lib().planar_lsd_set_tie_order(self.h, tie_order))
        self.tie_order = tie_order
        check(lib().planar_lsd_set_top_only(self.h, int(top_only)))
        self.top_only = top_only

    def ExtractLineSegment(self, img, lsdNFeatures: int = 40):
        img = np.ascontiguousarray(img, np.uint8)
        if img.ndim == 2:
            img = img[None]
        B, H, W = img.shape
        assert (H, W) == (self.H, self.W) and B <= self.max_batch
        kl = np.zeros((B, lsdNFeatures), KEYLINE_DTYPE)
        desc = np.zeros((B, lsdNFeatures, 32), np.uint8)
        eq = np.zeros((B, lsdNFeatures, 3), np.float64)
        n = np.zeros(B, np.int32)
        check(lib().planar_lsd_extract(self.h, img.ctypes.data, B, W, W * H, lsdNFeatures, kl.ctypes.data, desc.ctypes.data, eq.ctypes.data,
                                       n.ctypes.data))
        return kl, desc, eq, n

    def read_stage(self, frame: int, stage: int):
        w, h = self.scaled
        if stage in (0, 1):
            out = np.zeros((h, w), np.float32 if stage == 0 else np.uint32)
        elif stage == 2:
            out = np.zeros(w * h, np.int32)
        elif stage == 3:
            out = np.zeros(lib().planar_lsd_max_segments(), SEG_DTYPE)
        elif stage == 5:
            out = np.zeros(10, np.int64)
        elif stage == 6:
            out = np.zeros(4, np.int64)
        elif stage == 7:
            out = np.zeros(2, np.int32)
        else:
            out = np.zeros(1, np.int32)
        r = check(lib().planar_lsd_read_stage(self.h, frame, stage, out.ctypes.data, out.nbytes))
        return out[:min(r, len(out))] if stage in (2, 3) else out

    def close(self):
        if getattr(self, "h", None):
            lib().planar_lsd_destroy(self.h)
            self.h = None

    def __del__(self):
        try:
            self.close()
        except Exception:
            pass


def is_line_good(keylines, n_lines, depth, seeds, cam=(535.4, 539.2, 320.1, 247.6), depth_factor=1.0 / 5000.0, ctx: Context | None = None):
    import ctypes as C

    from ._lib import KEYLINE_DTYPE
    L = lib()
    ctx = ctx or Context(0)
    kl = np.ascontiguousarray(keylines, KEYLINE_DTYPE)
    B, S = kl.shape
    d = np.ascontiguousarray(depth, np.uint16)
    H, W = d.shape[1:]
    nl = np.ascontiguousarray(n_lines, np.int32); sd = np.ascontiguousarray(seeds, np.uint32)
    out = dict(depth_line=np.zeros((B, S), np.float32), lines3d=np.zeros((B, S, 6)), good=np.zeros((B, S), np.uint8), direction=np.zeros((B, S, 3)),
               n_inliers=np.zeros((B, S), np.int32), packed_dirs=np.zeros((B, S, 3)), n_good=np.zeros(B, np.int32))
    check(L.planar_is_line_good(ctx.h, B, kl.ctypes.data, nl.ctypes.data, S, d.ctypes.data, W, H, W, W * H, np.float32(depth_factor), cam[0], cam[1], cam[2], cam[3],
                                sd.ctypes.data, *[out[k].ctypes.data for k in ("depth_line", "lines3d", "good", "direction", "n_inliers", "packed_dirs", "n_good")]))
    return out
```

Baseline: 12670.

## Use packed dot-product blurs, trig lookup table, and fused ORB pyramid kernel

```diff
diff --git a/include/planar_abi.h b/include/planar_abi.h
--- a/include/planar_abi.h
+++ b/include/planar_abi.h
@@ -369,6 +369,7 @@
 int planar_lsd_detect_dev(planar_lsd* lsd, int B, int max_lines, planar_keyline* d_keylines, uint8_t* d_ldesc, double* d_line_eq, int32_t* d_n_lines);
 int planar_lsd_check(planar_lsd* lsd, int B);
 int planar_lsd_read_stage(planar_lsd* lsd, int frame, int stage, void* out, int64_t out_bytes);
+int planar_lsd_trig_table(float* out, int64_t out_floats);
 int planar_lsd_set_profiling(planar_lsd* lsd, int enable);
 int planar_lsd_get_profile(planar_lsd* lsd, double* total_ms, int64_t* calls);
 #ifdef PLANAR_TEST_HOOKS
diff --git a/planarslam_amd/_lib.py b/planarslam_amd/_lib.py
--- a/planarslam_amd/_lib.py
+++ b/planarslam_amd/_lib.py
@@ -202,6 +202,7 @@
     "planar_lsd_detect_dev": (C.c_int, [C.c_void_p, C.c_int, C.c_int, C.c_void_p, C.c_void_p, C.c_void_p, C.c_void_p]),
     "planar_lsd_check": (C.c_int, [C.c_void_p, C.c_int]),
     "planar_lsd_read_stage": (C.c_int, [C.c_void_p, C.c_int, C.c_int, C.c_void_p, C.c_int64]),
+    "planar_lsd_trig_table": (C.c_int, [C.c_void_p, C.c_int64]),
     "planar_debug_std_sort_desc": (C.c_int, [C.c_void_p, C.c_void_p, C.c_void_p, C.c_int]),
     "planar_peac_create": (C.c_int, [C.c_void_p, C.c_int, C.c_int, C.c_int, C.POINTER(C.c_void_p)]),
     "planar_peac_destroy": (None, [C.c_void_p]),
diff --git a/planarslam_amd/csrc/common.h b/planarslam_amd/csrc/common.h
--- a/planarslam_amd/csrc/common.h
+++ b/planarslam_amd/csrc/common.h
@@ -103,13 +103,14 @@
 };
 
 struct LaunchProfile {
-    const int slots;
+    int slots;
     bool on = false;
     bool open = false;
     std::vector<hipEvent_t> ev;
     std::vector<int> marked;
     size_t used = 0;
     explicit LaunchProfile(int nslots) : slots(nslots) {}
+    void set_slots(int nslots) { if (ev.empty()) slots = nslots; }
     LaunchProfile(const LaunchProfile&) = delete;
     ~LaunchProfile() { for (hipEvent_t e : ev) (void)hipEventDestroy(e); }
     void reset() { used = 0; open = false; }
@@ -163,6 +164,13 @@
     if (n < full) { const int g = n / group, r = n - g * group; frame = g * 8 + (r & 7); blk = r >> 3; }
     else { const int r = n - full; frame = (B & ~7) + r / per_frame; blk = r - (r / per_frame) * per_frame; }
 }
+
+typedef unsigned short planar_u16x2 __attribute__((ext_vector_type(2)));
+__device__ __forceinline__ uint32_t udot4_u8(uint32_t a, uint32_t b, uint32_t acc) { return __builtin_amdgcn_udot4(a, b, acc, false); }
+__device__ __forceinline__ uint32_t udot2_u16(uint32_t a, uint32_t b, uint32_t acc) {
+    return __builtin_amdgcn_udot2(__builtin_bit_cast(planar_u16x2, a), __builtin_bit_cast(planar_u16x2, b), acc, false);
+}
+__device__ __forceinline__ uint32_t byte_window(uint32_t hi, uint32_t lo, uint32_t shift) { return __builtin_amdgcn_alignbyte(hi, lo, shift); }
 #endif
 
 }
@@ -172,6 +180,7 @@
     hipStream_t own_stream = nullptr;
     hipStream_t stream = nullptr;
     planar::DevBuf scratch;
+    planar::DevBuf lsd_trig;
     hipStream_t seq_stream = nullptr;
     hipEvent_t seq_fork = nullptr, seq_join = nullptr;
     hipStream_t seq_begin() {
diff --git a/planarslam_amd/csrc/lsd.hip b/planarslam_amd/csrc/lsd.hip
--- a/planarslam_amd/csrc/lsd.hip
+++ b/planarslam_amd/csrc/lsd.hip
@@ -16,6 +16,7 @@
 constexpr int MAX_SEGS = 2048;
 constexpr int MAX_RECTS = 4096;
 constexpr int RING = 512;
+constexpr int TRIG_N = 511;
 constexpr int USED_LDS_BITS = 32768;
 
 struct Plan {
@@ -25,13 +26,15 @@
     int min_reg_size;
     size_t off_blur7, off_blur5, off_dx, off_dy, off_ang, off_g2, off_pix, off_seed, off_ord, off_ordr, off_gused, off_tmp, off_reg, off_valid, off_sortr, off_sortb, off_heapj, off_segs, off_kl, off_rects, off_res, off_est, frame_bytes;
     const double* lgamma_tab;
+    const float2* trig_tab;
+    int g2_rho;
     double p_log[12], p1_log[12], p_log10[12];
     double gaussCoefL[21], gaussCoefG[63];
 };
 
 struct Misc { uint32_t g2max; int n_ord; int n_seg; int n_kl; int status; int n_regions; int n_grown_px; int n_rect; long long t[8]; int sort_counts[2]; int heap_n; int sort_kv; int sort_prefix; int n_refine; float imp_T; int imp_done; int imp_redo; int imp_full; };
 
-__device__ __forceinline__ float fast_atan2_deg(float y, float x) {
+__host__ __device__ __forceinline__ float fast_atan2_deg(float y, float x) {
     const float scale = (float)(180 / 3.1415926535897932384626433832795);
     const float p1 = 0.9997878412794807f * scale, p3 = -0.3258083974640975f * scale;
     const float p5 = 0.1555786518463281f * scale, p7 = -0.04432655554792128f * scale;
@@ -88,7 +91,7 @@
     }
 }
 
-__global__ __launch_bounds__(256) void lsd_gauss75(const uint8_t* __restrict__ src, int pitch, int64_t src_stride, int W, int H, const int* __restrict__ taps_g,
+__global__ __launch_bounds__(256) void lsd_gauss75_wide(const uint8_t* __restrict__ src, int pitch, int64_t src_stride, int W, int H, const int* __restrict__ taps_g,
                                                    uint8_t* __restrict__ ws, size_t frame_bytes, size_t off7, size_t off5, int B) {
     constexpr int TW = 64, TH = 16, R = 3, NR = TH + 2 * R, NWD = TW / 4 + 2;
     __shared__ uint32_t s_in[NR][NWD + 1];
@@ -156,6 +159,77 @@
     }
 }
 
+__global__ __launch_bounds__(256) void lsd_gauss75(const uint8_t* __restrict__ src, int pitch, int64_t src_stride, int W, int H, const int* __restrict__ taps_g,
+                                                   uint8_t* __restrict__ ws, size_t frame_bytes, size_t off7, size_t off5, int B) {
+    constexpr int TW = 64, TH = 16, R = 3, NR = TH + 2 * R, NWD = TW / 4 + 2, NP = NR / 2;
+    __shared__ uint32_t s_in[NR][NWD + 1];
+    __shared__ __attribute__((aligned(16))) uint32_t s_h7[NP][TW + 4], s_h5[NP][TW + 4];
+    uint32_t t7[7], t5[5];
+    for (int i = 0; i < 7; i++) t7[i] = (uint32_t)taps_g[i];
+    for (int i = 0; i < 5; i++) t5[i] = (uint32_t)taps_g[8 + i];
+    const int tiles_x = (W + TW - 1) / TW, tiles_y = (H + TH - 1) / TH, tid = threadIdx.x;
+    int b, tile;
+    xcd_frame_block(tiles_x * tiles_y, B, b, tile);
+    const int x0 = (tile % tiles_x) * TW, y0 = (tile / tiles_x) * TH;
+    const uint8_t* S = src + (int64_t)b * src_stride;
+    for (int i = tid; i < NR * NWD; i += 256) {
+        const int r = i / NWD, wq = i - r * NWD;
+        const uint8_t* row = S + (int64_t)reflect101(y0 + r - R, H) * pitch;
+        const int xb = x0 - 4 + 4 * wq;
+        uint32_t v;
+        if (xb >= 0 && xb + 3 < W) v = *(const uint32_t*)(row + xb);
+        else v = (uint32_t)row[reflect101(xb, W)] | ((uint32_t)row[reflect101(xb + 1, W)] << 8) | ((uint32_t)row[reflect101(xb + 2, W)] << 16) | ((uint32_t)row[reflect101(xb + 3, W)] << 24);
+        s_in[r][wq] = v;
+    }
+    __syncthreads();
+    if (tid < NP * (TW / 4)) {
+        const int p = tid / (TW / 4), q = tid - p * (TW / 4);
+        const uint32_t k7lo = t7[0] | (t7[1] << 8) | (t7[2] << 16) | (t7[3] << 24), k7hi = t7[4] | (t7[5] << 8) | (t7[6] << 16);
+        const uint32_t k5lo = (t5[0] << 8) | (t5[1] << 16) | (t5[2] << 24), k5hi = t5[3] | (t5[4] << 8);
+        uint32_t h7[2][4], h5[2][4];
+#pragma unroll
+        for (int e = 0; e < 2; e++) {
+            const uint32_t w0 = s_in[2 * p + e][q], w1 = s_in[2 * p + e][q + 1], w2 = s_in[2 * p + e][q + 2];
+#pragma unroll
+            for (int o = 0; o < 4; o++) {
+                const uint32_t lo = o == 3 ? w1 : byte_window(w1, w0, o + 1), hi = o == 3 ? w2 : byte_window(w2, w1, o + 1);
+                h7[e][o] = min(udot4_u8(hi, k7hi, udot4_u8(lo, k7lo, 0u)), 65535u);
+                h5[e][o] = min(udot4_u8(hi, k5hi, udot4_u8(lo, k5lo, 0u)), 65535u);
+            }
+        }
+        *(uint4*)&s_h7[p][4 * q] = make_uint4(h7[0][0] | (h7[1][0] << 16), h7[0][1] | (h7[1][1] << 16), h7[0][2] | (h7[1][2] << 16), h7[0][3] | (h7[1][3] << 16));
+        *(uint4*)&s_h5[p][4 * q] = make_uint4(h5[0][0] | (h5[1][0] << 16), h5[0][1] | (h5[1][1] << 16), h5[0][2] | (h5[1][2] << 16), h5[0][3] | (h5[1][3] << 16));
+    }
+    __syncthreads();
+    {
+        const int r = tid >> 4, q = tid & 15;
+        const int x = x0 + 4 * q, y = y0 + r;
+        if (x < W && y < H) {
+            const bool odd = r & 1;
+            const uint32_t k7[4] = {odd ? t7[0] << 16 : t7[0] | (t7[1] << 16), odd ? t7[1] | (t7[2] << 16) : t7[2] | (t7[3] << 16),
+                                    odd ? t7[3] | (t7[4] << 16) : t7[4] | (t7[5] << 16), odd ? t7[5] | (t7[6] << 16) : t7[6]};
+            const uint32_t k5[3] = {odd ? t5[0] | (t5[1] << 16) : t5[0] << 16, odd ? t5[2] | (t5[3] << 16) : t5[1] | (t5[2] << 16), odd ? t5[4] : t5[3] | (t5[4] << 16)};
+            uint32_t a[4] = {0, 0, 0, 0}, c[4] = {0, 0, 0, 0};
+#pragma unroll
+            for (int k = 0; k < 4; k++) {
+                const uint4 v = *(const uint4*)&s_h7[(r >> 1) + k][4 * q];
+                a[0] = udot2_u16(v.x, k7[k], a[0]); a[1] = udot2_u16(v.y, k7[k], a[1]); a[2] = udot2_u16(v.z, k7[k], a[2]); a[3] = udot2_u16(v.w, k7[k], a[3]);
+            }
+#pragma unroll
+            for (int k = 0; k < 3; k++) {
+                const uint4 v = *(const uint4*)&s_h5[((r + 1) >> 1) + k][4 * q];
+                c[0] = udot2_u16(v.x, k5[k], c[0]); c[1] = udot2_u16(v.y, k5[k], c[1]); c[2] = udot2_u16(v.z, k5[k], c[2]); c[3] = udot2_u16(v.w, k5[k], c[3]);
+            }
+            uint32_t o7 = 0, o5 = 0;
+#pragma unroll
+            for (int o = 0; o < 4; o++) { o7 |= min((a[o] + 32768u) >> 16, 255u) << (8 * o); o5 |= min((c[o] + 32768u) >> 16, 255u) << (8 * o); }
+            uint8_t* F = ws + (size_t)b * frame_bytes;
+            *(uint32_t*)(F + off7 + (size_t)y * W + x) = o7;
+            *(uint32_t*)(F + off5 + (size_t)y * W + x) = o5;
+        }
+    }
+}
+
 struct Coef { int ofs, c0, c1; };
 
 __device__ __forceinline__ int scaled_px(const uint8_t* __restrict__ B7, int W, const Coef& cx, const Coef& cy) {
@@ -199,15 +273,13 @@
     const int DA = s11 - s00, BC = s10 - s01;
     const int gx = DA + BC, gy = DA - BC;
     const int g2 = gx * gx + gy * gy;
-    const double norm = sqrt(g2 / 4.0);
     g2a[o] = (uint32_t)g2;
-    if (norm <= P.rho) { ang[o] = NOTDEF_F; pix4[o] = make_float4(NOTDEF_F, 0.f, 0.f, 0.f); }
+    if (g2 <= P.g2_rho) { ang[o] = NOTDEF_F; pix4[o] = make_float4(NOTDEF_F, 0.f, 0.f, 0.f); }
     else {
         const float deg = fast_atan2_deg((float)gx, (float)(-gy));
         ang[o] = deg;
-        const double a = (double)deg * DEG_TO_RADS;
-        const float af = (float)a;
-        pix4[o] = make_float4(deg, (float)cos((double)af), (float)sin((double)af), 0.f);
+        const float2 cs = P.trig_tab[(DA + 255) * TRIG_N + (BC + 255)];
+        pix4[o] = make_float4(deg, cs.x, cs.y, 0.f);
         atomicMax(&misc->g2max, (uint32_t)g2);
     }
 }
@@ -1431,6 +1503,7 @@
     DevBuf d_in, d_kl, d_desc, d_eq, d_n;
     int stage_lines = 0;
     int pre_B = 0;
+    bool byte_taps = false;
     int tie_order = 0;
     int top_only = 0;
     int sort_smem_g = 0, sort_smem_l = 0, sort_rows = 0, sort_rows_long = 0;
@@ -1463,9 +1536,28 @@
     return true;
 }
 
+static void host_trig_table(float* out ) {
+    for (int DA = -255; DA <= 255; DA++)
+        for (int BC = -255; BC <= 255; BC++) {
+            const int gx = DA + BC, gy = DA - BC;
+            const float deg = lsd::fast_atan2_deg((float)gx, (float)(-gy));
+            const double a = (double)deg * lsd::DEG_TO_RADS;
+            const float af = (float)a;
+            float* e = out + 2 * ((size_t)(DA + 255) * lsd::TRIG_N + (BC + 255));
+            e[0] = (float)std::cos((double)af); e[1] = (float)std::sin((double)af);
+        }
+}
+
 extern "C" {
 
 int planar_lsd_max_segments(void) { return lsd::MAX_SEGS; }
+
+int planar_lsd_trig_table(float* out, int64_t out_floats) {
+    PLANAR_REQUIRE(out != nullptr, PLANAR_EINVAL, "null argument");
+    PLANAR_REQUIRE(out_floats >= (int64_t)2 * lsd::TRIG_N * lsd::TRIG_N, PLANAR_EINVAL, "buffer too small");
+    host_trig_table(out);
+    return PLANAR_OK;
+}
 
 int planar_lsd_create(planar_ctx* ctx, int width, int height, int max_batch, planar_lsd** out) {
     PLANAR_REQUIRE(ctx && out, PLANAR_EINVAL, "null argument");
@@ -1487,6 +1579,11 @@
     if (1 + 2 * (int)hk != 7) { delete o; set_error("planar_lsd_create: unexpected LSD Gaussian size"); return PLANAR_EINVAL; }
     host_taps_q8(7, sigma, P.taps7);
     host_taps_q8(5, 1.0, P.taps5);
+    o->byte_taps = true;
+    for (int t : P.taps7) o->byte_taps = o->byte_taps && t >= 0 && t <= 255;
+    for (int t : P.taps5) o->byte_taps = o->byte_taps && t >= 0 && t <= 255;
+    P.g2_rho = -1;
+    while (P.g2_rho < 8 * 255 * 255 && std::sqrt((P.g2_rho + 1) / 4.0) <= P.rho) P.g2_rho++;
     P.log_nt = 5 * (std::log10(double(P.w)) + std::log10(double(P.h))) / 2 + std::log10(11.0);
     P.min_reg_size = (int)(size_t)(-P.log_nt / std::log10(P.p));
     {
@@ -1527,6 +1624,14 @@
     int rc = o->d_lgamma.alloc(lgam.size() * 8);
     if (rc) { delete o; return rc; }
     P.lgamma_tab = o->d_lgamma.as<double>();
+    if (!ctx->lsd_trig.p) {
+        std::vector<float> trig((size_t)2 * lsd::TRIG_N * lsd::TRIG_N);
+        host_trig_table(trig.data());
+        rc = ctx->lsd_trig.alloc(trig.size() * 4);
+        if (rc) { delete o; return rc; }
+        if (hipMemcpy(ctx->lsd_trig.p, trig.data(), trig.size() * 4, hipMemcpyHostToDevice) != hipSuccess) { ctx->lsd_trig.release(); delete o; set_error("planar_lsd_create: table upload failed"); return PLANAR_EDEVICE; }
+    }
+    P.trig_tab = ctx->lsd_trig.as<float2>();
     if (hipMemcpy(o->d_lgamma.p, lgam.data(), lgam.size() * 8, hipMemcpyHostToDevice) != hipSuccess) { delete o; set_error("planar_lsd_create: table upload failed"); return PLANAR_EDEVICE; }
     rc = o->d_plan.alloc(sizeof(lsd::Plan));
     if (!rc) rc = o->d_cx.alloc(cx.size() * sizeof(lsd::Coef));
@@ -1571,8 +1676,10 @@
     o->prof.mark(st);
     const dim3 gfull((unsigned)(((P.W + 63) / 64) * ((P.H + 15) / 16) * B));
     if ((P.W & 3) == 0 && (pitch & 3) == 0 && (frame_stride & 3) == 0 && ((uintptr_t)d_gray & 3) == 0 && (P.off_blur7 & 3) == 0 && (P.off_blur5 & 3) == 0 && (P.frame_bytes & 3) == 0)
-        hipLaunchKernelGGL(lsd::lsd_gauss75, gfull, dim3(256), 0, st, d_gray, pitch, frame_stride, P.W, P.H, o->d_taps.as<int>(), ws, P.frame_bytes, P.off_blur7, P.off_blur5, B);
-    else {
+    {
+        const auto gauss75 = o->byte_taps ? lsd::lsd_gauss75 : lsd::lsd_gauss75_wide;
+        hipLaunchKernelGGL(gauss75, gfull, dim3(256), 0, st, d_gray, pitch, frame_stride, P.W, P.H, o->d_taps.as<int>(), ws, P.frame_bytes, P.off_blur7, P.off_blur5, B);
+    } else {
         hipLaunchKernelGGL(lsd::lsd_gauss<7>, gfull, dim3(256), 0, st, d_gray, pitch, frame_stride, P.W, P.H, o->d_taps.as<int>(), ws, P.frame_bytes, P.off_blur7, B);
         hipLaunchKernelGGL(lsd::lsd_gauss<5>, gfull, dim3(256), 0, st, d_gray, pitch, frame_stride, P.W, P.H, o->d_taps.as<int>() + 8, ws, P.frame_bytes, P.off_blur5, B);
     }
@@ -1729,6 +1836,9 @@
             ((int32_t*)out)[0] = m.n_refine & 0xffff; ((int32_t*)out)[1] = m.n_refine >> 16;
             return PLANAR_OK;
         }
+        case 8: bytes = (size_t)P.W * P.H; off = P.off_blur7; break;
+        case 9: bytes = (size_t)P.W * P.H; off = P.off_blur5; break;
+        case 10: bytes = NPs * 16; off = P.off_pix; break;
         default: set_error("planar_lsd_read_stage: unknown stage"); return PLANAR_EINVAL;
     }
     PLANAR_REQUIRE((int64_t)bytes <= out_bytes, PLANAR_EINVAL, "buffer too small");
diff --git a/planarslam_amd/csrc/orb.hip b/planarslam_amd/csrc/orb.hip
--- a/planarslam_amd/csrc/orb.hip
+++ b/planarslam_amd/csrc/orb.hip
@@ -96,6 +96,94 @@
     for (int i = 0; i < 4; i++)
         if (x0 + i < L.w) packed |= (uint32_t)s[x0 + i] << (8 * i);
     *(uint32_t*)(pyr + (int64_t)blockIdx.y * plan->pyr_stride + L.off + (int64_t)y * L.pitch + x0) = packed;
+}
+
+struct PyrSpan { short clo, chi, olo, ohi; };
+struct PyrGroupDev { int l_first, l_last, ntx, nty, sx_off, sy_off, buf_a, buf_b, tx_cap; };
+struct PyrGroup { PyrGroupDev dev; int smem; };
+#ifndef PLANAR_PYR_LEVELS
+#define PLANAR_PYR_LEVELS 16
+#endif
+#ifndef PLANAR_PYR_TILE
+#define PLANAR_PYR_TILE 32
+#endif
+constexpr int PYR_TILE = PLANAR_PYR_TILE, PYR_LDS_BUDGET = 64 * 1024;
+
+__global__ __launch_bounds__(256) void orb_pyramid(const PlanDev* __restrict__ plan, const short4* __restrict__ tabs, const PyrSpan* __restrict__ spans,
+                                                   const uint8_t* __restrict__ gray, int pitch, int64_t frame_stride, uint8_t* __restrict__ pyr, PyrGroupDev G, int B) {
+    extern __shared__ __attribute__((aligned(16))) uint8_t s_pyr[];
+    short4* s_tx = (short4*)(s_pyr + G.buf_a + G.buf_b);
+    short4* s_ty = s_tx + G.tx_cap;
+    int frame, tile;
+    xcd_frame_block(G.ntx * G.nty, B, frame, tile);
+    const int tx = tile % G.ntx, ty = tile / G.ntx, tid = threadIdx.x;
+    uint8_t* fr = pyr + (int64_t)frame * plan->pyr_stride;
+    const int ls = G.l_first - 1;
+    PyrSpan X = spans[G.sx_off + tx], Y = spans[G.sy_off + ty];
+    {
+        const LevelDev& S = plan->lv[ls];
+        const bool from_gray = ls == 0;
+        const uint8_t* src = from_gray ? gray + (int64_t)frame * frame_stride : fr + S.off;
+        const int sp = from_gray ? pitch : S.pitch;
+        const bool aligned = (((uintptr_t)src | (uintptr_t)sp) & 3) == 0;
+        const int cw4 = (X.chi - X.clo) >> 2, n = cw4 * (Y.chi - Y.clo);
+        uint32_t* dst = (uint32_t*)s_pyr;
+        for (int i = tid; i < n; i += 256) {
+            const int r = i / cw4, q = i - r * cw4, x = X.clo + 4 * q, y = Y.clo + r;
+            const uint8_t* row = src + (int64_t)y * sp;
+            uint32_t v = 0;
+            if (aligned && x + 3 < S.w) v = *(const uint32_t*)(row + x);
+            else {
+#pragma unroll
+                for (int k = 0; k < 4; k++)
+                    if (x + k < S.w) v |= (uint32_t)row[x + k] << (8 * k);
+            }
+            dst[i] = v;
+            if (from_gray && x >= X.olo && x < X.ohi && y >= Y.olo && y < Y.ohi) *(uint32_t*)(fr + S.off + (int64_t)y * S.pitch + x) = v;
+        }
+    }
+    for (int l = G.l_first; l <= G.l_last; l++) {
+        const int li = l - ls;
+        const PyrSpan PX = X, PY = Y;
+        X = spans[G.sx_off + li * G.ntx + tx]; Y = spans[G.sy_off + li * G.nty + ty];
+        const LevelDev& L = plan->lv[l];
+        const short4* gtx = tabs + L.rs_off;
+        const short4* gty = gtx + L.pitch;
+        const int cw = X.chi - X.clo, ch = Y.chi - Y.clo, pcw = PX.chi - PX.clo;
+        for (int i = tid; i < cw + ch; i += 256) {
+            if (i < cw) {
+                short4 t = make_short4(0, 0, 0, 0);
+                if (X.clo + i < L.w) { t = gtx[X.clo + i]; t.x -= PX.clo; t.y -= PX.clo; }
+                s_tx[i] = t;
+            } else {
+                short4 t = gty[Y.clo + i - cw];
+                t.x -= PY.clo; t.y -= PY.clo;
+                s_ty[i - cw] = t;
+            }
+        }
+        __syncthreads();
+        const uint8_t* prev = (li & 1) ? s_pyr : s_pyr + G.buf_a;
+        uint32_t* cur = (uint32_t*)((li & 1) ? s_pyr + G.buf_a : s_pyr);
+        const int cw4 = cw >> 2, n = cw4 * ch;
+        for (int i = tid; i < n; i += 256) {
+            const int r = i / cw4, q = i - r * cw4;
+            const short4 vy = s_ty[r];
+            const uint8_t* r0 = prev + (int)vy.x * pcw;
+            const uint8_t* r1 = prev + (int)vy.y * pcw;
+            uint32_t packed = 0;
+#pragma unroll
+            for (int k = 0; k < 4; k++) {
+                const short4 t = s_tx[4 * q + k];
+                const int h0 = r0[t.x] * t.z + r0[t.y] * t.w;
+                const int h1 = r1[t.x] * t.z + r1[t.y] * t.w;
+                packed |= ((uint32_t)(((((int)vy.z * (h0 >> 4)) >> 16) + (((int)vy.w * (h1 >> 4)) >> 16) + 2) >> 2) & 0xffu) << (8 * k);
+            }
+            cur[i] = packed;
+            const int x = X.clo + 4 * q, y = Y.clo + r;
+            if (x >= X.olo && x < X.ohi && y >= Y.olo && y < Y.ohi) *(uint32_t*)(fr + L.off + (int64_t)y * L.pitch + x) = packed;
+        }
+        __syncthreads();
+    }
 }
 
 __device__ __forceinline__ bool has9(uint32_t m16) {
@@ -583,7 +671,7 @@
 __global__ __launch_bounds__(256) void orb_blur(const PlanDev* __restrict__ plan, const TileDev* __restrict__ tiles,
                                                 const uint8_t* __restrict__ pyr, uint8_t* __restrict__ blur, int n_tiles, int B) {
     __shared__ uint32_t s_pw[22][19];
-    __shared__ __attribute__((aligned(8))) uint16_t s_h[22][68];
+    __shared__ __attribute__((aligned(16))) uint32_t s_h[11][68];
     int frame, tile;
     xcd_frame_block(n_tiles, B, frame, tile);
     const TileDev T = tiles[tile];
@@ -611,32 +699,34 @@
         s_pw[r][wq] = w;
     }
     __syncthreads();
-    for (int i = tid; i < 22 * 16; i += 256) {
-        const int r = i >> 4, q = i & 15;
-        const uint32_t w0 = s_pw[r][q], w1 = s_pw[r][q + 1], w2 = s_pw[r][q + 2];
-        uint32_t b[10];
-        b[0] = (w0 >> 8) & 255u; b[1] = (w0 >> 16) & 255u; b[2] = w0 >> 24;
-        b[3] = w1 & 255u; b[4] = (w1 >> 8) & 255u; b[5] = (w1 >> 16) & 255u; b[6] = w1 >> 24;
-        b[7] = w2 & 255u; b[8] = (w2 >> 8) & 255u; b[9] = (w2 >> 16) & 255u;
-        uint32_t o[4];
-#pragma unroll
-        for (int j = 0; j < 4; j++) {
-            const uint32_t v = 18u * (b[j] + b[j + 6]) + 34u * (b[j + 1] + b[j + 5]) + 49u * (b[j + 2] + b[j + 4]) + 55u * b[j + 3];
-            o[j] = min(v, 65535u);
-        }
-        *(uint2*)&s_h[r][4 * q] = make_uint2(o[0] | (o[1] << 16), o[2] | (o[3] << 16));
+    if (tid < 11 * 16) {
+        const int p = tid >> 4, q = tid & 15;
+        constexpr uint32_t KLO = 18u | (34u << 8) | (49u << 16) | (55u << 24), KHI = 49u | (34u << 8) | (18u << 16);
+        uint32_t h[2][4];
+#pragma unroll
+        for (int e = 0; e < 2; e++) {
+            const uint32_t w0 = s_pw[2 * p + e][q], w1 = s_pw[2 * p + e][q + 1], w2 = s_pw[2 * p + e][q + 2];
+#pragma unroll
+            for (int j = 0; j < 4; j++) {
+                const uint32_t lo = j == 3 ? w1 : byte_window(w1, w0, j + 1), hi = j == 3 ? w2 : byte_window(w2, w1, j + 1);
+                h[e][j] = udot4_u8(hi, KHI, udot4_u8(lo, KLO, 0u));
+            }
+        }
+        *(uint4*)&s_h[p][4 * q] = make_uint4(h[0][0] | (h[1][0] << 16), h[0][1] | (h[1][1] << 16), h[0][2] | (h[1][2] << 16), h[0][3] | (h[1][3] << 16));
     }
     __syncthreads();
     {
         const int c4 = (tid & 15) * 4, r = tid >> 4;
-        uint32_t acc[4] = {0, 0, 0, 0};
-        const uint32_t taps[7] = {18u, 34u, 49u, 55u, 49u, 34u, 18u};
-#pragma unroll
-        for (int k = 0; k < 7; k++) {
-            const uint2 v = *(const uint2*)&s_h[r + k][c4];
-            acc[0] += taps[k] * (v.x & 0xffffu); acc[1] += taps[k] * (v.x >> 16);
-            acc[2] += taps[k] * (v.y & 0xffffu); acc[3] += taps[k] * (v.y >> 16);
-        }
+        const bool odd = r & 1;
+        const uint32_t k0 = odd ? (18u << 16) : (18u | (34u << 16)), k1 = odd ? (34u | (49u << 16)) : (49u | (55u << 16));
+        const uint32_t k2 = odd ? (55u | (49u << 16)) : (49u | (34u << 16)), k3 = odd ? (34u | (18u << 16)) : 18u;
+        const uint4 v0 = *(const uint4*)&s_h[(r >> 1)][c4], v1 = *(const uint4*)&s_h[(r >> 1) + 1][c4];
+        const uint4 v2 = *(const uint4*)&s_h[(r >> 1) + 2][c4], v3 = *(const uint4*)&s_h[(r >> 1) + 3][c4];
+        uint32_t acc[4];
+        acc[0] = udot2_u16(v3.x, k3, udot2_u16(v2.x, k2, udot2_u16(v1.x, k1, udot2_u16(v0.x, k0, 0u))));
+        acc[1] = udot2_u16(v3.y, k3, udot2_u16(v2.y, k2, udot2_u16(v1.y, k1, udot2_u16(v0.y, k0, 0u))));
+        acc[2] = udot2_u16(v3.z, k3, udot2_u16(v2.z, k2, udot2_u16(v1.z, k1, udot2_u16(v0.z, k0, 0u))));
+        acc[3] = udot2_u16(v3.w, k3, udot2_u16(v2.w, k2, udot2_u16(v1.w, k1, udot2_u16(v0.w, k0, 0u))));
         uint32_t packed = 0;
 #pragma unroll
         for (int i = 0; i < 4; i++) packed |= min((acc[i] + 32768u) >> 16, 255u) << (8 * i);
@@ -759,10 +849,57 @@
     DevBuf d_plan, d_cells, d_tiles, d_tabs, d_pyr, d_blur, d_cand, d_cell_count, d_sortA, d_sortB, d_level_count,
         d_kept, d_kept_count, d_dropped;
     DevBuf d_in, d_kps, d_desc, d_nout;
+    std::vector<PyrGroup> pyr_groups;
+    DevBuf d_spans;
     std::vector<const char*> launch_names;
     LaunchProfile prof;
     explicit planar_orb(int nlevels) : prof(nlevels + 5) {}
 };
+
+static int plan_pyr_group(const PlanDev& P, const std::vector<short4>& tabs, int l_first, int l_last, std::vector<PyrSpan>& spans, PyrGroup& G) {
+    const LevelDev& T = P.lv[l_last];
+    const int ntx = (T.w + PYR_TILE - 1) / PYR_TILE, nty = (T.h + PYR_TILE - 1) / PYR_TILE, ls = l_first - 1, nlv = l_last - ls + 1;
+    const int sx_off = (int)spans.size(), sy_off = sx_off + nlv * ntx;
+    spans.resize(spans.size() + (size_t)nlv * (ntx + nty));
+    std::vector<int> maxw(nlv, 0), maxh(nlv, 0);
+    for (int axis = 0; axis < 2; axis++) {
+        const bool isx = axis == 0;
+        const int nt = isx ? ntx : nty;
+        PyrSpan* out = spans.data() + (isx ? sx_off : sy_off);
+        for (int t = 0; t < nt; t++) {
+            int n = isx ? T.w : T.h;
+            int olo = t * PYR_TILE, ohi = std::min((t + 1) * PYR_TILE, n), nlo = olo, nhi = ohi;
+            for (int l = l_last; l >= ls; l--) {
+                const LevelDev& L = P.lv[l];
+                n = isx ? L.w : L.h;
+                int clo, chi, wlo = olo, whi = ohi;
+                if (isx) {
+                    wlo = olo & ~3; whi = ohi == n ? L.pitch : ohi & ~3;
+                    clo = std::min(nlo, wlo) & ~3;
+                    chi = ohi == n ? L.pitch : (std::max(nhi, whi) + 3) & ~3;
+                    maxw[l - ls] = std::max(maxw[l - ls], chi - clo);
+                } else {
+                    clo = std::min(nlo, olo); chi = std::max(nhi, ohi);
+                    maxh[l - ls] = std::max(maxh[l - ls], chi - clo);
+                }
+                out[(l - ls) * nt + t] = PyrSpan{(short)clo, (short)chi, (short)wlo, (short)whi};
+                if (l == ls) break;
+                const short4* tab = tabs.data() + L.rs_off + (isx ? 0 : L.pitch);
+                const int nprev = isx ? P.lv[l - 1].w : P.lv[l - 1].h;
+                nlo = tab[clo].x; nhi = tab[std::min(chi, n) - 1].y + 1;
+                olo = olo == 0 ? 0 : tab[olo].x; ohi = ohi == n ? nprev : tab[ohi].x;
+            }
+        }
+    }
+    int buf[2] = {0, 0}, tx_cap = 0, ty_cap = 0;
+    for (int i = 0; i < nlv; i++) {
+        buf[i & 1] = std::max(buf[i & 1], align_up(maxw[i] * maxh[i], 16));
+        if (i > 0) { tx_cap = std::max(tx_cap, maxw[i]); ty_cap = std::max(ty_cap, maxh[i]); }
+    }
+    G.dev = PyrGroupDev{l_first, l_last, ntx, nty, sx_off, sy_off, buf[0], buf[1], tx_cap};
+    G.smem = buf[0] + buf[1] + (tx_cap + ty_cap) * (int)sizeof(short4);
+    return G.smem;
+}
 
 static inline int cv_round_f(float v) { return (int)nearbyintf(v); }
 static inline int cv_round_d(double v) { return (int)nearbyint(v); }
@@ -941,9 +1078,31 @@
     if (e == hipSuccess && o->oct_smem > 64 * 1024)
         e = hipFuncSetAttribute((const void*)orb_octree, hipFuncAttributeMaxDynamicSharedMemorySize, o->oct_smem);
     if (e != hipSuccess) { delete o; set_error("planar_orb_create: upload failed: %s", hipGetErrorString(e)); return PLANAR_EDEVICE; }
-    o->launch_names.push_back("orb_copy_level0");
-    for (int l = 1; l < nl; l++) o->launch_names.push_back("orb_resize");
+    {
+        std::vector<PyrSpan> spans;
+        bool ok = nl > 1;
+        for (int l = 1; ok && l < nl;) {
+            int last = std::min(nl - 1, l + PLANAR_PYR_LEVELS - 1);
+            PyrGroup G;
+            for (;; last--) {
+                const size_t keep = spans.size();
+                if (plan_pyr_group(P, tabs, l, last, spans, G) <= PYR_LDS_BUDGET) break;
+                spans.resize(keep);
+                if (last == l) { ok = false; break; }
+            }
+            if (ok) { o->pyr_groups.push_back(G); l = last + 1; }
+        }
+        if (ok) {
+            if ((rc = o->d_spans.alloc(spans.size() * sizeof(PyrSpan)))) { delete o; return rc; }
+            if (hipMemcpy(o->d_spans.p, spans.data(), spans.size() * sizeof(PyrSpan), hipMemcpyHostToDevice) != hipSuccess) { delete o; set_error("planar_orb_create: upload failed"); return PLANAR_EDEVICE; }
+        } else o->pyr_groups.clear();
+    }
+    if (o->pyr_groups.empty()) {
+        o->launch_names.push_back("orb_copy_level0");
+        for (int l = 1; l < nl; l++) o->launch_names.push_back("orb_resize");
+    } else for (size_t g = 0; g < o->pyr_groups.size(); g++) o->launch_names.push_back("orb_pyramid");
     for (const char* n : {"orb_fast_cells", "orb_sort", "orb_octree", "orb_blur", "orb_describe"}) o->launch_names.push_back(n);
+    o->prof.set_slots((int)o->launch_names.size());
     *out = o;
     return PLANAR_OK;
 }
@@ -1008,12 +1167,17 @@
     if (rc) return rc;
     auto mark = [&]() { o->prof.mark(st); };
     mark();
-    {
+    for (const PyrGroup& G : o->pyr_groups) {
+        hipLaunchKernelGGL(orb_pyramid, dim3((unsigned)(G.dev.ntx * G.dev.nty) * B), dim3(256), G.smem, st, dp, o->d_tabs.as<short4>(), o->d_spans.as<PyrSpan>(),
+                           d_gray, pitch, frame_stride, pyr, G.dev, B);
+        mark();
+    }
+    if (o->pyr_groups.empty()) {
         const int n = (P.lv[0].pitch / 4) * P.lv[0].h;
         hipLaunchKernelGGL(orb_copy_level0, dim3((n + 255) / 256, B), dim3(256), 0, st, dp, d_gray, pitch, frame_stride, pyr);
         mark();
     }
-    for (int l = 1; l < P.nlevels; l++) {
+    for (int l = 1; o->pyr_groups.empty() && l < P.nlevels; l++) {
         const int n = (P.lv[l].pitch / 4) * P.lv[l].h;
         hipLaunchKernelGGL(orb_resize, dim3((n + 255) / 256, B), dim3(256), 0, st, dp, o->d_tabs.as<short4>(), pyr, l);
         mark();
diff --git a/planarslam_amd/lines.py b/planarslam_amd/lines.py
--- a/planarslam_amd/lines.py
+++ b/planarslam_amd/lines.py
@@ -52,6 +52,10 @@
             out = np.zeros(4, np.int64)
         elif stage == 7:
             out = np.zeros(2, np.int32)
+        elif stage in (8, 9):
+            out = np.zeros((self.H, self.W), np.uint8)
+        elif stage == 10:
+            out = np.zeros((h, w, 4), np.float32)
         else:
             out = np.zeros(1, np.int32)
         r = check(lib().planar_lsd_read_stage(self.h, frame, stage, out.ctypes.data, out.nbytes))
@@ -67,6 +71,12 @@
             self.close()
         except Exception:
             pass
+
+
+def trig_table():
+    out = np.zeros((511, 511, 2), np.float32)
+    check(lib().planar_lsd_trig_table(out.ctypes.data, out.size))
+    return out
 
 
 def is_line_good(keylines, n_lines, depth, seeds, cam=(535.4, 539.2, 320.1, 247.6), depth_factor=1.0 / 5000.0, ctx: Context | None = None):
```

Result: no change. 12670 (median of 2 runs) (+0.0%).
